# rakhimovv/lvt

Hardware: AMD Instinct MI355X
Metric: video-clips/sec/node (VQVAE+DSFVT train step, BAIR 64x64x16) (higher is better)
Workload: dtype f32

## Files before the change

include/lvt_hip.h:

```cpp
#ifndef LVT_HIP_H
#define LVT_HIP_H
#include <stddef.h>
#include <stdint.h>
#ifdef __cplusplus
extern "C" {
#endif

#define LVT_OK            0
#define LVT_EINVAL      (-1)
#define LVT_EWORKSPACE  (-2)
#define LVT_ELAUNCH     (-3)
#define LVT_ENODEVICE   (-4)

const char *lvt_last_error(void);
int lvt_version(void);
int lvt_device_info(char *name, int name_len, int *cus, int *clock_khz, long long *hbm_bytes);

#define LVT_MATH_F32   (1 << 16)
#define LVT_MATH_F16X2 (1 << 18)
typedef struct { const float *a; const float *b; float *c; } lvt_amax_io;
int lvt_amax(const float *x, long long n, float *out, void *stream);
typedef struct { const float *x; long long n; float *out; } lvt_amax_entry;
int lvt_amax_multi(const lvt_amax_entry *entries, int n, void *stream);
int lvt_amax_merge(const float *a, const float *b, float *out, void *stream);
#define LVT_VQ_COARSE  (1 << 17)
#define LVT_VQ_GENERIC (1 << 22)

#define LVT_EPI_BIAS        1
#define LVT_EPI_RESIDUAL    2
#define LVT_EPI_RELU        4
#define LVT_EPI_TANH        8
#define LVT_EPI_MASK       16
#define LVT_EPI_ACCUM      32
#define LVT_EPI_PLANES     64
#define LVT_CAUSAL_KMAX   (1 << 8)
#define LVT_CAUSAL_KMIN   (1 << 9)
#define LVT_CAUSAL_TILE   (1 << 10)

typedef struct {
    int M, N, K;
    int ta, tb;
    const float *A; long long lda; int a_kb; long long a_skb;
    const float *B; long long ldb; int b_kb; long long b_skb;
    float *C;       long long ldc;
    int batch_outer, batch_inner;
    long long sA_o, sA_i, sB_o, sB_i, sC_o, sC_i;
    float alpha;
    int flags;
    const float *bias;
    const float *res;  long long ldr;
    const float *mask; long long ldm;
    int splits;
    float *a_colsum;
    long long c_plane;
    const float *a_amax, *b_amax;
    const float *a_amax2, *b_amax2;
    float *c_amax;
} lvt_gemm_desc;
size_t lvt_gemm_workspace_bytes(const lvt_gemm_desc *d);
int lvt_gemm_f32(const lvt_gemm_desc *d, void *workspace, size_t workspace_bytes, void *stream);

int lvt_vq_argmax_scores(const float *scores, long long rows, int K, long long ld, const float *codebook, int D,
                         long long *idx, void *stream);

typedef struct {
    int M, N, K;
    const void *A; long long lda; int a_planes; int a_kb; long long a_skb;
    const void *B; long long ldb;
    float *C; long long ldc;
    int batch_outer, batch_inner;
    long long sA_o, sA_i, sB_o, sB_i, sC_o, sC_i;
    float alpha;
    int flags;
    const float *bias;
    const float *res;  long long ldr;
    const float *mask; long long ldm;
    const float *a_amax, *b_amax;
    float *c_amax;
    void *Cp; long long ldcp; const float *cp_amax;
} lvt_gemm_p2_desc;
int lvt_gemm_p2_f32(const lvt_gemm_p2_desc *d, void *stream);
typedef struct { const float *src; void *dst; int rows, cols; long long ld_src, ld_dst; int transpose; const float *amax;
                 int batch; long long bs_src, bs_dst; } lvt_p2_pack_entry;
int lvt_p2_pack_multi(const lvt_p2_pack_entry *entries, int n, void *stream);

int lvt_gemm_smallm_f32(int M, int N, int K, int tb, const float *A, long long lda, const float *B,
                        long long ldb, float *C, long long ldc, int batch, long long sB, long long sC,
                        float alpha, int flags, const float *bias, const float *res, long long ldr,
                        const int *pos, long long c_pos, long long r_pos, void *stream);
size_t lvt_gemm_smallm_splitk_workspace_bytes(int M, int N, int splits);
int lvt_gemm_smallm_splitk_f32(int M, int N, int K, int splits, const float *A, long long lda, const float *B,
                               long long ldb, float *C, long long ldc, float alpha, int flags, const float *bias,
                               const float *res, long long ldr, const int *pos, long long c_pos, long long r_pos,
                               void *workspace, size_t workspace_bytes, void *stream);
int lvt_gemm_smallm_partial_f32(int M, int N, int K, int splits, const float *A, long long lda, const float *B,
                                long long ldb, void *workspace, size_t workspace_bytes, void *stream);
int lvt_splitsum_layernorm_fwd(const float *partials, int splits, int rows, int d, const float *bias, const float *res,
                               long long ldr, float *x_out, float eps, const float *w, const float *b, float *y,
                               void *stream);

typedef struct {
    int N, Ti, Hi, Wi, Ci;
    int To, Ho, Wo, Co;
    int Kt, Kh, Kw;
    int st, sh, sw;
    int pt, ph, pw;
} lvt_conv_geom;
int lvt_conv3d_pack_weight(const lvt_conv_geom *g, const float *w, int Ci_real, int Co_real,
                           float *wp, void *stream);
typedef struct { const float *w; float *dst; int kind, taps, Ci, Co, Ci_real, Co_real; } lvt_pack_entry;
int lvt_conv3d_pack_weights_multi(const lvt_pack_entry *entries, int n, void *stream);
#define LVT_CONV_WEIGHT_IMAGE (1 << 21)
typedef struct { const float *wp; int rows, cols; const float *amax; } lvt_weight_image_entry;
size_t lvt_conv3d_weight_image_bytes(int rows, int cols);
int lvt_conv3d_weight_images(const lvt_weight_image_entry *entries, int n, void *stream);
int lvt_conv3d_pack_weight_t(const lvt_conv_geom *g, const float *w, int Ci_real, int Co_real,
                             float *wt, void *stream);
int lvt_conv3d_uses_patch_kernel(const lvt_conv_geom *g, int flags);
int lvt_conv3d_fwd_uses_parity_kernel(const lvt_conv_geom *g, int flags);
int lvt_conv3d_pack_weight_parity(const lvt_conv_geom *g, const float *w, int Ci_real, int Co_real,
                                  float *wq, void *stream);
int lvt_conv3d_fwd_parity(const lvt_conv_geom *g, const float *x, const float *wq, const float *bias,
                          const float *res, const float *mask, float *y, int flags, const lvt_amax_io *ax,
        void *stream);
int lvt_conv3d_fwd(const lvt_conv_geom *g, const float *x, const float *wp, const float *bias,
                   const float *res, const float *mask, float *y, int flags, const lvt_amax_io *ax,
        void *stream);
int lvt_conv3d_bwd_data_uses_phase_kernel(const lvt_conv_geom *g, int flags);
int lvt_conv3d_pack_weight_phases(const lvt_conv_geom *g, const float *w, int Ci_real, int Co_real,
                                  float *wph, void *stream);
int lvt_conv3d_bwd_data_phases(const lvt_conv_geom *g, const float *dy, const float *wph, const float *bias,
                               const float *res, const float *mask, float *dx, int flags, const lvt_amax_io *ax,
        void *stream);
int lvt_conv3d_bwd_data(const lvt_conv_geom *g, const float *dy, const float *wp, const float *bias,
                        const float *res, const float *mask, float *dx, int flags, const lvt_amax_io *ax,
        void *stream);
size_t lvt_conv3d_bwd_weight_workspace_bytes(const lvt_conv_geom *g);
int lvt_conv3d_bwd_weight_fuses_bias(const lvt_conv_geom *g, int flags);
#define LVT_WGRAD_DB_OF_X (1 << 20)
int lvt_conv3d_bwd_weight(const lvt_conv_geom *g, const float *x, const float *dy, float *dw, float *db,
                          int Ci_real, int Co_real, int flags, const lvt_amax_io *ax, void *workspace,
                          size_t workspace_bytes, void *stream);
int lvt_convt4_fwd(const float *x, const float *w, const float *bias, int N, int Hi, int Wi, int Ci, int Cr,
                   int act_tanh, float *y, int flags, const lvt_amax_io *ax, void *stream);
size_t lvt_colsum_workspace_bytes(long long M, int N);
int lvt_colsum(const float *g, long long M, int N, long long ld, float *out, void *workspace,
               size_t workspace_bytes, void *stream);

size_t lvt_vq_nearest_workspace_bytes(long long rows, int num, int KC);
size_t lvt_vq_nearest_generic_workspace_bytes(int num, int D, int KC);
int lvt_vq_nearest(const float *z, long long rows, int ldz, int num, int D, int KC,
                   const float *codebooks, long long *idx, int P, int flags, void *workspace, size_t workspace_bytes,
                   void *stream);
int lvt_vq_gather(const long long *idx, const float *codebooks, long long rows, int num, int D, int KC,
                  int P, float *out, int ldo, void *stream);
size_t lvt_vq_ema_workspace_bytes(long long rows, int num, int D, int KC);
int lvt_vq_ema_accumulate(const long long *idx, const float *z, long long rows, int ldz, int num, int D,
                          int KC, int P, float *stats, void *workspace, size_t workspace_bytes,
                          void *stream);
int lvt_vq_ema_finalize(const float *stats, int num, int D, int KC, float decay, float eps,
                        float *running_size, float *running_sum, float *weight, void *stream);

int lvt_to_channels_last(const float *in, int B, int C, long long R, int ldo, int mode, const float *a,
                         const float *s, float *out, float *out_amax, void *stream);
int lvt_to_channels_first(const float *in, int B, int C, long long R, int ldi, int mode, const float *a,
                          const float *s, float lo, float hi, float *out, void *stream);

size_t lvt_reduce_workspace_bytes(void);
int lvt_mse_fwd(const float *a, const float *b, long long n, double denom, float scale, float *out,
                void *workspace, size_t workspace_bytes, void *stream);
int lvt_mse_bwd(const float *a, const float *b, long long n, double denom, float scale,
                const float *gout_dev, const float *add, int tanh_of_a, float *out, float *out_amax, void *stream);
int lvt_l1_fwd(const float *a, const float *b, long long n, double denom, float scale, float *out,
               void *workspace, size_t workspace_bytes, void *stream);
int lvt_l1_bwd(const float *a, const float *b, long long n, double denom, float scale,
               const float *gout_dev, const float *add, int tanh_of_a, float *out, float *out_amax, void *stream);
int lvt_tanh_bwd(const float *g, const float *y, long long n, float *out, float *out_amax, void *stream);
int lvt_axpy(const float *x, const float *add, long long n, const float *alpha_dev, float alpha,
             float *out, void *stream);
int lvt_add_periodic(float *x, const float *table, long long rows, int P, int d, void *stream);

int lvt_layernorm_fwd(const float *x, long long rows, int d, float eps, const float *w, const float *b,
                      float *y, float *mean, float *rstd, float *y_amax, const float *w_amax, const float *b_amax,
                      void *stream);
int lvt_layernorm_fwd_p2(const float *x, long long rows, int d, float eps, const float *w, const float *b,
                         float *y, void *yp, float *mean, float *rstd, float *y_amax, const float *w_amax,
                         const float *b_amax, void *stream);
size_t lvt_layernorm_bwd_workspace_bytes(int d);
int lvt_layernorm_bwd(const float *dy, const float *x, const float *mean, const float *rstd,
                      const float *w, long long rows, int d, const float *add, float *dx, float *dw,
                      float *db, float *dx_amax, void *workspace, size_t workspace_bytes, void *stream);

int lvt_attn_softmax_fwd(float *scores, int B, int H, int S, float temper, const float *dt,
                         const float *dh, const float *dw, int bt, int bh, int bw, int masked, float fill,
                         void *stream);
int lvt_attn_softmax_bwd(const float *P, float *dP, int B, int H, int S, float temper, int bt, int bh,
                         int bw, float *G, float *ddt, float *ddh, float *ddw, void *stream);

int lvt_attn_fwd(const float *q, const float *k, const float *v, int B, int H, int S, int da, float temper,
                 const float *dt, const float *dh, const float *dw, int bt, int bh, int bw, int masked, float fill,
                 float *P, float *o, void *stream);

int lvt_attn_planes_supported(int S, int da, int bt, int bh, int bw);
int lvt_attn_fwd_planes(const void *qkv_planes, long long plane_stride, long long operand_stride, int B, int H, int S, int da,
                        float temper, const float *dt, const float *dh, const float *dw, int bt, int bh, int bw, int masked,
                        float fill, float *P, float *o, float *o_amax, void *stream);
size_t lvt_attn_bwd_planes_workspace_bytes(int B, int H, int S, int bt, int bh, int bw);
int lvt_attn_bwd_planes(const void *qkv_planes, long long plane_stride, long long operand_stride, const void *do_planes,
                        const float *P, const float *o, int B, int H, int S, int da, float temper, int bt, int bh, int bw,
                        int masked, float *dq, float *dk, float *dv, float *ddt, float *ddh, float *ddw, float *d_amax,
                        void *workspace, size_t workspace_bytes, void *stream);

int lvt_attn_flash_supported(int S, int da, int bt, int bh, int bw);
int lvt_attn_fwd_flash(const float *q, const float *k, const float *v, long long ld, int B, int H, int S, int da,
                       float temper, const float *dt, const float *dh, const float *dw, int bt, int bh, int bw,
                       int masked, float fill, float *o, float *stats, float *o_amax, void *stream);
size_t lvt_attn_bwd_flash_workspace_bytes(int B, int H, int S, int bt, int bh, int bw);
int lvt_attn_bwd_flash(const float *q, const float *k, const float *v, const float *d_o, long long ld, const float *stats,
                       const float *o, int B, int H, int S, int da, float temper, const float *dt, const float *dh, const float *dw,
                       int bt, int bh, int bw, int masked, float fill, float *dq, float *dk, float *dv, float *ddt,
                       float *ddh, float *ddw, float *d_amax, void *workspace, size_t workspace_bytes, void *stream);

int lvt_attn_decode(const float *q, long long ldq, const float *Kc, const float *Vc, int B, int H, int S, int da, int qi,
                    float temper, const float *dt, const float *dh, const float *dw, int bt, int bh, int bw,
                    float *o, const int *pos, long long q_pos, void *stream);

int lvt_decode_gather_codes(const long long *codes, const long long *nb, const int *pos, int rows, int S1, int taps,
                            long long *out, void *stream);
int lvt_decode_commit(const long long *drawn, int rows, int S1, long long *codes, int *pos, void *stream);

int lvt_sample_categorical(const float *logits, long long rows, int V, float temp, const float *u,
                           long long *out, long long out_stride, float *probs, const int *pos, long long u_pos,
                           void *stream);

int lvt_embbag_fwd(const long long *idx, long long bstride, int P, long long rows, int nslots,
                   const int *slot_off, const int *tab_row, const float *table, int D, const float *bias,
                   const float *btable, const long long *bindex, float *out, void *stream);
#define LVT_ONEHOT_DENSE (1 << 19)
size_t lvt_onehot_tn_workspace_bytes(int nslots, int V, int N, long long rows);
int lvt_onehot_tn_is_gather(int nslots, int V, int N, long long ldb, const float *dout, int flags);
int lvt_onehot_tn_gemm(const long long *idx, int nslots, int V, const int *slot_off, long long bstride,
                       long long pstride, int P, long long rows, const float *dout, long long ldb, int N,
                       float *out, int flags, const float *dout_amax, void *workspace, size_t workspace_bytes,
                       void *stream);
int lvt_permute3(const float *in, long long s0, long long s1, long long s2, int n0, int n1, int n2,
                 float *out, void *stream);

int lvt_row_gather(const float *x, const long long *perm, long long B, int S, int d, float *out, void *stream);

int lvt_slice_context(const long long *video, int B, int T, int nc, int H, int W, const int *abc, int st, int sh,
                      int sw, int kt, int kh, int kw, int n_prime, long long pad_value, long long *ctx,
                      long long *slice, long long *slice_idx, unsigned char *ignore, void *stream);

size_t lvt_xent_workspace_bytes(void);
int lvt_xent_fwd(const float *logits, const long long *target, long long tstride_b, long long tstride_pos,
                 int P, long long rows, int V, long long ignore, float scale, float *row_loss, float *lse,
                 float *loss, float *count, void *workspace, size_t workspace_bytes, void *stream);
int lvt_xent_bwd(const float *logits, const long long *target, long long tstride_b, long long tstride_pos,
                 int P, long long rows, int V, long long ignore, const float *lse, const float *count,
                 const float *gout, float scale, float *dlogits, float *dl_amax, void *stream);

typedef struct {
    float *p; const float *g; float *s0; float *s1;
    long long n; float lr; float wd;
} lvt_opt_entry;
int lvt_adam_step(const lvt_opt_entry *entries, int n, float beta1, float beta2, float eps, int step,
                  void *stream);
int lvt_rmsprop_step(const lvt_opt_entry *entries, int n, float alpha, float eps, float momentum,
                     void *stream);

#define LVT_BN_RUNNING  1
#define LVT_BN_UPDATE   2
#define LVT_BN_UNBIASED 4
#define LVT_BN_COUNT    8
#define LVT_BN_TRAIN    16
size_t lvt_bn_workspace_bytes(long long M, int Cp);
int lvt_bn_stats(const float *y, long long M, int Cp, float *stats, void *workspace, size_t workspace_bytes, void *stream);
int lvt_bn_finalize(const float *stats, int nranks, long long count, int C, int Cp, const float *gamma, const float *beta,
                    float *running_mean, float *running_var, long long *num_batches_tracked, float momentum, float eps,
                    int flags, float *scale, float *shift, float *saved, void *stream);
int lvt_bn_apply(const float *y, const float *res, long long M, int Cp, const float *scale, const float *shift, int flags,
                 float *out, float *out_amax, void *stream);
int lvt_bn_bwd_reduce(const float *g, const float *y, long long M, int Cp, const float *saved, float *sums, void *workspace,
                      size_t workspace_bytes, void *stream);
int lvt_bn_bwd_apply(const float *g, const float *y, long long M, int Cp, const float *scale, const float *saved,
                     const float *sums, long long n, int flags, float *dy, float *dy_amax, void *stream);
typedef struct {
    const float *w; float *w_out; int outer, Co, inner, Cp;
    const float *gamma, *beta, *running_mean, *running_var; float eps;
    float *bias_out; float *w_amax;
} lvt_bn_fold_entry;
int lvt_bn_fold(const lvt_bn_fold_entry *entries, int n, void *stream);

#ifdef __cplusplus
}
#endif
#endif
```

lvt_amd/csrc/attention_flash.hip:

```cpp
#include "attn_common.h"

namespace {

template <int I> struct IC { static constexpr int value = I; };
template <int N, int I = 0, class F> __device__ __forceinline__ void static_for(F &&f) {
    if constexpr (I < N) { f(IC<I>{}); static_for<N, I + 1>(f); }
}

typedef _Float16 f16x8 __attribute__((ext_vector_type(8)));
typedef _Float16 f16x2v __attribute__((ext_vector_type(2)));
typedef float f32x2 __attribute__((ext_vector_type(2)));
typedef float f32x4v __attribute__((ext_vector_type(4)));
typedef short s16x4 __attribute__((ext_vector_type(4)));
typedef __attribute__((address_space(3))) s16x4 lds_s16x4;
typedef unsigned u32x4 __attribute__((ext_vector_type(4)));

#define FA_LD 144
#define FA_PL (64 * FA_LD)
#define FA_SLOT (2 * FA_PL)
#define FA_EMIN 30
#define FA_EMAX 254
#define FA_LOG2E 1.4426950408889634f

typedef unsigned u32x2 __attribute__((ext_vector_type(2)));

__device__ __forceinline__ float fa_u2f(unsigned u) { return __uint_as_float(u); }
__device__ __forceinline__ float fa_exp_field(int e) { return e <= 0 ? 0.f : fa_u2f((unsigned)e << 23); }
__device__ __forceinline__ int fa_clamp_e(int e) { return e < FA_EMIN ? FA_EMIN : (e > FA_EMAX ? FA_EMAX : e); }
__device__ __forceinline__ int fa_ebits(float nonneg) { return fa_clamp_e((int)((__float_as_uint(nonneg) >> 23) & 0xffu)); }
template <int CTRL> __device__ __forceinline__ float fa_dpp_max(float v) {
    const int o = __builtin_amdgcn_update_dpp(0, __builtin_bit_cast(int, v), CTRL, 0xf, 0xf, false);
    return fmaxf(v, __builtin_bit_cast(float, o));
}
__device__ __forceinline__ float fa_row16_max(float v) {
    v = fa_dpp_max<0xB1>(v);
    v = fa_dpp_max<0x4E>(v);
    v = fa_dpp_max<0x141>(v);
    v = fa_dpp_max<0x140>(v);
    return v;
}
__device__ __forceinline__ float fa_kg_max(float v) {
    u32x2 r = __builtin_amdgcn_permlane16_swap(__float_as_uint(v), __float_as_uint(v), false, false);
    v = fmaxf(fa_u2f(r[0]), fa_u2f(r[1]));
    r = __builtin_amdgcn_permlane32_swap(__float_as_uint(v), __float_as_uint(v), false, false);
    return fmaxf(fa_u2f(r[0]), fa_u2f(r[1]));
}
__device__ __forceinline__ float fa_kg_sum(float v) {
    u32x2 r = __builtin_amdgcn_permlane16_swap(__float_as_uint(v), __float_as_uint(v), false, false);
    v = fa_u2f(r[0]) + fa_u2f(r[1]);
    r = __builtin_amdgcn_permlane32_swap(__float_as_uint(v), __float_as_uint(v), false, false);
    return fa_u2f(r[0]) + fa_u2f(r[1]);
}
__device__ __forceinline__ float fa_max4(const f32x4v a) { return fmaxf(fmaxf(a[0], a[1]), fmaxf(a[2], a[3])); }
__device__ __forceinline__ float fa_absmax4(const float4 a) { return fmaxf(fmaxf(fabsf(a.x), fabsf(a.y)), fmaxf(fabsf(a.z), fabsf(a.w))); }

__device__ __forceinline__ float fa_mix_lo(unsigned h, float c) {
    float r;
    asm("v_fma_mix_f32 %0, %1, %2, %3 op_sel:[0,0,0] op_sel_hi:[1,0,0]" : "=v"(r) : "v"(h), "v"(-1.f), "v"(c));
    return r;
}
__device__ __forceinline__ float fa_mix_hi(unsigned h, float c) {
    float r;
    asm("v_fma_mix_f32 %0, %1, %2, %3 op_sel:[1,0,0] op_sel_hi:[1,0,0]" : "=v"(r) : "v"(h), "v"(-1.f), "v"(c));
    return r;
}
__device__ __forceinline__ void fa_split_pair(float a, float b, float s, unsigned &ph, unsigned &pl) {
    const f32x2 t = f32x2{a, b} * s;
    ph = __builtin_bit_cast(unsigned, __builtin_convertvector(t, f16x2v));
    const f32x2 r = {fa_mix_lo(ph, t.x), fa_mix_hi(ph, t.y)};
    pl = __builtin_bit_cast(unsigned, __builtin_convertvector(r, f16x2v));
}
__device__ __forceinline__ void fa_split_pair1(float a, float b, unsigned &ph, unsigned &pl) {
    const f32x2 t = {a, b};
    ph = __builtin_bit_cast(unsigned, __builtin_convertvector(t, f16x2v));
    const f32x2 r = {fa_mix_lo(ph, a), fa_mix_hi(ph, b)};
    pl = __builtin_bit_cast(unsigned, __builtin_convertvector(r, f16x2v));
}
__device__ __forceinline__ void fa_split8(const float (&v)[8], f16x8 &h, f16x8 &l) {
    u32x4 uh, ul;
    unsigned a, b;
    fa_split_pair1(v[0], v[1], a, b); uh[0] = a; ul[0] = b;
    fa_split_pair1(v[2], v[3], a, b); uh[1] = a; ul[1] = b;
    fa_split_pair1(v[4], v[5], a, b); uh[2] = a; ul[2] = b;
// ... 758 lines not shown
#pragma unroll
        for (int qt = 0; qt < 2; ++qt) {
            const int T = 2 * c + qt;
            const f32x4v qinv = *reinterpret_cast<const f32x4v *>(cinv + 16 * qt + 4 * kg);
            const f32x4v doinv = *reinterpret_cast<const f32x4v *>(cinv + 32 + 16 * qt + 4 * kg);
            const float bth = bt_[T / HP] + dhl[HSTEP * (T % HP)];
            const f32x4v qk = qinv * kc, bm = bw4 + bth;
            const f32x4v lds = l4[qt] * (doinv * srun);
            const f32x4v qzl = l4[qt] * qinv;
            const f32x4v dvq = (doinv * vinv) * qzl, dq_ = d4[qt] * qzl;
#pragma unroll
            for (int r = 0; r < 4; ++r) {
                float x = fa_score(st[qt][r], qk[r], bm[r]);
                if (MASKED && j > 16 * T + 4 * kg + r) x = A.fill2;
                const float ex = __builtin_amdgcn_exp2f(x - m4[qt][r]);
                pw[4 * qt + r] = ex * lds[r];
                u[4 * qt + r] = (ex * fmaf(dp[qt][r], dvq[r], -dq_[r])) * zrun;
            }
        }
        f16x8 pbh, pbl, ubh, ubl;
        fa_split8(pw, pbh, pbl);
        fa_split8(u, ubh, ubl);
        f16x8 ao[2][2], aqt[2];
        auto load_o = [&](int d_, int bf) {
#pragma unroll
            for (int pl = 0; pl < 2; ++pl) ao[bf][pl] = fa_trfrag(cur, pl, 32, d_, c16, kg);
        };
        load_o(0, 0);
        static_for<AT_D / 16>([&](auto dc) {
            constexpr int d = decltype(dc)::value, bf = d & 1;
#pragma unroll
            for (int pl = 0; pl < 2; ++pl) aqt[pl] = fa_trfrag(cur, pl, 0, d, c16, kg);
            accv[d] = fa_mfma(ao[bf][1], pbh, accv[d]);
            accv[d] = fa_mfma(ao[bf][0], pbl, accv[d]);
            accv[d] = fa_mfma(ao[bf][0], pbh, accv[d]);
            if constexpr (d + 1 < AT_D / 16) load_o(d + 1, bf ^ 1);
            acck[d] = fa_mfma(aqt[1], ubh, acck[d]);
            acck[d] = fa_mfma(aqt[0], ubl, acck[d]);
            acck[d] = fa_mfma(aqt[0], ubh, acck[d]);
            __builtin_amdgcn_sched_group_barrier(0x100, 4, 0);
            __builtin_amdgcn_sched_group_barrier(0x008, 3, 0);
            if constexpr (d + 1 < AT_D / 16) __builtin_amdgcn_sched_group_barrier(0x100, 4, 0);
            __builtin_amdgcn_sched_group_barrier(0x008, 3, 0);
            __builtin_amdgcn_sched_barrier(0);
        });
        __syncthreads();
    });
    const float fvs = domax * (1.f / 32768.f), fks = fa_exp_field(zb - 14) * A.inv_temper;
    float am = 0.f;
    {
        float *vrow = A.dv + (row0 + j) * A.ld + h * AT_D + 4 * kg, *krow = A.dk + (row0 + j) * A.ld + h * AT_D + 4 * kg;
#pragma unroll
        for (int d = 0; d < AT_D / 16; ++d) {
            const f32x4v ov = accv[d] * fvs, ok = acck[d] * fks;
            *reinterpret_cast<f32x4v *>(vrow + 16 * d) = ov;
            *reinterpret_cast<f32x4v *>(krow + 16 * d) = ok;
#pragma unroll
            for (int e = 0; e < 4; ++e) am = fmaxf(am, fmaxf(fabsf(ov[e]), fabsf(ok[e])));
        }
    }
    return am;
}

template <int BT, int BH, int BW, int MASKED>
__global__ __launch_bounds__(512, 1) void lvt_attn_bwd_flash_b_kernel(const FaArgs A, float *__restrict__ d_amax) {
    __shared__ __attribute__((aligned(16))) FaSmemB sm;
    if (threadIdx.x >= 256) __builtin_amdgcn_s_setprio(1);
    float am;
    if (MASKED) {
        if (fa_half(blockIdx.x) == 0) am = fa_bwd_b_body<BT, BH, BW, MASKED, 0, 8>(A, sm, fa_pair(blockIdx.x), 0);
        else am = fa_bwd_b_body<BT, BH, BW, MASKED, 4, 4>(A, sm, fa_pair(blockIdx.x), 1);
    } else {
        am = fa_bwd_b_body<BT, BH, BW, MASKED, 0, 8>(A, sm, fa_pair(blockIdx.x), fa_half(blockIdx.x));
    }
    if (d_amax) {
        __syncthreads();
        lvt_block_amax_commit(am, d_amax, reinterpret_cast<float *>(sm.ring[0]));
    }
}

__global__ __launch_bounds__(256) void lvt_attn_flash_bank_reduce_kernel(const float *__restrict__ partial, int B, int H, int NB, int nt,
                                                                         int nh, float *__restrict__ ddt, float *__restrict__ ddh,
                                                                         float *__restrict__ ddw) {
    const int idx = blockIdx.x * 4 + (threadIdx.x >> 6), lane = threadIdx.x & 63;
    if (idx >= H * NB) return;
    const int h = idx / NB, e = idx % NB;
    float s = 0.f;
    for (int jj = lane; jj < 2 * B; jj += 64) s += partial[(((long long)(jj >> 1) * H + h) * 2 + (jj & 1)) * NB + e];
#pragma unroll
    for (int m = 32; m >= 1; m >>= 1) s += __shfl_xor(s, m, 64);
    if (lane) return;
    const int nw = NB - nt - nh;
    if (e < nt) ddt[h * nt + e] = nt == 1 ? 0.f : s;
    else if (e < nt + nh) ddh[h * nh + e - nt] = nh == 1 ? 0.f : s;
    else ddw[h * nw + e - nt - nh] = nw == 1 ? 0.f : s;
}

}

extern "C" int lvt_attn_flash_supported(int S, int da, int bt, int bh, int bw) {
    return S == AT_S && da == AT_D && ((bt == 1 && bh == 16 && bw == 16) || (bt == 4 && bh == 8 && bw == 8)) ? 1 : 0;
}

#define LVT_FA_GEOMS(X) X(1, 16, 16) X(4, 8, 8)

extern "C" int lvt_attn_fwd_flash(const float *q, const float *k, const float *v, long long ld, int B, int H, int S, int da,
                                  float temper, const float *dt, const float *dh, const float *dw, int bt, int bh, int bw,
                                  int masked, float fill, float *o, float *stats, float *o_amax, void *stream) {
    LVT_REQUIRE(q && k && v && dt && dh && dw && o && stats && B > 0 && H > 0, "attn_fwd_flash: bad args");
    LVT_REQUIRE((B * H) % 8 == 0, "attn_fwd_flash: B * H = %d must be a multiple of 8 (workgroup pairing per XCD)", B * H);
    LVT_REQUIRE(lvt_attn_flash_supported(S, da, bt, bh, bw), "attn_fwd_flash: S=%d da=%d block (%d,%d,%d) has no instantiation", S, da, bt, bh, bw);
    LVT_REQUIRE(lvt_aligned16(q) && lvt_aligned16(k) && lvt_aligned16(v) && lvt_aligned16(o) && lvt_aligned16(stats) && ld % 4 == 0 &&
                ld >= (long long)H * da, "attn_fwd_flash: alignment / row stride");
    FaArgs A = {};
    A.q = q; A.k = k; A.v = v; A.ld = ld; A.H = H; A.inv_temper = 1.f / temper; A.c1 = FA_LOG2E / temper; A.fill2 = fill * FA_LOG2E;
    A.dt = dt; A.dh = dh; A.dw = dw; A.o = o; A.m = stats; A.l = stats + (size_t)B * H * S;
    const dim3 grid((unsigned)(B * H * (masked ? 1 : 2))), blk(512);
    hipStream_t s = (hipStream_t)stream;
#define LVT_X(BT, BH, BW)                                                                                       \
    if (bt == BT && bh == BH && bw == BW) {                                                                     \
        if (masked) hipLaunchKernelGGL((lvt_attn_fwd_flash_kernel<BT, BH, BW, 1>), grid, blk, 0, s, A, o_amax); \
        else hipLaunchKernelGGL((lvt_attn_fwd_flash_kernel<BT, BH, BW, 0>), grid, blk, 0, s, A, o_amax);        \
    }
    LVT_FA_GEOMS(LVT_X)
#undef LVT_X
    LVT_CHECK_LAUNCH("lvt_attn_fwd_flash_kernel");
    return LVT_OK;
}

extern "C" size_t lvt_attn_bwd_flash_workspace_bytes(int B, int H, int S, int bt, int bh, int bw) {
    const size_t nb = (size_t)(2 * bt - 1) + (2 * bh - 1) + (2 * bw - 1);
    return (size_t)B * H * S * sizeof(float) + (size_t)B * H * 4 * sizeof(float) + (size_t)B * H * 2 * nb * sizeof(float);
}

extern "C" int lvt_attn_bwd_flash(const float *q, const float *k, const float *v, const float *d_o, long long ld, const float *stats,
                                  const float *o, int B, int H, int S, int da, float temper, const float *dt, const float *dh, const float *dw,
                                  int bt, int bh, int bw, int masked, float fill, float *dq, float *dk, float *dv, float *ddt,
                                  float *ddh, float *ddw, float *d_amax, void *workspace, size_t workspace_bytes, void *stream) {
    LVT_REQUIRE(q && k && v && d_o && stats && dt && dh && dw && dq && dk && dv && ddt && ddh && ddw && B > 0 && H > 0, "attn_bwd_flash: bad args");
    LVT_REQUIRE((B * H) % 8 == 0, "attn_bwd_flash: B * H = %d must be a multiple of 8 (workgroup pairing per XCD)", B * H);
    LVT_REQUIRE(lvt_attn_flash_supported(S, da, bt, bh, bw), "attn_bwd_flash: S=%d da=%d block (%d,%d,%d) has no instantiation", S, da, bt, bh, bw);
    LVT_REQUIRE(lvt_aligned16(q) && lvt_aligned16(k) && lvt_aligned16(v) && lvt_aligned16(d_o) && lvt_aligned16(stats) && lvt_aligned16(dq) &&
                lvt_aligned16(dk) && lvt_aligned16(dv) && ld % 4 == 0 && ld >= (long long)H * da, "attn_bwd_flash: alignment / row stride");
    if (!workspace || workspace_bytes < lvt_attn_bwd_flash_workspace_bytes(B, H, S, bt, bh, bw) || !lvt_aligned16(workspace)) {
        lvt_set_error("attn_bwd_flash: workspace too small or misaligned");
        return LVT_EWORKSPACE;
    }
    FaArgs A = {};
    A.q = q; A.k = k; A.v = v; A.d_o = d_o; A.ld = ld; A.H = H; A.inv_temper = 1.f / temper; A.c1 = FA_LOG2E / temper; A.fill2 = fill * FA_LOG2E;
    A.dt = dt; A.dh = dh; A.dw = dw; A.m = const_cast<float *>(stats); A.l = const_cast<float *>(stats) + (size_t)B * H * S;
    A.dq = dq; A.dk = dk; A.dv = dv;
    LVT_REQUIRE(!o || lvt_aligned16(o), "attn_bwd_flash: o must be 16-byte aligned");
    const bool onep = o != nullptr;
    A.o = const_cast<float *>(o);
    A.delta = (float *)workspace;
    A.scal = A.delta + (size_t)B * H * S;
    A.bank_partial = A.scal + (size_t)B * H * 4;
    const int nt = 2 * bt - 1, nh = 2 * bh - 1, nw = 2 * bw - 1, nb = nt + nh + nw;
    const dim3 grid((unsigned)(B * H * (masked ? 1 : 2))), blk(512);
    const dim3 gridb((unsigned)(B * H * 2));
    hipStream_t s = (hipStream_t)stream;
#define LVT_X(BT, BH, BW)                                                                                         \
    if (bt == BT && bh == BH && bw == BW) {                                                                       \
        if (masked && onep) hipLaunchKernelGGL((lvt_attn_bwd_flash_a_kernel<BT, BH, BW, 1, 1>), grid, blk, 0, s, A, d_amax); \
        else if (masked) hipLaunchKernelGGL((lvt_attn_bwd_flash_a_kernel<BT, BH, BW, 1, 0>), grid, blk, 0, s, A, d_amax);    \
        else if (onep) hipLaunchKernelGGL((lvt_attn_bwd_flash_a_kernel<BT, BH, BW, 0, 1>), grid, blk, 0, s, A, d_amax);      \
        else hipLaunchKernelGGL((lvt_attn_bwd_flash_a_kernel<BT, BH, BW, 0, 0>), grid, blk, 0, s, A, d_amax);                \
    }
    LVT_FA_GEOMS(LVT_X)
#undef LVT_X
    LVT_CHECK_LAUNCH("lvt_attn_bwd_flash_a_kernel");
#define LVT_X(BT, BH, BW)                                                                                         \
    if (bt == BT && bh == BH && bw == BW) {                                                                       \
        if (masked) hipLaunchKernelGGL((lvt_attn_bwd_flash_b_kernel<BT, BH, BW, 1>), gridb, blk, 0, s, A, d_amax); \
        else hipLaunchKernelGGL((lvt_attn_bwd_flash_b_kernel<BT, BH, BW, 0>), grid, blk, 0, s, A, d_amax);        \
    }
    LVT_FA_GEOMS(LVT_X)
#undef LVT_X
    LVT_CHECK_LAUNCH("lvt_attn_bwd_flash_b_kernel");
    hipLaunchKernelGGL(lvt_attn_flash_bank_reduce_kernel, dim3((unsigned)lvt_cdiv((long long)H * nb, 4)), dim3(256), 0, s,
                       A.bank_partial, B, H, nb, nt, nh, ddt, ddh, ddw);
    LVT_CHECK_LAUNCH("lvt_attn_flash_bank_reduce_kernel");
    return LVT_OK;
}
```

lvt_amd/csrc/elementwise.hip:

```cpp
#include "lvt_common.h"

static inline int grid_for(long long n, int per_block, int cap = 8192) {
    long long b = lvt_cdiv(n, per_block);
    if (b < 1) b = 1;
    return (int)(b < cap ? b : cap);
}

__device__ __forceinline__ float wave_sum(float v) {
#pragma unroll
    for (int off = 32; off >= 1; off >>= 1) v += __shfl_xor(v, off);
    return v;
}
__device__ __forceinline__ float wave_max(float v) {
#pragma unroll
    for (int off = 32; off >= 1; off >>= 1) v = fmaxf(v, __shfl_xor(v, off));
    return v;
}

__global__ void lvt_to_channels_last_kernel(const float *__restrict__ in, int B, int C, long long R, int ldo,
                                            int mode, const float *__restrict__ a, const float *__restrict__ s,
                                            float *__restrict__ out, float *__restrict__ out_amax) {
    __shared__ float amax_scratch[4];
    float am = 0.f;
    const long long total = (long long)B * R * ldo;
    for (long long i = (long long)blockIdx.x * blockDim.x + threadIdx.x; i < total;
         i += (long long)gridDim.x * blockDim.x) {
        const int c = i % ldo; const long long t = i / ldo;
        const long long r = t % R; const long long b = t / R;
        float v = 0.f;
        if (c < C) {
            v = in[(b * C + c) * R + r];
            if (mode == 1) v = (v - a[c]) / s[c];
        }
        out[i] = v;
        am = fmaxf(am, lvt_absf(v));
    }
    if (out_amax) lvt_block_amax_commit(am, out_amax, amax_scratch);
}
__global__ void lvt_to_channels_first_kernel(const float *__restrict__ in, int B, int C, long long R, int ldi,
                                             int mode, const float *__restrict__ a, const float *__restrict__ s,
                                             float lo, float hi, float *__restrict__ out) {
    const long long total = (long long)B * C * R;
    for (long long i = (long long)blockIdx.x * blockDim.x + threadIdx.x; i < total;
         i += (long long)gridDim.x * blockDim.x) {
        const long long r = i % R; const long long t = i / R;
        const int c = t % C; const long long b = t / C;
        float v = in[(b * R + r) * ldi + c];
        if (mode == 2) { v = v * s[c] + a[c]; v = fminf(fmaxf(v, lo), hi); }
        out[i] = v;
    }
}

extern "C" int lvt_to_channels_last(const float *in, int B, int C, long long R, int ldo, int mode, const float *a,
                                    const float *s, float *out, float *out_amax, void *stream) {
    LVT_REQUIRE(in && out && B > 0 && C > 0 && R > 0 && ldo >= C, "to_channels_last: bad args");
    LVT_REQUIRE(mode == 0 || (a && s), "to_channels_last: affine tables missing");
    hipLaunchKernelGGL(lvt_to_channels_last_kernel, dim3(grid_for((long long)B * R * ldo, 256, out_amax ? 2048 : 8192)), dim3(256), 0,
                       (hipStream_t)stream, in, B, C, R, ldo, mode, a, s, out, out_amax);
    LVT_CHECK_LAUNCH("lvt_to_channels_last_kernel");
    return LVT_OK;
}
extern "C" int lvt_to_channels_first(const float *in, int B, int C, long long R, int ldi, int mode, const float *a,
                                     const float *s, float lo, float hi, float *out, void *stream) {
    LVT_REQUIRE(in && out && B > 0 && C > 0 && R > 0 && ldi >= C, "to_channels_first: bad args");
    LVT_REQUIRE(mode == 0 || (a && s), "to_channels_first: affine tables missing");
    hipLaunchKernelGGL(lvt_to_channels_first_kernel, dim3(grid_for((long long)B * C * R, 256)), dim3(256), 0,
                       (hipStream_t)stream, in, B, C, R, ldi, mode, a, s, lo, hi, out);
    LVT_CHECK_LAUNCH("lvt_to_channels_first_kernel");
    return LVT_OK;
}

#define RED_BLOCKS 1024
template <int L1>
__global__ void lvt_sqdiff_partial_kernel(const float *__restrict__ a, const float *__restrict__ b, long long n4,
                                          float *__restrict__ partial) {
    __shared__ float red[256];
    float s = 0.f;
    for (long long i = (long long)blockIdx.x * blockDim.x + threadIdx.x; i < n4;
         i += (long long)gridDim.x * blockDim.x) {
        const float4 x = reinterpret_cast<const float4 *>(a)[i];
        const float4 y = reinterpret_cast<const float4 *>(b)[i];
        const float d0 = x.x - y.x, d1 = x.y - y.y, d2 = x.z - y.z, d3 = x.w - y.w;
        if (L1) s += (fabsf(d0) + fabsf(d1)) + (fabsf(d2) + fabsf(d3));
// ... 284 lines not shown
    const int d4 = d / 4;
    float4 adw[LN_MAXV], adb[LN_MAXV];
#pragma unroll
    for (int i = 0; i < LN_MAXV; ++i) { adw[i] = make_float4(0.f, 0.f, 0.f, 0.f); adb[i] = adw[i]; }
    const long long rows_per_block = lvt_cdiv(rows, gridDim.x);
    const long long r0 = blockIdx.x * rows_per_block;
    const long long r1 = min(rows, r0 + rows_per_block);
    for (long long row0 = r0 + wave; row0 < r1; row0 += 4 * LN_BWD_ROWS) {
        float4 xh[LN_BWD_ROWS][LN_MAXV], gw[LN_BWD_ROWS][LN_MAXV], zv[LN_BWD_ROWS][LN_MAXV];
        float rs[LN_BWD_ROWS], s1[LN_BWD_ROWS], s2[LN_BWD_ROWS];
#pragma unroll
        for (int u = 0; u < LN_BWD_ROWS; ++u) {
            const long long row = row0 + 4 * u;
            if (row >= r1) continue;
            if (add) {
#pragma unroll
                for (int i = 0; i < LN_MAXV; ++i)
                    if (lane + 64 * i < d4) zv[u][i] = reinterpret_cast<const float4 *>(add + row * d)[lane + 64 * i];
            }
            const float m = mean[row];
            rs[u] = rstd[row];
            const float4 *xp = reinterpret_cast<const float4 *>(x + row * d);
            const float4 *gp = reinterpret_cast<const float4 *>(dy + row * d);
            s1[u] = 0.f; s2[u] = 0.f;
#pragma unroll
            for (int i = 0; i < LN_MAXV; ++i) {
                const int c = lane + 64 * i;
                if (c < d4) {
                    const float4 xv = xp[c], gv = gp[c], ww = reinterpret_cast<const float4 *>(w)[c];
                    const float r = rs[u];
                    xh[u][i] = make_float4((xv.x - m) * r, (xv.y - m) * r, (xv.z - m) * r, (xv.w - m) * r);
                    gw[u][i] = make_float4(gv.x * ww.x, gv.y * ww.y, gv.z * ww.z, gv.w * ww.w);
                    const float4 h = xh[u][i], g = gw[u][i];
                    s1[u] += (g.x + g.y) + (g.z + g.w);
                    s2[u] += (g.x * h.x + g.y * h.y) + (g.z * h.z + g.w * h.w);
                    adw[i].x += gv.x * h.x; adw[i].y += gv.y * h.y; adw[i].z += gv.z * h.z; adw[i].w += gv.w * h.w;
                    adb[i].x += gv.x; adb[i].y += gv.y; adb[i].z += gv.z; adb[i].w += gv.w;
                }
            }
        }
#pragma unroll
        for (int u = 0; u < LN_BWD_ROWS; ++u) {
            const long long row = row0 + 4 * u;
            if (row >= r1) continue;
            const float m1 = wave_sum(s1[u]) / d, m2 = wave_sum(s2[u]) / d;
            float4 *op = reinterpret_cast<float4 *>(dx + row * d);
#pragma unroll
            for (int i = 0; i < LN_MAXV; ++i) {
                const int c = lane + 64 * i;
                if (c < d4) {
                    const float4 h = xh[u][i], g = gw[u][i];
                    const float r = rs[u];
                    float4 o;
                    o.x = r * (g.x - m1 - h.x * m2); o.y = r * (g.y - m1 - h.y * m2);
                    o.z = r * (g.z - m1 - h.z * m2); o.w = r * (g.w - m1 - h.w * m2);
                    if (add) {
                        const float4 z = zv[u][i];
                        o.x += z.x; o.y += z.y; o.z += z.z; o.w += z.w;
                    }
                    op[c] = o;
                    am = fmaxf(am, fmaxf(fmaxf(lvt_absf(o.x), lvt_absf(o.y)), fmaxf(lvt_absf(o.z), lvt_absf(o.w))));
                }
            }
        }
    }
    if (dx_amax) lvt_block_amax_commit(am, dx_amax, amax_scratch);
#pragma unroll
    for (int i = 0; i < LN_MAXV; ++i) {
        const int c = lane + 64 * i;
        if (c < d4) {
            reinterpret_cast<float4 *>(sdw[wave])[c] = adw[i];
            reinterpret_cast<float4 *>(sdb[wave])[c] = adb[i];
        }
    }
    __syncthreads();
    for (int c = threadIdx.x; c < d; c += 256) {
        pdw[(long long)blockIdx.x * d + c] = ((sdw[0][c] + sdw[1][c]) + sdw[2][c]) + sdw[3][c];
        pdb[(long long)blockIdx.x * d + c] = ((sdb[0][c] + sdb[1][c]) + sdb[2][c]) + sdb[3][c];
    }
}
__global__ __launch_bounds__(256) void lvt_rowsum_partials_kernel(const float *__restrict__ partial0, const float *__restrict__ partial1,
                                                                  int nblk, int n, float *__restrict__ out0, float *__restrict__ out1) {
    __shared__ float red[256];
    const float *partial = blockIdx.y ? partial1 : partial0;
    float *out = blockIdx.y ? out1 : out0;
    constexpr int cols = 8, RL = 256 / cols;
    const int c = blockIdx.x * cols + (threadIdx.x % cols);
    const int rl = threadIdx.x / cols;
    float s0 = 0.f, s1 = 0.f, s2 = 0.f, s3 = 0.f;
    if (c < n) {
        int b = rl;
        for (; b + 3 * RL < nblk; b += 4 * RL) {
            s0 += partial[(long long)b * n + c]; s1 += partial[(long long)(b + RL) * n + c];
            s2 += partial[(long long)(b + 2 * RL) * n + c]; s3 += partial[(long long)(b + 3 * RL) * n + c];
        }
        for (; b < nblk; b += RL) s0 += partial[(long long)b * n + c];
    }
    float s = (s0 + s1) + (s2 + s3);
    red[threadIdx.x] = s;
    __syncthreads();
    if (rl == 0 && c < n) {
        for (int k = 1; k < RL; ++k) s += red[k * cols + threadIdx.x];
        out[c] = s;
    }
}
extern "C" size_t lvt_layernorm_bwd_workspace_bytes(int d) { return (size_t)2 * LN_BWD_BLOCKS * d * sizeof(float); }
extern "C" int lvt_layernorm_bwd(const float *dy, const float *x, const float *mean, const float *rstd,
                                 const float *w, long long rows, int d, const float *add, float *dx, float *dw,
                                 float *db, float *dx_amax, void *workspace, size_t workspace_bytes, void *stream) {
    LVT_REQUIRE(dy && x && mean && rstd && w && dx && dw && db && rows > 0 && d % 4 == 0 && d <= 256 * LN_MAXV,
                "layernorm_bwd: bad args");
    LVT_REQUIRE(workspace && workspace_bytes >= lvt_layernorm_bwd_workspace_bytes(d), "layernorm_bwd: workspace");
    hipStream_t s = (hipStream_t)stream;
    int blocks = (int)(lvt_cdiv(rows, 8) < LN_BWD_BLOCKS ? lvt_cdiv(rows, 8) : LN_BWD_BLOCKS);
    const long long rpb = lvt_cdiv(rows, blocks);
    blocks = (int)lvt_cdiv(rows, rpb);
    float *pdw = (float *)workspace, *pdb = pdw + (size_t)LN_BWD_BLOCKS * d;
    hipLaunchKernelGGL(lvt_layernorm_bwd_kernel, dim3(blocks), dim3(256), 0, s, dy, x, mean, rstd, w, rows, d, add,
                       dx, pdw, pdb, dx_amax);
    LVT_CHECK_LAUNCH("lvt_layernorm_bwd_kernel");
    hipLaunchKernelGGL(lvt_rowsum_partials_kernel, dim3((d + 7) / 8, 2), dim3(256), 0, s, (const float *)pdw, (const float *)pdb,
                       blocks, d, dw, db);
    LVT_CHECK_LAUNCH("lvt_rowsum_partials_kernel");
    return LVT_OK;
}

struct SliceGeom { int B, T, nc, H, W, st, sh, sw, kt, kh, kw, n_prime, t, h, w, Tc, Hc, Wc; long long pad; };
__global__ void lvt_slice_context_kernel(const long long *__restrict__ video, const int *__restrict__ abc, SliceGeom g,
                                         long long *__restrict__ ctx, long long *__restrict__ slice,
                                         long long *__restrict__ slice_idx, unsigned char *__restrict__ ignore) {
    const long long n_ctx = (long long)g.B * g.nc * g.Tc * g.Hc * g.Wc;
    const long long n_sl = (long long)g.B * g.nc * g.t * g.h * g.w;
    const long long n_ig = (long long)g.B * g.t * g.h * g.w;
    const long long total = n_ctx + n_sl + n_ig + g.B;
    for (long long i = (long long)blockIdx.x * blockDim.x + threadIdx.x; i < total; i += (long long)gridDim.x * blockDim.x) {
        if (i < n_ctx) {
            long long r = i;
            const int ow = r % g.Wc; r /= g.Wc;
            const int oh = r % g.Hc; r /= g.Hc;
            const int ot = r % g.Tc; r /= g.Tc;
            const int ch = r % g.nc; const int b = r / g.nc;
            const int a = abc[3 * b], bo = abc[3 * b + 1], c = abc[3 * b + 2];
            const int ti = ot - g.kt / 2 + a, hi = oh - g.kh / 2 + bo, wi = ow - g.kw / 2 + c;
            long long v = g.pad;
            if ((unsigned)ti < (unsigned)g.T && (unsigned)hi < (unsigned)g.H && (unsigned)wi < (unsigned)g.W) {
                const int mine = ((ti % g.st) * g.sh + (hi % g.sh)) * g.sw + (wi % g.sw);
                if (mine < (a * g.sh + bo) * g.sw + c)
                    v = video[((((long long)b * g.T + ti) * g.nc + ch) * g.H + hi) * g.W + wi];
            }
            ctx[i] = v;
        } else if (i < n_ctx + n_sl) {
            long long r = i - n_ctx;
            const int wi = r % g.w; r /= g.w;
            const int hi = r % g.h; r /= g.h;
            const int ti = r % g.t; r /= g.t;
            const int ch = r % g.nc; const int b = r / g.nc;
            const int a = abc[3 * b], bo = abc[3 * b + 1], c = abc[3 * b + 2];
            slice[i - n_ctx] = video[((((long long)b * g.T + ti * g.st + a) * g.nc + ch) * g.H + hi * g.sh + bo) * g.W + wi * g.sw + c];
        } else if (i < n_ctx + n_sl + n_ig) {
            long long r = i - n_ctx - n_sl;
            r /= (long long)g.h * g.w;
            const int ti = r % g.t; const int b = r / g.t;
            ignore[i - n_ctx - n_sl] = (ti * g.st + abc[3 * b]) < g.n_prime ? 1 : 0;
        } else {
            const int b = (int)(i - n_ctx - n_sl - n_ig);
            slice_idx[b] = (abc[3 * b] * g.sh + abc[3 * b + 1]) * g.sw + abc[3 * b + 2];
        }
    }
}
extern "C" int lvt_slice_context(const long long *video, int B, int T, int nc, int H, int W, const int *abc, int st, int sh,
                                 int sw, int kt, int kh, int kw, int n_prime, long long pad_value, long long *ctx,
                                 long long *slice, long long *slice_idx, unsigned char *ignore, void *stream) {
    LVT_REQUIRE(video && abc && ctx && slice && slice_idx && ignore, "slice_context: null pointer");
    LVT_REQUIRE(B > 0 && nc > 0 && st > 0 && sh > 0 && sw > 0 && T % st == 0 && H % sh == 0 && W % sw == 0 &&
                kt > 0 && kh > 0 && kw > 0, "slice_context: bad geometry");
    SliceGeom g;
    g.B = B; g.T = T; g.nc = nc; g.H = H; g.W = W; g.st = st; g.sh = sh; g.sw = sw; g.kt = kt; g.kh = kh; g.kw = kw;
    g.n_prime = n_prime; g.pad = pad_value;
    g.t = T / st; g.h = H / sh; g.w = W / sw;
    g.Tc = 2 * (kt / 2) + (g.t - 1) * st + 1; g.Hc = 2 * (kh / 2) + (g.h - 1) * sh + 1; g.Wc = 2 * (kw / 2) + (g.w - 1) * sw + 1;
    const long long total = (long long)B * nc * g.Tc * g.Hc * g.Wc + (long long)B * (nc + 1) * g.t * g.h * g.w + B;
    const int blocks = (int)(lvt_cdiv(total, 256) < 4096 ? lvt_cdiv(total, 256) : 4096);
    hipLaunchKernelGGL(lvt_slice_context_kernel, dim3(blocks), dim3(256), 0, (hipStream_t)stream, video, abc, g, ctx, slice,
                       slice_idx, ignore);
    LVT_CHECK_LAUNCH("lvt_slice_context_kernel");
    return LVT_OK;
}

__global__ void lvt_row_gather_kernel(const float *__restrict__ x, const long long *__restrict__ perm, long long B, int S,
                                      int d4, float *__restrict__ out) {
    const long long total = B * S * d4;
    for (long long i = (long long)blockIdx.x * blockDim.x + threadIdx.x; i < total; i += (long long)gridDim.x * blockDim.x) {
        const int c = i % d4; const long long r = i / d4;
        const int s = r % S; const long long b = r / S;
        reinterpret_cast<float4 *>(out)[i] = reinterpret_cast<const float4 *>(x)[(b * S + perm[s]) * d4 + c];
    }
}
extern "C" int lvt_row_gather(const float *x, const long long *perm, long long B, int S, int d, float *out, void *stream) {
    LVT_REQUIRE(x && perm && out && B > 0 && S > 0 && d > 0 && d % 4 == 0 && lvt_aligned16(x) && lvt_aligned16(out),
                "row_gather: bad args");
    const long long total = B * S * (d / 4);
    const int blocks = (int)(lvt_cdiv(total, 256) < 8192 ? lvt_cdiv(total, 256) : 8192);
    hipLaunchKernelGGL(lvt_row_gather_kernel, dim3(blocks), dim3(256), 0, (hipStream_t)stream, x, perm, B, S, d / 4, out);
    LVT_CHECK_LAUNCH("lvt_row_gather_kernel");
    return LVT_OK;
}

// ... 74 lines not shown
```

lvt_amd/csrc/gemm_engine.hip:

```cpp
#include "lvt_common.h"
#include "epilogue_fast.h"
#include <string.h>
#include <stdlib.h>
#include <stdint.h>
#include <type_traits>

typedef float f32x16 __attribute__((ext_vector_type(16)));

#define BK 32
#define NTHREADS 256

enum { A_KPLAIN = 0, A_MPLAIN = 1, A_CONV_K = 2, A_CONVT_K = 3, A_CONV_M = 4, A_ONEHOT_M = 5, A_PATCH = 6, A_PATCHT = 7 };
enum { B_KPLAIN = 0, B_NPLAIN = 1, B_CONVT_W = 2 };

struct KParams {
    int M, N, K;
    const float *A; long long lda; int a_kb; long long a_skb;
    const float *B; long long ldb; int b_kb; long long b_skb;
    float *C; long long ldc; long long c_plane;
    int batch_inner;
    long long sA_o, sA_i, sB_o, sB_i, sC_o, sC_i;
    float alpha; int flags;
    const float *bias; const float *res; long long ldr; const float *mask; long long ldm;
    int splits; int k_per_split; float *partial; long long partial_stride;
    int vec_epi;
    float *colsum_partial;
    const float *a_amax, *b_amax;
    const float *a_amax2, *b_amax2;
    float *c_amax;
    lvt_conv_geom g;
    const char *b_img;
    int Tq, Hq, Wq;
    int jT, jH, jW;
    const long long *oh_idx; long long oh_bstride, oh_pstride; int oh_P, oh_V; int oh_off[32];
};

__device__ __forceinline__ float4 ldg4(const float *p) { return *reinterpret_cast<const float4 *>(p); }

__device__ __forceinline__ unsigned cvt_pk_bf16(float lo, float hi) {
    unsigned r;
    asm("v_cvt_pk_bf16_f32 %0, %1, %2" : "=v"(r) : "v"(lo), "v"(hi));
    return r;
}
__device__ __forceinline__ float bf_lo(unsigned p) { return __uint_as_float(p << 16); }
__device__ __forceinline__ float bf_hi(unsigned p) { return __uint_as_float(p & 0xffff0000u); }
__device__ __forceinline__ void split3(const float4 v, uint2 &p1, uint2 &p2, uint2 &p3) {
    p1.x = cvt_pk_bf16(v.x, v.y); p1.y = cvt_pk_bf16(v.z, v.w);
    const float r0 = v.x - bf_lo(p1.x), r1 = v.y - bf_hi(p1.x), r2 = v.z - bf_lo(p1.y), r3 = v.w - bf_hi(p1.y);
    p2.x = cvt_pk_bf16(r0, r1); p2.y = cvt_pk_bf16(r2, r3);
    const float s0 = r0 - bf_lo(p2.x), s1 = r1 - bf_hi(p2.x), s2 = r2 - bf_lo(p2.y), s3 = r3 - bf_hi(p2.y);
    p3.x = cvt_pk_bf16(s0, s1); p3.y = cvt_pk_bf16(s2, s3);
}
#define HLD 40
template <int ROWS> __device__ __forceinline__ int hrow(int m) {
    if (ROWS >= 128) {
        const int r = (m & ~127) + ((m & 3) << 5) + ((m & 127) >> 2);
        return r * HLD + (r >> 5) * 32;
    }
    return m * HLD;
}
template <int ROWS> struct HPlane { static constexpr int SIZE = ROWS * HLD + (ROWS >= 128 ? ROWS : 0); };
template <int ROWS> __device__ __forceinline__ void store_split_k(unsigned short *lds, int row, int k4, const float4 v) {
    uint2 p1, p2, p3;
    split3(v, p1, p2, p3);
    unsigned short *d = lds + hrow<ROWS>(row) + k4;
    *reinterpret_cast<uint2 *>(d) = p1;
    *reinterpret_cast<uint2 *>(d + HPlane<ROWS>::SIZE) = p2;
    *reinterpret_cast<uint2 *>(d + 2 * HPlane<ROWS>::SIZE) = p3;
}
template <int ROWS> __device__ __forceinline__ void store_split_m(unsigned short *lds, int row4, int k, const float4 v) {
    uint2 p[3];
    split3(v, p[0], p[1], p[2]);
#pragma unroll
    for (int q = 0; q < 3; ++q) {
        unsigned short *d = lds + q * HPlane<ROWS>::SIZE + k;
        d[hrow<ROWS>(row4)] = (unsigned short)(p[q].x & 0xffffu); d[hrow<ROWS>(row4 + 1)] = (unsigned short)(p[q].x >> 16);
        d[hrow<ROWS>(row4 + 2)] = (unsigned short)(p[q].y & 0xffffu); d[hrow<ROWS>(row4 + 3)] = (unsigned short)(p[q].y >> 16);
    }
}
template <int ROWS> __device__ __forceinline__ void store_split_block(unsigned short *lds, int row4, int k4, const float4 *v) {
    store_split_k<ROWS>(lds, row4 + 0, k4, make_float4(v[0].x, v[1].x, v[2].x, v[3].x));
    store_split_k<ROWS>(lds, row4 + 1, k4, make_float4(v[0].y, v[1].y, v[2].y, v[3].y));
    store_split_k<ROWS>(lds, row4 + 2, k4, make_float4(v[0].z, v[1].z, v[2].z, v[3].z));
    store_split_k<ROWS>(lds, row4 + 3, k4, make_float4(v[0].w, v[1].w, v[2].w, v[3].w));
// ... 1343 lines not shown
                for (int i = 0; i < TM; ++i) a[q][i] = *reinterpret_cast<const f16x8 *>(cur + fa[i] + q * PSA + ks);
#pragma unroll
                for (int j = 0; j < TN; ++j) b[q][j] = *reinterpret_cast<const f16x8 *>(cur + fb[j] + q * PSB + ks);
            }
#pragma unroll
            for (int i = 0; i < TM; ++i)
#pragma unroll
                for (int j = 0; j < TN; ++j)
                    acx[i][j] = __builtin_amdgcn_mfma_f32_32x32x16_f16(a[0][i], b[1][j], acx[i][j], 0, 0, 0);
#pragma unroll
            for (int i = 0; i < TM; ++i)
#pragma unroll
                for (int j = 0; j < TN; ++j)
                    acc[i][j] = __builtin_amdgcn_mfma_f32_32x32x16_f16(a[0][i], b[0][j], acc[i][j], 0, 0, 0);
#pragma unroll
            for (int i = 0; i < TM; ++i)
#pragma unroll
                for (int j = 0; j < TN; ++j)
                    acx[i][j] = __builtin_amdgcn_mfma_f32_32x32x16_f16(a[1][i], b[0][j], acx[i][j], 0, 0, 0);
            if (ks == 0) {
                if constexpr (decltype(do_store)::value) store(nxt);
                if constexpr (decltype(do_fetch)::value) fetch();
            }
        }
    };
    typedef std::integral_constant<bool, true> yes_t;
    typedef std::integral_constant<bool, false> no_t;

    const int ntiles = kbeg < kend ? (kend - kbeg) / BK : 0;
    if (ntiles > 0) {
        fetch();
        store(S0);
        if (ntiles > 1) fetch();
    }
    __syncthreads();
    int kt = 0;
    for (; kt + 2 < ntiles; ++kt) {
        tile(S0 + (kt & 1) * STAGE, S0 + ((kt + 1) & 1) * STAGE, yes_t(), yes_t());
        __syncthreads();
    }
    if (kt + 1 < ntiles) {
        tile(S0 + (kt & 1) * STAGE, S0 + ((kt + 1) & 1) * STAGE, yes_t(), no_t());
        __syncthreads();
        ++kt;
    }
    if (kt < ntiles) tile(S0 + (kt & 1) * STAGE, nullptr, no_t(), no_t());
    __syncthreads();
    lvt_f16x2_finish<TM, TN>(acc, acx, unscale);

    if (TA && sum_on) {
        float *scratch = lds;
        *reinterpret_cast<float4 *>(&scratch[(kk0 * 64 + mq) * 4]) = colacc;
        __syncthreads();
        if (tid < BM) {
            float s_ = 0.f;
            for (int r = 0; r < 8; ++r) s_ += scratch[(r * 64 + tid / 4) * 4 + (tid & 3)];
            if (m0 + tid < p.M) p.colsum_partial[((long long)tc.split * gridDim.y + tc.z) * p.M + m0 + tid] = s_;
        }
        __syncthreads();
    }
    if (p.vec_epi && !(p.flags & (LVT_EPI_PLANES | LVT_EPI_ACCUM | LVT_EPI_TANH))) {
        LvtEpi e;
        e.M = p.M; e.N = p.N;
        float *wave_tile = lds + wave * (32 * TN * 32);
        if (p.splits > 1) {
            e.C = p.partial; e.ldc = p.N; e.coff = tc.split * p.partial_stride + (long long)tc.z * p.M * p.N; e.alpha = 1.f; e.flags = 0;
            e.bias = nullptr; e.res = nullptr; e.ldr = 0; e.mask = nullptr; e.ldm = 0;
            (void)lvt_epi_fast_wave<0, TM, TN>(e, acc, wave_tile, m0 + wm * (TM * 32), n0 + wn * (TN * 32), lane);
            return;
        }
        const unsigned seen = lvt_amax_peek(p.c_amax);
        e.C = p.C; e.ldc = p.ldc; e.coff = tc.coff; e.alpha = p.alpha; e.flags = p.flags;
        e.bias = p.bias; e.res = p.res; e.ldr = p.ldr; e.mask = p.mask; e.ldm = p.ldm;
        const float am_w = lvt_epi_fast_dispatch<TM, TN>(e, acc, wave_tile, m0 + wm * (TM * 32), n0 + wn * (TN * 32), lane);
        if (p.c_amax) lvt_block_amax_commit_seen(am_w, p.c_amax, lds + TURN_FLOATS, seen);
        return;
    }
    if (p.vec_epi) lvt_epilogue_vec<AMODE, BM, BN, WM, WN>(p, acc, lds, m0, n0, wm, wn, lane, 0, tc.coff, tc.z, tc.split);
    else lvt_epilogue<AMODE, BM, BN, WM, WN>(p, acc, m0, n0, wm, wn, l31, half, 0, tc.coff, tc.z, tc.split);
}

__global__ void lvt_reduce_splits_kernel(const float *__restrict__ partial, long long n4, long long stride,
                                         int splits, float *__restrict__ out, int accumulate) {
    long long i = (long long)blockIdx.x * blockDim.x + threadIdx.x;
    const long long step = (long long)gridDim.x * blockDim.x;
    for (; i < n4; i += step) {
        float4 s0 = ldg4(partial + i * 4), s1 = zero4(), s2 = zero4(), s3 = zero4();
        int k = 1;
        for (; k + 3 < splits; k += 4) {
            const float4 t0 = ldg4(partial + k * stride + i * 4), t1 = ldg4(partial + (k + 1) * stride + i * 4);
            const float4 t2 = ldg4(partial + (k + 2) * stride + i * 4), t3 = ldg4(partial + (k + 3) * stride + i * 4);
            s0.x += t0.x; s0.y += t0.y; s0.z += t0.z; s0.w += t0.w;
            s1.x += t1.x; s1.y += t1.y; s1.z += t1.z; s1.w += t1.w;
            s2.x += t2.x; s2.y += t2.y; s2.z += t2.z; s2.w += t2.w;
            s3.x += t3.x; s3.y += t3.y; s3.z += t3.z; s3.w += t3.w;
        }
        for (; k < splits; ++k) {
            const float4 t = ldg4(partial + k * stride + i * 4);
            s0.x += t.x; s0.y += t.y; s0.z += t.z; s0.w += t.w;
        }
        float4 s;
        s.x = (s0.x + s1.x) + (s2.x + s3.x); s.y = (s0.y + s1.y) + (s2.y + s3.y);
        s.z = (s0.z + s1.z) + (s2.z + s3.z); s.w = (s0.w + s1.w) + (s2.w + s3.w);
        float4 *o = reinterpret_cast<float4 *>(out + i * 4);
        if (accumulate) { const float4 c = *o; s.x += c.x; s.y += c.y; s.z += c.z; s.w += c.w; }
        *o = s;
    }
}

__global__ void lvt_pack_weight_kernel(const float *__restrict__ w, float *__restrict__ wp, int taps, int Ci,
                                       int Co, int Ci_real, int Co_real) {
    const long long total = (long long)taps * Ci * Co;
    for (long long i = (long long)blockIdx.x * blockDim.x + threadIdx.x; i < total;
         i += (long long)gridDim.x * blockDim.x) {
        const int co = i % Co; long long t = i / Co;
        const int ci = t % Ci; const int tap = t / Ci;
        float v = 0.f;
        if (co < Co_real && ci < Ci_real) v = w[((long long)co * Ci_real + ci) * taps + tap];
        wp[i] = v;
    }
}
__global__ void lvt_pack_weight_t_kernel(const float *__restrict__ w, float *__restrict__ wt, int taps, int Ci,
                                         int Co, int Ci_real, int Co_real) {
    const long long total = (long long)taps * Co * Ci;
    for (long long i = (long long)blockIdx.x * blockDim.x + threadIdx.x; i < total;
         i += (long long)gridDim.x * blockDim.x) {
        const int ci = i % Ci; long long t = i / Ci;
        const int co = t % Co; const int tr = t / Co;
        float v = 0.f;
        if (co < Co_real && ci < Ci_real) v = w[((long long)co * Ci_real + ci) * taps + (taps - 1 - tr)];
        wt[i] = v;
    }
}
__global__ void lvt_pack_weight_phases_kernel(const float *__restrict__ w, float *__restrict__ wph, int Ci, int Co,
                                              int Ci_real, int Co_real) {
    const long long total = 16LL * Co * Ci;
    for (long long i = (long long)blockIdx.x * blockDim.x + threadIdx.x; i < total; i += (long long)gridDim.x * blockDim.x) {
        const int ci = i % Ci; long long t = i / Ci;
        const int co = t % Co; const int pt = t / Co;
        const int ph = pt >> 2, tap = pt & 3;
        const int ky = 3 - (ph >> 1) - 2 * (tap >> 1), kx = 3 - (ph & 1) - 2 * (tap & 1);
        float v = 0.f;
        if (co < Co_real && ci < Ci_real) v = w[(((long long)co * Ci_real + ci) * 4 + ky) * 4 + kx];
        wph[i] = v;
    }
}
__global__ void lvt_pack_weight_parity_kernel(const float *__restrict__ w, float *__restrict__ wq, int Ci, int Co,
                                              int Ci_real, int Co_real) {
    const long long total = 16LL * Ci * Co;
    for (long long i = (long long)blockIdx.x * blockDim.x + threadIdx.x; i < total; i += (long long)gridDim.x * blockDim.x) {
        const int co = i % Co; long long t = i / Co;
        const int ci = t % Ci; const int ct = t / Ci;
        const int cls = ct >> 2, tap = ct & 3;
        const int ky = 2 * (tap >> 1) + (cls >> 1), kx = 2 * (tap & 1) + (cls & 1);
        float v = 0.f;
        if (co < Co_real && ci < Ci_real) v = w[(((long long)co * Ci_real + ci) * 4 + ky) * 4 + kx];
        wq[i] = v;
    }
}
#define UW_CO 64
#define UW_CI 4
#define UW_WAVES 16
__global__ __launch_bounds__(64 * UW_WAVES) void lvt_unpack_wgrad_tiled_kernel(const float *__restrict__ partial, long long stride,
                                                                               int splits, float *__restrict__ dw, int taps, int Ci,
                                                                               int Co) {
    extern __shared__ float tile[];
    const int ld = UW_CI * taps + 1;
    const int nco = Co / UW_CO;
    const int co0 = (blockIdx.x % nco) * UW_CO, ci0 = (blockIdx.x / nco) * UW_CI;
    const int lane_co = threadIdx.x & (UW_CO - 1), r0 = threadIdx.x >> 6;
    const int rows = taps * UW_CI;
    for (int r = r0; r < rows; r += UW_WAVES) {
        const int tap = r / UW_CI, cil = r % UW_CI;
        const float *src = partial + ((long long)tap * Ci + ci0 + cil) * Co + co0 + lane_co;
        float s0 = 0.f, s1 = 0.f, s2 = 0.f, s3 = 0.f;
        int k = 0;
        for (; k + 3 < splits; k += 4) {
            s0 += src[k * stride]; s1 += src[(k + 1) * stride]; s2 += src[(k + 2) * stride]; s3 += src[(k + 3) * stride];
        }
        for (; k < splits; ++k) s0 += src[k * stride];
        tile[lane_co * ld + cil * taps + tap] = (s0 + s1) + (s2 + s3);
    }
    __syncthreads();
    const int per_co = UW_CI * taps;
    for (int e = threadIdx.x; e < UW_CO * per_co; e += 64 * UW_WAVES) {
        const int col = e / per_co, off = e % per_co;
        dw[((long long)(co0 + col) * Ci + ci0) * taps + off] = tile[col * ld + off];
    }
}

// ... 83 lines not shown
            ok = ok && al16(p.C) && p.ldc % 4 == 0 && p.sC_o % 4 == 0 && p.sC_i % 4 == 0;
            if (p.flags & LVT_EPI_BIAS) ok = ok && al16(p.bias);
            if (p.flags & LVT_EPI_RESIDUAL) ok = ok && al16(p.res) && p.ldr % 4 == 0;
            if (p.flags & LVT_EPI_MASK) ok = ok && al16(p.mask) && p.ldm % 4 == 0;
        }
        pv.vec_epi = ok ? 1 : 0;
    }
    if ((p.flags & LVT_EPI_PLANES) && !pv.vec_epi) {
        lvt_set_error("gemm: LVT_EPI_PLANES needs 16-byte aligned bias / res / mask and ldr, ldm %% 4 == 0");
        return LVT_EINVAL;
    }
    if (math_of(p.flags) == 2)
        hipLaunchKernelGGL((lvt_gemm_kernel<AMODE, BMODE, BM, BN, WM, WN, 2>), grid, dim3(NTHREADS), 0, s, pv);
    else if (math_of(p.flags) == 1)
        hipLaunchKernelGGL((lvt_gemm_kernel<AMODE, BMODE, BM, BN, WM, WN, 1>), grid, dim3(NTHREADS), 0, s, pv);
    else
        hipLaunchKernelGGL((lvt_gemm_kernel<AMODE, BMODE, BM, BN, WM, WN, 0>), grid, dim3(NTHREADS), 0, s, pv);
    LVT_CHECK_LAUNCH("lvt_gemm_kernel");
    return LVT_OK;
}

template <int TA, int TB>
static int launch_wide(const KParams &p, int zcount, hipStream_t s) {
    const long long ntm = lvt_cdiv(p.M, 256), ntn = lvt_cdiv(p.N, 128);
    if (ntm * ntn > 0x7fffffffLL || zcount > 65535 || p.splits > 65535) {
        lvt_set_error("gemm: grid too large (%lld tiles, z=%d, splits=%d)", ntm * ntn, zcount, p.splits);
        return LVT_EINVAL;
    }
    dim3 grid((unsigned)(ntm * ntn), (unsigned)zcount, (unsigned)(p.splits > 1 ? p.splits : 1));
    KParams pv = p;
    {
        auto al16 = [](const void *q) { return ((uintptr_t)q & 15) == 0; };
        bool ok = p.N % 4 == 0;
        if (p.splits > 1) ok = ok && al16(p.partial) && p.partial_stride % 4 == 0 && ((long long)p.M * p.N) % 4 == 0;
        else {
            ok = ok && al16(p.C) && p.ldc % 4 == 0 && p.sC_o % 4 == 0 && p.sC_i % 4 == 0;
            if (p.flags & LVT_EPI_BIAS) ok = ok && al16(p.bias);
            if (p.flags & LVT_EPI_RESIDUAL) ok = ok && al16(p.res) && p.ldr % 4 == 0;
            if (p.flags & LVT_EPI_MASK) ok = ok && al16(p.mask) && p.ldm % 4 == 0;
        }
        pv.vec_epi = ok ? 1 : 0;
    }
    if ((p.flags & LVT_EPI_PLANES) && !pv.vec_epi) {
        lvt_set_error("gemm: LVT_EPI_PLANES needs 16-byte aligned bias / res / mask and ldr, ldm %% 4 == 0");
        return LVT_EINVAL;
    }
    hipLaunchKernelGGL((lvt_gemm_wide_kernel<TA, TB>), grid, dim3(WIDE_THREADS), 0, s, pv);
    LVT_CHECK_LAUNCH("lvt_gemm_wide_kernel");
    return LVT_OK;
}

static int choose_splits(long long tiles, int K, int min_k) {
    int s = (int)((2 * LVT_NUM_CU) / (tiles > 0 ? tiles : 1));
    const int maxs = K / min_k > 0 ? K / min_k : 1;
    if (s > maxs) s = maxs;
    if (s < 1) s = 1;
    return s;
}

static void kparams_from_desc(const lvt_gemm_desc *d, KParams &p) {
    memset(&p, 0, sizeof(p));
    p.M = d->M; p.N = d->N; p.K = d->K;
    p.A = d->A; p.lda = d->lda; p.a_kb = d->a_kb > 0 ? d->a_kb : d->K; p.a_skb = d->a_skb;
    p.B = d->B; p.ldb = d->ldb; p.b_kb = d->b_kb > 0 ? d->b_kb : d->K; p.b_skb = d->b_skb;
    p.C = d->C; p.ldc = d->ldc; p.c_plane = d->c_plane;
    p.batch_inner = d->batch_inner > 0 ? d->batch_inner : 1;
    p.sA_o = d->sA_o; p.sA_i = d->sA_i; p.sB_o = d->sB_o; p.sB_i = d->sB_i; p.sC_o = d->sC_o; p.sC_i = d->sC_i;
    p.alpha = d->alpha; p.flags = d->flags; p.bias = d->bias; p.res = d->res; p.ldr = d->ldr;
    p.mask = d->mask; p.ldm = d->ldm;
    p.splits = d->splits > 1 ? d->splits : 1;
    p.a_amax = d->a_amax; p.b_amax = d->b_amax; p.c_amax = d->c_amax;
    p.a_amax2 = d->a_amax2; p.b_amax2 = d->b_amax2;
}

static int gemm_batch(const lvt_gemm_desc *d) {
    return (d->batch_outer > 0 ? d->batch_outer : 1) * (d->batch_inner > 0 ? d->batch_inner : 1);
}

extern "C" size_t lvt_gemm_workspace_bytes(const lvt_gemm_desc *d) {
    if (!d || d->splits <= 1) return 0;
    return (size_t)d->splits * gemm_batch(d) * ((size_t)d->M * d->N + (d->a_colsum ? (size_t)d->M : 0)) * sizeof(float);
}

extern "C" int lvt_gemm_f32(const lvt_gemm_desc *d, void *workspace, size_t workspace_bytes, void *stream) {
    LVT_REQUIRE(d && d->A && d->B && d->C, "gemm: null pointer");
    LVT_REQUIRE(d->M > 0 && d->N > 0 && d->K > 0, "gemm: bad shape %d %d %d", d->M, d->N, d->K);
    LVT_REQUIRE(d->K % 4 == 0, "gemm: K=%d must be a multiple of 4", d->K);
    LVT_REQUIRE(d->lda % 4 == 0 && d->ldb % 4 == 0, "gemm: lda/ldb must be multiples of 4");
    LVT_REQUIRE(lvt_aligned16(d->A) && lvt_aligned16(d->B), "gemm: A/B must be 16-byte aligned");
    LVT_REQUIRE(d->ta == 0 || d->M % 4 == 0, "gemm: ta=1 needs M %% 4 == 0");
    LVT_REQUIRE(d->tb == 0 || d->N % 4 == 0, "gemm: tb=1 needs N %% 4 == 0");
    LVT_REQUIRE(d->a_kb <= 0 || (d->a_kb % 4 == 0 && d->a_skb % 4 == 0), "gemm: a_kb/a_skb %% 4");
    LVT_REQUIRE(d->b_kb <= 0 || (d->b_kb % 4 == 0 && d->b_skb % 4 == 0), "gemm: b_kb/b_skb %% 4");
    LVT_REQUIRE(!(d->ta == 1 && d->tb == 0), "gemm: (ta=1, tb=0) is not instantiated");
    LVT_REQUIRE(!(d->flags & LVT_EPI_BIAS) || d->bias, "gemm: BIAS flag without bias");
    LVT_REQUIRE(!(d->flags & LVT_EPI_RESIDUAL) || d->res, "gemm: RESIDUAL flag without res");
    LVT_REQUIRE(!(d->flags & LVT_EPI_MASK) || d->mask, "gemm: MASK flag without mask");
    LVT_REQUIRE(math_of(d->flags) != 2 || (d->a_amax && d->b_amax), "gemm: LVT_MATH_F16X2 needs a_amax and b_amax");
    LVT_REQUIRE(!d->c_amax || d->splits <= 1, "gemm: c_amax is not produced by split-K launches");
    if (d->flags & LVT_EPI_PLANES)
        LVT_REQUIRE(d->splits <= 1 && !(d->flags & LVT_EPI_ACCUM) && d->N % 4 == 0 && d->ldc % 4 == 0 && d->c_plane % 4 == 0 &&
                    d->sC_o % 4 == 0 && d->sC_i % 4 == 0 && lvt_aligned16(d->C) && !(d->flags & LVT_MATH_F32),
                    "gemm: PLANES needs the bf16x3 arithmetic, no split-K / ACCUM, N, ldc, c_plane, sC %% 4 == 0 and an aligned C");
    hipStream_t s = (hipStream_t)stream;
    KParams p; kparams_from_desc(d, p);
    const int zc = gemm_batch(d);
    if (p.splits > 1) {
        LVT_REQUIRE((d->flags & ~(LVT_EPI_ACCUM | LVT_MATH_F32 | LVT_MATH_F16X2)) == 0 && d->alpha == 1.0f, "gemm: split-K allows only ACCUM");
        LVT_REQUIRE(d->ldc == d->N && (zc == 1 || (d->sC_i == (long long)d->M * d->N)),
                    "gemm: split-K needs a dense C (ldc == N)");
        LVT_REQUIRE(((long long)d->M * d->N) % 4 == 0 && lvt_aligned16(d->C), "gemm: split-K C alignment");
        const size_t need = lvt_gemm_workspace_bytes(d);
        if (workspace_bytes < need || !workspace) {
            lvt_set_error("gemm: workspace %zu < %zu", workspace_bytes, need);
            return LVT_EWORKSPACE;
        }
        p.k_per_split = (int)(lvt_cdiv(lvt_cdiv(p.K, p.splits), BK) * BK);
        p.partial = (float *)workspace;
        p.partial_stride = (long long)zc * d->M * d->N;
        if (d->a_colsum) {
            LVT_REQUIRE(d->ta == 1 && d->M % 4 == 0, "gemm: a_colsum needs ta == 1 and M %% 4 == 0");
            p.colsum_partial = p.partial + (long long)p.splits * p.partial_stride;
        }
    } else {
        LVT_REQUIRE(!d->a_colsum, "gemm: a_colsum needs splits > 1");
    }
    int rc;
    const long long a_span = d->ta ? (long long)d->K * d->lda : (long long)d->M * d->lda + (long long)(d->K / p.a_kb) * d->a_skb;
    const long long b_span = d->tb ? (long long)d->K * d->ldb : (long long)d->N * d->ldb + (long long)(d->K / p.b_kb) * d->b_skb;
    const bool wide = math_of(d->flags) == 2 && d->M > 128 && d->K % BK == 0 && p.a_kb % BK == 0 &&
                      p.b_kb % BK == 0 && a_span < (1LL << 30) && b_span < (1LL << 30) &&
                      !(d->flags & (LVT_CAUSAL_KMAX | LVT_CAUSAL_KMIN | LVT_CAUSAL_TILE));
    if (wide && d->ta == 0 && d->tb == 0) rc = launch_wide<0, 0>(p, zc, s);
    else if (wide && d->ta == 0 && d->tb == 1) rc = launch_wide<0, 1>(p, zc, s);
    else if (wide) rc = launch_wide<1, 1>(p, zc, s);
    else if (d->ta == 0 && d->tb == 0) rc = launch_tile<A_KPLAIN, B_KPLAIN, 128, 128, 2, 2>(p, zc, s);
    else if (d->ta == 0 && d->tb == 1) rc = launch_tile<A_KPLAIN, B_NPLAIN, 128, 128, 2, 2>(p, zc, s);
    else rc = launch_tile<A_MPLAIN, B_NPLAIN, 128, 128, 2, 2>(p, zc, s);
    if (rc != LVT_OK) return rc;
    if (p.splits > 1) {
        const long long n4 = p.partial_stride / 4;
        const int blocks = (int)(lvt_cdiv(n4, 256) < 2048 ? lvt_cdiv(n4, 256) : 2048);
        hipLaunchKernelGGL(lvt_reduce_splits_kernel, dim3(blocks), dim3(256), 0, s, p.partial, n4,
                           p.partial_stride, p.splits, d->C, (d->flags & LVT_EPI_ACCUM) ? 1 : 0);
        LVT_CHECK_LAUNCH("lvt_reduce_splits_kernel");
        if (p.colsum_partial) {
            hipLaunchKernelGGL(lvt_reduce_splits_kernel, dim3((unsigned)lvt_cdiv((long long)zc * d->M / 4, 256)), dim3(256), 0, s,
                               (const float *)p.colsum_partial, (long long)zc * d->M / 4, (long long)zc * d->M, p.splits,
                               d->a_colsum, 0);
            LVT_CHECK_LAUNCH("lvt_reduce_splits_kernel");
        }
    }
    return LVT_OK;
}

struct PackTable { const float *w[64]; float *dst[64]; int kind[64], taps[64], Ci[64], Co[64], Ci_real[64], Co_real[64]; };
__global__ void lvt_pack_weights_multi_kernel(const PackTable t) {
    const int e = blockIdx.y;
    const float *__restrict__ w = t.w[e];
    float *__restrict__ dst = t.dst[e];
    const int kind = t.kind[e], taps = t.taps[e], Ci = t.Ci[e], Co = t.Co[e], Ci_real = t.Ci_real[e], Co_real = t.Co_real[e];
    const long long total = (long long)(kind >= 2 ? 16 : taps) * Ci * Co;
    for (long long i = (long long)blockIdx.x * blockDim.x + threadIdx.x; i < total; i += (long long)gridDim.x * blockDim.x) {
        int co, ci, tap;
        if (kind == 0 || kind == 3) { co = i % Co; const long long q = i / Co; ci = q % Ci; tap = (int)(q / Ci); }
        else { ci = i % Ci; const long long q = i / Ci; co = q % Co; tap = (int)(q / Co); }
        int src_tap = tap;
        if (kind == 1) src_tap = taps - 1 - tap;
        else if (kind == 2) { const int ph = tap >> 2, tp = tap & 3; src_tap = (3 - (ph >> 1) - 2 * (tp >> 1)) * 4 + 3 - (ph & 1) - 2 * (tp & 1); }
        else if (kind == 3) { const int cls = tap >> 2, tp = tap & 3; src_tap = (2 * (tp >> 1) + (cls >> 1)) * 4 + 2 * (tp & 1) + (cls & 1); }
        float v = 0.f;
        if (co < Co_real && ci < Ci_real) v = w[((long long)co * Ci_real + ci) * (kind >= 2 ? 16 : taps) + src_tap];
        dst[i] = v;
    }
}
extern "C" int lvt_conv3d_pack_weights_multi(const lvt_pack_entry *entries, int n, void *stream) {
    LVT_REQUIRE(entries && n > 0, "pack_weights_multi: bad args");
    for (int base = 0; base < n; base += 64) {
        const int cnt = n - base < 64 ? n - base : 64;
        PackTable t;
        long long biggest = 0;
        for (int i = 0; i < cnt; ++i) {
            const lvt_pack_entry &e = entries[base + i];
            LVT_REQUIRE(e.w && e.dst && e.kind >= 0 && e.kind <= 3 && e.taps > 0 && e.Ci > 0 && e.Co > 0 && e.Ci_real <= e.Ci &&
                            e.Co_real <= e.Co && (e.kind < 2 || e.taps == 16), "pack_weights_multi: bad entry %d", base + i);
            t.w[i] = e.w; t.dst[i] = e.dst; t.kind[i] = e.kind; t.taps[i] = e.taps; t.Ci[i] = e.Ci; t.Co[i] = e.Co;
            t.Ci_real[i] = e.Ci_real; t.Co_real[i] = e.Co_real;
            const long long total = (long long)e.taps * e.Ci * e.Co;
            if (total > biggest) biggest = total;
        }
        const unsigned bx = (unsigned)(lvt_cdiv(biggest, 256) < 1024 ? lvt_cdiv(biggest, 256) : 1024);
        hipLaunchKernelGGL(lvt_pack_weights_multi_kernel, dim3(bx, (unsigned)cnt), dim3(256), 0, (hipStream_t)stream, t);
        LVT_CHECK_LAUNCH("lvt_pack_weights_multi_kernel");
    }
    return LVT_OK;
}

struct WImgTable { const float *wp[64]; char *img[64]; const float *amax[64]; int rows[64], cols[64]; };
__global__ __launch_bounds__(256) void lvt_weight_images_kernel(const WImgTable t) {
    const int e = blockIdx.y;
    const float *__restrict__ wp = t.wp[e];
    const int rows = t.rows[e], cols = t.cols[e];
    const int ntn = cols / 128, ntiles = (rows / 32) * ntn;
    int unscale = 0;
    const float sb = lvt_f16_scale(t.amax[e], unscale);
    const int n = threadIdx.x & 127, q0 = threadIdx.x >> 7;
    for (int tile = blockIdx.x; tile < ntiles; tile += gridDim.x) {
        const int kt = tile / ntn, nt = tile - kt * ntn;
        unsigned short *img = reinterpret_cast<unsigned short *>(t.img[e] + (long long)tile * PT_BIMG_BYTES);
        const float *src = wp + (long long)(kt * 32) * cols + nt * 128 + n;
#pragma unroll
        for (int kq = q0; kq < 8; kq += 2) {
            const float4 v = make_float4(src[(long long)(4 * kq) * cols], src[(long long)(4 * kq + 1) * cols],
                                         src[(long long)(4 * kq + 2) * cols], src[(long long)(4 * kq + 3) * cols]);
            store_split2_k<128>(img, n, 4 * kq, v, sb);
        }
    }
}
extern "C" size_t lvt_conv3d_weight_image_bytes(int rows, int cols) {
    if (rows <= 0 || cols <= 0 || rows % 32 || cols % 128) return 0;
    return (size_t)(rows / 32) * (cols / 128) * PT_BIMG_BYTES;
}
extern "C" int lvt_conv3d_weight_images(const lvt_weight_image_entry *entries, int n, void *stream) {
    LVT_REQUIRE(entries && n > 0, "weight_images: bad args");
    for (int base = 0; base < n; base += 64) {
        const int cnt = n - base < 64 ? n - base : 64;
        WImgTable t;
        int most = 0;
        for (int i = 0; i < cnt; ++i) {
            const lvt_weight_image_entry &e = entries[base + i];
            LVT_REQUIRE(e.wp && e.amax && e.rows > 0 && e.cols > 0 && e.rows % 32 == 0 && e.cols % 128 == 0,
                        "weight_images: entry %d: rows %% 32 / cols %% 128 / pointers", base + i);
            t.wp[i] = e.wp; t.img[i] = (char *)(e.wp + (size_t)e.rows * e.cols); t.amax[i] = e.amax; t.rows[i] = e.rows; t.cols[i] = e.cols;
            LVT_REQUIRE(lvt_aligned16(t.img[i]), "weight_images: entry %d: the packed weight must be 16-byte aligned", base + i);
            const int tiles = (e.rows / 32) * (e.cols / 128);
            if (tiles > most) most = tiles;
// ... 443 lines not shown
```

lvt_amd/csrc/lvt_core.hip:

```cpp
#include "lvt_common.h"
#include <string.h>

static thread_local char g_err[512] = "";

void lvt_set_error(const char *fmt, ...) {
    va_list ap;
    va_start(ap, fmt);
    vsnprintf(g_err, sizeof(g_err), fmt, ap);
    va_end(ap);
}

extern "C" const char *lvt_last_error(void) { return g_err; }
extern "C" int lvt_version(void) { return 630; }

extern "C" int lvt_device_info(char *name, int name_len, int *cus, int *clock_khz, long long *hbm_bytes) {
    int n = 0;
    if (hipGetDeviceCount(&n) != hipSuccess || n == 0) {
        lvt_set_error("no HIP device visible");
        return LVT_ENODEVICE;
    }
    int dev = 0;
    (void)hipGetDevice(&dev);
    hipDeviceProp_t prop;
    if (hipGetDeviceProperties(&prop, dev) != hipSuccess) {
        lvt_set_error("hipGetDeviceProperties failed");
        return LVT_ENODEVICE;
    }
    if (name && name_len > 0) {
        snprintf(name, name_len, "%s (%s)", prop.name, prop.gcnArchName);
    }
    if (cus) *cus = prop.multiProcessorCount;
    if (clock_khz) *clock_khz = prop.clockRate;
    if (hbm_bytes) *hbm_bytes = (long long)prop.totalGlobalMem;
    return LVT_OK;
}
```

lvt_amd/hip/binding.py:

```python
import ctypes as C
import os

import torch

_HERE = os.path.dirname(os.path.abspath(__file__))
_LIB_PATH = os.environ.get("LVT_HIP_LIB") or os.path.join(os.path.dirname(_HERE), "liblvt_hip.so")

EPI_BIAS, EPI_RESIDUAL, EPI_RELU, EPI_TANH, EPI_MASK, EPI_ACCUM, EPI_PLANES = 1, 2, 4, 8, 16, 32, 64
CAUSAL_KMAX, CAUSAL_KMIN, CAUSAL_TILE = 1 << 8, 1 << 9, 1 << 10
ABI_VERSION = 630
MATH_F32 = 1 << 16
MATH_F16X2 = 1 << 18
ONEHOT_DENSE = 1 << 19
WGRAD_DB_OF_X = 1 << 20
CONV_WEIGHT_IMAGE = 1 << 21
BN_RUNNING, BN_UPDATE, BN_UNBIASED, BN_COUNT, BN_TRAIN = 1, 2, 4, 8, 16


class LvtError(RuntimeError):
    pass


class GemmDesc(C.Structure):
    _fields_ = [
        ("M", C.c_int), ("N", C.c_int), ("K", C.c_int), ("ta", C.c_int), ("tb", C.c_int),
        ("A", C.c_void_p), ("lda", C.c_longlong), ("a_kb", C.c_int), ("a_skb", C.c_longlong),
        ("B", C.c_void_p), ("ldb", C.c_longlong), ("b_kb", C.c_int), ("b_skb", C.c_longlong),
        ("C", C.c_void_p), ("ldc", C.c_longlong),
        ("batch_outer", C.c_int), ("batch_inner", C.c_int),
        ("sA_o", C.c_longlong), ("sA_i", C.c_longlong), ("sB_o", C.c_longlong), ("sB_i", C.c_longlong),
        ("sC_o", C.c_longlong), ("sC_i", C.c_longlong),
        ("alpha", C.c_float), ("flags", C.c_int),
        ("bias", C.c_void_p), ("res", C.c_void_p), ("ldr", C.c_longlong),
        ("mask", C.c_void_p), ("ldm", C.c_longlong), ("splits", C.c_int),
        ("a_colsum", C.c_void_p), ("c_plane", C.c_longlong),
        ("a_amax", C.c_void_p), ("b_amax", C.c_void_p), ("a_amax2", C.c_void_p), ("b_amax2", C.c_void_p), ("c_amax", C.c_void_p),
    ]


class GemmP2Desc(C.Structure):
    _fields_ = [
        ("M", C.c_int), ("N", C.c_int), ("K", C.c_int),
        ("A", C.c_void_p), ("lda", C.c_longlong), ("a_planes", C.c_int), ("a_kb", C.c_int), ("a_skb", C.c_longlong),
        ("B", C.c_void_p), ("ldb", C.c_longlong),
        ("C", C.c_void_p), ("ldc", C.c_longlong),
        ("batch_outer", C.c_int), ("batch_inner", C.c_int),
        ("sA_o", C.c_longlong), ("sA_i", C.c_longlong), ("sB_o", C.c_longlong), ("sB_i", C.c_longlong),
        ("sC_o", C.c_longlong), ("sC_i", C.c_longlong),
        ("alpha", C.c_float), ("flags", C.c_int),
        ("bias", C.c_void_p), ("res", C.c_void_p), ("ldr", C.c_longlong),
        ("mask", C.c_void_p), ("ldm", C.c_longlong),
        ("a_amax", C.c_void_p), ("b_amax", C.c_void_p), ("c_amax", C.c_void_p),
        ("Cp", C.c_void_p), ("ldcp", C.c_longlong), ("cp_amax", C.c_void_p),
    ]


class P2PackEntry(C.Structure):
    _fields_ = [("src", C.c_void_p), ("dst", C.c_void_p), ("rows", C.c_int), ("cols", C.c_int), ("ld_src", C.c_longlong),
                ("ld_dst", C.c_longlong), ("transpose", C.c_int), ("amax", C.c_void_p),
                ("batch", C.c_int), ("bs_src", C.c_longlong), ("bs_dst", C.c_longlong)]


class AmaxEntry(C.Structure):
    _fields_ = [("x", C.c_void_p), ("n", C.c_longlong), ("out", C.c_void_p)]


class PackEntry(C.Structure):
    _fields_ = [("w", C.c_void_p), ("dst", C.c_void_p), ("kind", C.c_int), ("taps", C.c_int), ("Ci", C.c_int), ("Co", C.c_int),
                ("Ci_real", C.c_int), ("Co_real", C.c_int)]


class WeightImageEntry(C.Structure):
    _fields_ = [("wp", C.c_void_p), ("rows", C.c_int), ("cols", C.c_int), ("amax", C.c_void_p)]


class BnFoldEntry(C.Structure):
    _fields_ = [("w", C.c_void_p), ("w_out", C.c_void_p), ("outer", C.c_int), ("Co", C.c_int), ("inner", C.c_int),
                ("Cp", C.c_int), ("gamma", C.c_void_p), ("beta", C.c_void_p), ("running_mean", C.c_void_p),
                ("running_var", C.c_void_p), ("eps", C.c_float), ("bias_out", C.c_void_p), ("w_amax", C.c_void_p)]


class AmaxIO(C.Structure):
    _fields_ = [("a", C.c_void_p), ("b", C.c_void_p), ("c", C.c_void_p)]


class OptEntry(C.Structure):
    _fields_ = [("p", C.c_void_p), ("g", C.c_void_p), ("s0", C.c_void_p), ("s1", C.c_void_p),
                ("n", C.c_longlong), ("lr", C.c_float), ("wd", C.c_float)]


class ConvGeom(C.Structure):
    _fields_ = [(n, C.c_int) for n in
                ("N", "Ti", "Hi", "Wi", "Ci", "To", "Ho", "Wo", "Co", "Kt", "Kh", "Kw",
                 "st", "sh", "sw", "pt", "ph", "pw")]

    def key(self):
        return tuple(getattr(self, n) for n, _ in self._fields_)


_lib = None


def _declare(lib):
    vp, ci, cll, cf, sz = C.c_void_p, C.c_int, C.c_longlong, C.c_float, C.c_size_t
    P = C.POINTER
    sigs = {
        "lvt_last_error": (C.c_char_p, []),
        "lvt_version": (ci, []),
        "lvt_device_info": (ci, [C.c_char_p, ci, P(ci), P(ci), P(cll)]),
        "lvt_gemm_workspace_bytes": (sz, [P(GemmDesc)]),
        "lvt_gemm_f32": (ci, [P(GemmDesc), vp, sz, vp]),
        "lvt_vq_argmax_scores": (ci, [vp, cll, ci, cll, vp, ci, vp, vp]),
        "lvt_gemm_p2_f32": (ci, [P(GemmP2Desc), vp]),
        "lvt_p2_pack_multi": (ci, [P(P2PackEntry), ci, vp]),
        "lvt_layernorm_fwd_p2": (ci, [vp, cll, ci, cf, vp, vp, vp, vp, vp, vp, vp, vp, vp, vp]),
        "lvt_gemm_smallm_f32": (ci, [ci, ci, ci, ci, vp, cll, vp, cll, vp, cll, ci, cll, cll, cf, ci, vp, vp, cll, vp, cll, cll, vp]),
        "lvt_gemm_smallm_splitk_workspace_bytes": (sz, [ci, ci, ci]),
        "lvt_gemm_smallm_splitk_f32": (ci, [ci, ci, ci, ci, vp, cll, vp, cll, vp, cll, cf, ci, vp, vp, cll, vp, cll, cll, vp, sz, vp]),
        "lvt_gemm_smallm_partial_f32": (ci, [ci, ci, ci, ci, vp, cll, vp, cll, vp, sz, vp]),
        "lvt_splitsum_layernorm_fwd": (ci, [vp, ci, ci, ci, vp, vp, cll, vp, cf, vp, vp, vp, vp]),
        "lvt_conv3d_pack_weight": (ci, [P(ConvGeom), vp, ci, ci, vp, vp]),
        "lvt_conv3d_pack_weight_t": (ci, [P(ConvGeom), vp, ci, ci, vp, vp]),
        "lvt_conv3d_uses_patch_kernel": (ci, [P(ConvGeom), ci]),
        "lvt_conv3d_fwd_uses_parity_kernel": (ci, [P(ConvGeom), ci]),
        "lvt_conv3d_pack_weight_parity": (ci, [P(ConvGeom), vp, ci, ci, vp, vp]),
        "lvt_amax": (ci, [vp, cll, vp, vp]),
        "lvt_amax_multi": (ci, [P(AmaxEntry), ci, vp]),
        "lvt_conv3d_pack_weights_multi": (ci, [P(PackEntry), ci, vp]),
        "lvt_conv3d_weight_image_bytes": (sz, [ci, ci]),
        "lvt_conv3d_weight_images": (ci, [P(WeightImageEntry), ci, vp]),
        "lvt_amax_merge": (ci, [vp, vp, vp, vp]),
        "lvt_conv3d_fwd_parity": (ci, [P(ConvGeom), vp, vp, vp, vp, vp, vp, ci, P(AmaxIO), vp]),
        "lvt_conv3d_fwd": (ci, [P(ConvGeom), vp, vp, vp, vp, vp, vp, ci, P(AmaxIO), vp]),
        "lvt_conv3d_bwd_data_uses_phase_kernel": (ci, [P(ConvGeom), ci]),
        "lvt_conv3d_pack_weight_phases": (ci, [P(ConvGeom), vp, ci, ci, vp, vp]),
        "lvt_conv3d_bwd_data_phases": (ci, [P(ConvGeom), vp, vp, vp, vp, vp, vp, ci, P(AmaxIO), vp]),
        "lvt_conv3d_bwd_data": (ci, [P(ConvGeom), vp, vp, vp, vp, vp, vp, ci, P(AmaxIO), vp]),
        "lvt_conv3d_bwd_weight_workspace_bytes": (sz, [P(ConvGeom)]),
        "lvt_conv3d_bwd_weight_fuses_bias": (ci, [P(ConvGeom), ci]),
        "lvt_conv3d_bwd_weight": (ci, [P(ConvGeom), vp, vp, vp, vp, ci, ci, ci, P(AmaxIO), vp, sz, vp]),
        "lvt_convt4_fwd": (ci, [vp, vp, vp, ci, ci, ci, ci, ci, ci, vp, ci, vp, vp]),
        "lvt_colsum_workspace_bytes": (sz, [cll, ci]),
        "lvt_colsum": (ci, [vp, cll, ci, cll, vp, vp, sz, vp]),
        "lvt_vq_nearest_workspace_bytes": (sz, [cll, ci, ci]),
        "lvt_vq_nearest_generic_workspace_bytes": (sz, [ci, ci, ci]),
        "lvt_vq_nearest": (ci, [vp, cll, ci, ci, ci, ci, vp, vp, ci, ci, vp, sz, vp]),
        "lvt_vq_gather": (ci, [vp, vp, cll, ci, ci, ci, ci, vp, ci, vp]),
        "lvt_vq_ema_workspace_bytes": (sz, [cll, ci, ci, ci]),
        "lvt_vq_ema_accumulate": (ci, [vp, vp, cll, ci, ci, ci, ci, ci, vp, vp, sz, vp]),
        "lvt_vq_ema_finalize": (ci, [vp, ci, ci, ci, cf, cf, vp, vp, vp, vp]),
        "lvt_to_channels_last": (ci, [vp, ci, ci, cll, ci, ci, vp, vp, vp, vp, vp]),
        "lvt_to_channels_first": (ci, [vp, ci, ci, cll, ci, ci, vp, vp, cf, cf, vp, vp]),
        "lvt_reduce_workspace_bytes": (sz, []),
        "lvt_mse_fwd": (ci, [vp, vp, cll, C.c_double, cf, vp, vp, sz, vp]),
        "lvt_mse_bwd": (ci, [vp, vp, cll, C.c_double, cf, vp, vp, ci, vp, vp, vp]),
        "lvt_l1_fwd": (ci, [vp, vp, cll, C.c_double, cf, vp, vp, sz, vp]),
        "lvt_l1_bwd": (ci, [vp, vp, cll, C.c_double, cf, vp, vp, ci, vp, vp, vp]),
        "lvt_tanh_bwd": (ci, [vp, vp, cll, vp, vp, vp]),
        "lvt_axpy": (ci, [vp, vp, cll, vp, cf, vp, vp]),
        "lvt_add_periodic": (ci, [vp, vp, cll, ci, ci, vp]),
        "lvt_layernorm_fwd": (ci, [vp, cll, ci, cf, vp, vp, vp, vp, vp, vp, vp, vp, vp]),
        "lvt_layernorm_bwd_workspace_bytes": (sz, [ci]),
        "lvt_layernorm_bwd": (ci, [vp, vp, vp, vp, vp, cll, ci, vp, vp, vp, vp, vp, vp, sz, vp]),
        "lvt_attn_softmax_fwd": (ci, [vp, ci, ci, ci, cf, vp, vp, vp, ci, ci, ci, ci, cf, vp]),
        "lvt_attn_softmax_bwd": (ci, [vp, vp, ci, ci, ci, cf, ci, ci, ci, vp, vp, vp, vp, vp]),
        "lvt_attn_fwd": (ci, [vp, vp, vp, ci, ci, ci, ci, cf, vp, vp, vp, ci, ci, ci, ci, cf, vp, vp, vp]),
        "lvt_attn_planes_supported": (ci, [ci, ci, ci, ci, ci]),
        "lvt_attn_fwd_planes": (ci, [vp, cll, cll, ci, ci, ci, ci, cf, vp, vp, vp, ci, ci, ci, ci, cf, vp, vp, vp, vp]),
        "lvt_attn_bwd_planes_workspace_bytes": (sz, [ci, ci, ci, ci, ci, ci]),
        "lvt_attn_bwd_planes": (ci, [vp, cll, cll, vp, vp, vp, ci, ci, ci, ci, cf, ci, ci, ci, ci, vp, vp, vp, vp, vp, vp, vp, vp, sz, vp]),
        "lvt_attn_flash_supported": (ci, [ci, ci, ci, ci, ci]),
        "lvt_attn_fwd_flash": (ci, [vp, vp, vp, cll, ci, ci, ci, ci, cf, vp, vp, vp, ci, ci, ci, ci, cf, vp, vp, vp, vp]),
        "lvt_attn_bwd_flash_workspace_bytes": (sz, [ci, ci, ci, ci, ci, ci]),
        "lvt_attn_bwd_flash": (ci, [vp, vp, vp, vp, cll, vp, vp, ci, ci, ci, ci, cf, vp, vp, vp, ci, ci, ci, ci, cf, vp, vp, vp, vp,
                                    vp, vp, vp, vp, sz, vp]),
        "lvt_attn_decode": (ci, [vp, cll, vp, vp, ci, ci, ci, ci, ci, cf, vp, vp, vp, ci, ci, ci, vp, vp, cll, vp]),
        "lvt_decode_gather_codes": (ci, [vp, vp, vp, ci, ci, ci, vp, vp]),
        "lvt_decode_commit": (ci, [vp, ci, ci, vp, vp, vp]),
        "lvt_sample_categorical": (ci, [vp, cll, ci, cf, vp, vp, cll, vp, vp, cll, vp]),
        "lvt_embbag_fwd": (ci, [vp, cll, ci, cll, ci, P(ci), P(ci), vp, ci, vp, vp, vp, vp, vp]),
        "lvt_onehot_tn_workspace_bytes": (sz, [ci, ci, ci, cll]),
        "lvt_onehot_tn_is_gather": (ci, [ci, ci, ci, cll, vp, ci]),
        "lvt_onehot_tn_gemm": (ci, [vp, ci, ci, P(ci), cll, cll, ci, cll, vp, cll, ci, vp, ci, vp, vp, sz, vp]),
        "lvt_permute3": (ci, [vp, cll, cll, cll, ci, ci, ci, vp, vp]),
        "lvt_row_gather": (ci, [vp, vp, cll, ci, ci, vp, vp]),
        "lvt_slice_context": (ci, [vp, ci, ci, ci, ci, ci, vp, ci, ci, ci, ci, ci, ci, ci, cll, vp, vp, vp, vp, vp]),
        "lvt_xent_workspace_bytes": (sz, []),
        "lvt_xent_fwd": (ci, [vp, vp, cll, cll, ci, cll, ci, cll, cf, vp, vp, vp, vp, vp, sz, vp]),
        "lvt_xent_bwd": (ci, [vp, vp, cll, cll, ci, cll, ci, cll, vp, vp, vp, cf, vp, vp, vp]),
        "lvt_adam_step": (ci, [P(OptEntry), ci, cf, cf, cf, ci, vp]),
        "lvt_rmsprop_step": (ci, [P(OptEntry), ci, cf, cf, cf, vp]),
        "lvt_bn_workspace_bytes": (sz, [cll, ci]),
        "lvt_bn_stats": (ci, [vp, cll, ci, vp, vp, sz, vp]),
        "lvt_bn_finalize": (ci, [vp, ci, cll, ci, ci, vp, vp, vp, vp, vp, cf, cf, ci, vp, vp, vp, vp]),
        "lvt_bn_apply": (ci, [vp, vp, cll, ci, vp, vp, ci, vp, vp, vp]),
        "lvt_bn_bwd_reduce": (ci, [vp, vp, cll, ci, vp, vp, vp, sz, vp]),
        "lvt_bn_bwd_apply": (ci, [vp, vp, cll, ci, vp, vp, vp, cll, ci, vp, vp, vp]),
        "lvt_bn_fold": (ci, [P(BnFoldEntry), ci, vp]),
    }
    for name, (res, args) in sigs.items():
        fn = getattr(lib, name)
        fn.restype = res
        fn.argtypes = args
    return sigs


def available():
    return os.path.exists(_LIB_PATH)


def lib():
    global _lib
    if _lib is None:
        if not os.path.exists(_LIB_PATH):
            raise LvtError("liblvt_hip.so not found at %s -- run `python -c 'import __graft_entry__ as g; "
                           "g.build()'` (or `make -C lvt_amd/csrc`); there is no CPU fallback" % _LIB_PATH)
        handle = C.CDLL(_LIB_PATH)
        handle.lvt_version.restype = C.c_int
        if handle.lvt_version() != ABI_VERSION:
            raise LvtError("liblvt_hip.so at %s has ABI version %d, this package binds version %d -- rebuild it "
                           "(`make -C lvt_amd/csrc`)" % (_LIB_PATH, handle.lvt_version(), ABI_VERSION))
        handle._lvt_sigs = _declare(handle)
        _lib = handle
    return _lib


MATH_MODES = ("f32", "bf16x3", "f16x2")
_math_mode = os.environ.get("LVT_MATH", "f16x2")
if _math_mode not in MATH_MODES:
    raise LvtError("LVT_MATH must be one of %s (got %r)" % (MATH_MODES, _math_mode))


def set_math_mode(mode):
    global _math_mode
    if mode not in MATH_MODES:
        raise LvtError("math mode must be one of %s (got %r)" % (MATH_MODES, mode))
    _math_mode = mode
    bump_epoch()


def get_math_mode():
    return _math_mode


def math_flag():
    return MATH_F32 if _math_mode == "f32" else (MATH_F16X2 if _math_mode == "f16x2" else 0)


def f16x2():
    return _math_mode == "f16x2"


_amax_pool, _amax_pos, _epoch = None, 0, 0
_wgen, _wlog = 0, {}
_WLOG_MAX = 64


def bump_epoch():
# ... 265 lines not shown
```

lvt_amd/hip/ew.py:

```python
import ctypes as C

import torch

from . import binding as L


def _f32(*shape, like):
    return torch.empty(*shape, dtype=torch.float32, device=like.device)


def to_channels_last(x_bcr, ldo, mode=0, a=None, s=None):
    L.require(x_bcr, a, s)
    B, Cc, R = x_bcr.shape
    out = _f32(B, R, ldo, like=x_bcr)
    L.check(L.lib().lvt_to_channels_last(L.ptr(x_bcr), B, Cc, R, ldo, mode, L.ptr(a), L.ptr(s), L.ptr(out),
                                         L.out_amax(out), L.stream_ptr()), "lvt_to_channels_last")
    return out


def to_channels_first(x_brc, Cc, mode=0, a=None, s=None, lo=0.0, hi=0.0):
    L.require(x_brc, a, s)
    B, R, ldi = x_brc.shape
    out = _f32(B, Cc, R, like=x_brc)
    L.check(L.lib().lvt_to_channels_first(L.ptr(x_brc), B, Cc, R, ldi, mode, L.ptr(a), L.ptr(s), lo, hi,
                                          L.ptr(out), L.stream_ptr()), "lvt_to_channels_first")
    return out


def _red_ws(dev):
    n = L.lib().lvt_reduce_workspace_bytes()
    return L.workspace(n, dev, "reduce"), n


def mse_fwd(a, b, denom, scale=1.0, l1=False):
    L.require(a, b)
    out = _f32(1, like=a)
    ws, n = _red_ws(a.device)
    L.check((L.lib().lvt_l1_fwd if l1 else L.lib().lvt_mse_fwd)(L.ptr(a), L.ptr(b), a.numel(), float(denom), scale, L.ptr(out), L.ptr(ws), n,
                                L.stream_ptr()), "lvt_mse_fwd")
    return out.view(())


def mse_bwd(a, b, denom, scale=1.0, gout=None, add=None, tanh_of_a=False, l1=False):
    L.require(a, b, gout, add)
    out = torch.empty_like(a)
    L.check((L.lib().lvt_l1_bwd if l1 else L.lib().lvt_mse_bwd)(L.ptr(a), L.ptr(b), a.numel(), float(denom), scale, L.ptr(gout), L.ptr(add),
                                1 if tanh_of_a else 0, L.ptr(out), L.out_amax(out), L.stream_ptr()), "lvt_mse_bwd")
    return out


def tanh_bwd(g, y):
    L.require(g, y)
    out = torch.empty_like(g)
    L.check(L.lib().lvt_tanh_bwd(L.ptr(g), L.ptr(y), g.numel(), L.ptr(out), L.out_amax(out), L.stream_ptr()), "lvt_tanh_bwd")
    return out


def axpy(x, alpha=1.0, alpha_dev=None, add=None):
    L.require(x, alpha_dev, add)
    out = torch.empty_like(x)
    L.check(L.lib().lvt_axpy(L.ptr(x), L.ptr(add), x.numel(), L.ptr(alpha_dev), alpha, L.ptr(out), L.stream_ptr()),
            "lvt_axpy")
    return out


def add_periodic_(x, table, P):
    L.require(x, table)
    d = x.shape[-1]
    L.check(L.lib().lvt_add_periodic(L.ptr(x), L.ptr(table), x.numel() // d, P, d, L.stream_ptr()),
            "lvt_add_periodic")
    L.drop_amax(x)
    return x


def layernorm_fwd(x, w, b, eps=1e-5, save_stats=True):
    L.require(x, w, b)
    d = x.shape[-1]
    rows = x.numel() // d
    y = torch.empty_like(x)
    mean = _f32(rows, like=x) if save_stats else None
    rstd = _f32(rows, like=x) if save_stats else None
    f16 = L.f16x2()
    L.check(L.lib().lvt_layernorm_fwd(L.ptr(x), rows, d, eps, L.ptr(w), L.ptr(b), L.ptr(y), L.ptr(mean),
                                      L.ptr(rstd), L.out_amax(y), L.ptr(L.amax_of(w)) if f16 else None,
                                      L.ptr(L.amax_of(b)) if f16 else None, L.stream_ptr()), "lvt_layernorm_fwd")
    return y, mean, rstd


def layernorm_fwd_p2(x, w, b, eps=1e-5):
    L.require(x, w, b)
    d = x.shape[-1]
    rows = x.numel() // d
    y = torch.empty_like(x)
    yp = torch.empty_like(x)
    mean, rstd = _f32(rows, like=x), _f32(rows, like=x)
    L.check(L.lib().lvt_layernorm_fwd_p2(L.ptr(x), rows, d, eps, L.ptr(w), L.ptr(b), L.ptr(y), L.ptr(yp), L.ptr(mean),
                                         L.ptr(rstd), L.out_amax(y), L.ptr(L.amax_of(w)), L.ptr(L.amax_of(b)),
                                         L.stream_ptr()), "lvt_layernorm_fwd_p2")
    return y, yp, mean, rstd


def layernorm_bwd(dy, x, mean, rstd, w, add=None):
    L.require(dy, x, mean, rstd, w, add)
    d = x.shape[-1]
    rows = x.numel() // d
    dx = torch.empty_like(x)
    dw, db = _f32(d, like=x), _f32(d, like=x)
    n = L.lib().lvt_layernorm_bwd_workspace_bytes(d)
    ws = L.workspace(n, x.device, "ln")
    L.check(L.lib().lvt_layernorm_bwd(L.ptr(dy), L.ptr(x), L.ptr(mean), L.ptr(rstd), L.ptr(w), rows, d, L.ptr(add),
                                      L.ptr(dx), L.ptr(dw), L.ptr(db), L.out_amax(dx), L.ptr(ws), n, L.stream_ptr()),
            "lvt_layernorm_bwd")
    return dx, dw, db


def row_gather(x, perm, S):
    L.require(x, perm)
    d = x.shape[-1]
    out = torch.empty_like(x)
    L.check(L.lib().lvt_row_gather(L.ptr(x), L.ptr(perm), x.numel() // (S * d), S, d, L.ptr(out), L.stream_ptr()),
            "lvt_row_gather")
    if L.f16x2() and L._valid_amax(x) is not None:
        L.set_amax(out, L._valid_amax(x))
    return out
```

lvt_amd/hip/gemm.py:

```python
import ctypes as C
import os

import torch

from . import binding as L


def gemm(A, B, C_out, M, N, K, ta=0, tb=0, lda=None, ldb=None, ldc=None, a_kb=0, a_skb=0, b_kb=0,
         b_skb=0, batch_outer=1, batch_inner=1, sA=(0, 0), sB=(0, 0), sC=(0, 0), alpha=1.0, flags=0,
         bias=None, res=None, ldr=0, mask=None, ldm=0, splits=1, a_colsum=None, c_plane=0, a_also=None, b_also=None):
    L.require(A, B, C_out, bias, res, mask)
    d = L.GemmDesc()
    d.M, d.N, d.K, d.ta, d.tb = M, N, K, ta, tb
    d.A, d.lda, d.a_kb, d.a_skb = A.data_ptr(), (lda if lda is not None else (K if ta == 0 else M)), a_kb, a_skb
    d.B, d.ldb, d.b_kb, d.b_skb = B.data_ptr(), (ldb if ldb is not None else (K if tb == 0 else N)), b_kb, b_skb
    d.C, d.ldc = C_out.data_ptr(), (ldc if ldc is not None else N)
    d.batch_outer, d.batch_inner = batch_outer, batch_inner
    d.sA_o, d.sA_i = sA
    d.sB_o, d.sB_i = sB
    d.sC_o, d.sC_i = sC
    d.alpha, d.flags = alpha, flags | L.math_flag()
    d.bias = bias.data_ptr() if bias is not None else None
    d.res = res.data_ptr() if res is not None else None
    d.ldr = ldr if res is not None and ldr else d.ldc
    d.mask = mask.data_ptr() if mask is not None else None
    d.ldm = ldm if mask is not None and ldm else d.ldc
    d.splits = splits
    d.a_colsum = a_colsum.data_ptr() if a_colsum is not None else None
    d.c_plane = c_plane
    if L.f16x2():
        d.a_amax, d.b_amax = L.amax_of(A).data_ptr(), L.amax_of(B).data_ptr()
        d.a_amax2 = L.amax_of(a_also).data_ptr() if a_also is not None else None
        d.b_amax2 = L.amax_of(b_also).data_ptr() if b_also is not None else None
        if splits <= 1 and C_out.dtype == torch.float32:
            d.c_amax = L.new_amax(C_out).data_ptr()
    if not d.c_amax:
        L.drop_amax(C_out)
    lib = L.lib()
    ws, nws = None, 0
    if splits > 1:
        nws = lib.lvt_gemm_workspace_bytes(C.byref(d))
        ws = L.workspace(nws, A.device, "gemm")
    t0 = L.TIMER.begin() if L.TIMER is not None else None
    L.check(lib.lvt_gemm_f32(C.byref(d), L.ptr(ws), nws, L.stream_ptr()), "lvt_gemm_f32")
    if t0 is not None:
        causal = 0.75 if flags & (L.CAUSAL_KMAX | L.CAUSAL_KMIN | L.CAUSAL_TILE) and M == 256 and N % 128 == 0 else 1.0
        L.TIMER.end("gemm_%s%s" % ("nt"[ta], "tn"[tb]), 2.0 * M * N * K * batch_outer * batch_inner * causal, t0)
    return C_out


class P2Image:
    __slots__ = ("data", "amax")

    def __init__(self, data, amax):
        self.data, self.amax = data, amax


def p2_mode(force=None):
    if not L.f16x2():
        return "off"
    if force is not None:
        return "full" if force else "off"
    env = os.environ.get("LVT_P2", "")
    if env == "qkv":
        return "qkv"
    return "full" if env not in ("", "0") else "off"


def p2_supported(force=None):
    return p2_mode(force) == "full"


def p2_pack(specs):
    arr = (L.P2PackEntry * len(specs))()
    for e, sp in zip(arr, specs):
        src, transpose, dst, amax = sp[:4]
        if src.dim() != 2 or dst.dim() != 2 or src.stride(1) != 1 or dst.stride(1) != 1 or not src.is_cuda:
            raise L.LvtError("p2_pack: 2-D device views with unit column stride expected")
        e.src, e.dst, e.rows, e.cols = src.data_ptr(), dst.data_ptr(), src.shape[0], src.shape[1]
        e.ld_src, e.ld_dst, e.transpose, e.amax = src.stride(0), dst.stride(0), int(bool(transpose)), amax.data_ptr()
        e.batch, e.bs_src, e.bs_dst = sp[4:7] if len(sp) > 4 else (1, 0, 0)
    L.check(L.lib().lvt_p2_pack_multi(arr, len(specs), L.stream_ptr()), "lvt_p2_pack_multi")


def gemm_p2(A, Bimg, C_out, M, N, K, lda=None, a_kb=0, a_skb=0, ldb=None, ldc=None, batch_outer=1, batch_inner=1, sA=(0, 0),
            sB=(0, 0), sC=(0, 0), alpha=1.0, flags=0, bias=None, res=None, ldr=0, mask=None, ldm=0, out_image=None, out_bound=None):
    a_img = isinstance(A, P2Image)
    At = A.data if a_img else A
    L.require(C_out, bias, res, mask)
    d = L.GemmP2Desc()
    d.M, d.N, d.K = M, N, K
    d.A, d.lda, d.a_planes, d.a_kb, d.a_skb = At.data_ptr(), (lda if lda is not None else K), int(a_img), a_kb, a_skb
    d.B, d.ldb = Bimg.data.data_ptr(), (ldb if ldb is not None else K)
    d.C, d.ldc = C_out.data_ptr(), (ldc if ldc is not None else N)
    d.batch_outer, d.batch_inner = batch_outer, batch_inner
    d.sA_o, d.sA_i = sA
    d.sB_o, d.sB_i = sB
    d.sC_o, d.sC_i = sC
    d.alpha, d.flags = alpha, flags | L.MATH_F16X2
    d.bias = bias.data_ptr() if bias is not None else None
    d.res = res.data_ptr() if res is not None else None
    d.ldr = ldr if res is not None and ldr else d.ldc
    d.mask = mask.data_ptr() if mask is not None else None
    d.ldm = ldm if mask is not None and ldm else d.ldc
    d.a_amax = (A.amax if a_img else L.amax_of(A)).data_ptr()
    d.b_amax = Bimg.amax.data_ptr()
    d.c_amax = L.new_amax(C_out).data_ptr()
    img = None
    if out_image is not None:
        d.Cp, d.ldcp, d.cp_amax = out_image.data_ptr(), d.ldc, out_bound.data_ptr()
        img = P2Image(out_image, out_bound)
    t0 = L.TIMER.begin() if L.TIMER is not None else None
    L.check(L.lib().lvt_gemm_p2_f32(C.byref(d), L.stream_ptr()), "lvt_gemm_p2_f32")
    if t0 is not None:
        L.TIMER.end("gemm_p2a" if a_img else "gemm_p2", 2.0 * M * N * K * batch_outer * batch_inner, t0)
    return C_out, img


def _smallm_splits(N, K):
    if K < 1024 or K % 256 != 0:
        return 1
    return K // 256


def gemm_small(A, B, C_out, M, N, K, tb=0, lda=None, ldb=None, ldc=None, batch=1, sB=0, sC=0, alpha=1.0, flags=0,
               bias=None, res=None, ldr=0, split_ws=None, pos=None, c_pos=0, r_pos=0):
    L.require(A, B, bias, res, pos)
# ... 292 lines not shown
```

lvt_amd/hip/tx.py:

```python
import ctypes as C

import torch

from . import binding as L
from . import ew


def _iarr(vals):
    return (C.c_int * len(vals))(*[int(v) for v in vals])


def attn_softmax_fwd_(scores, temper, dt, dh, dw, block, masked, fill=-1e4):
    L.require(scores, dt, dh, dw)
    B, H, S, _ = scores.shape
    L.check(L.lib().lvt_attn_softmax_fwd(L.ptr(scores), B, H, S, temper, L.ptr(dt), L.ptr(dh), L.ptr(dw),
                                         block[0], block[1], block[2], 1 if masked else 0, fill, L.stream_ptr()),
            "lvt_attn_softmax_fwd")
    L.drop_amax(scores)
    return scores


def attn_fwd_supported(S, da):
    return S == 256 and da == 128


def attn_fwd(q, k, v, B, H, S, da, temper, dt, dh, dw, block, masked, fill=-1e4):
    L.require(q, k, v, dt, dh, dw)
    P = torch.empty(B, H, S, S, dtype=torch.float32, device=q.device)
    o = torch.empty(B * S, H * da, dtype=torch.float32, device=q.device)
    t0 = L.TIMER.begin() if L.TIMER is not None else None
    L.check(L.lib().lvt_attn_fwd(L.ptr(q), L.ptr(k), L.ptr(v), B, H, S, da, temper, L.ptr(dt), L.ptr(dh), L.ptr(dw),
                                 block[0], block[1], block[2], 1 if masked else 0, fill, L.ptr(P), L.ptr(o),
                                 L.stream_ptr()), "lvt_attn_fwd")
    if t0 is not None:
        L.TIMER.end("attn_fwd", 4.0 * B * H * S * S * da, t0)
    return P, o


def attn_planes_supported(S, da, block, bh_pairs=8):
    return bh_pairs % 8 == 0 and bool(L.lib().lvt_attn_planes_supported(S, da, block[0], block[1], block[2])) and L.get_math_mode() != "f32"


def attn_fwd_planes(qkvp, B, H, S, da, temper, dt, dh, dw, block, masked, fill=-1e4):
    L.require(qkvp, dt, dh, dw)
    M, hd = B * S, H * da
    P = torch.empty(B, H, S, S, dtype=torch.float32, device=qkvp.device)
    o = torch.empty(M, hd, dtype=torch.float32, device=qkvp.device)
    t0 = L.TIMER.begin() if L.TIMER is not None else None
    L.check(L.lib().lvt_attn_fwd_planes(L.ptr(qkvp), M * hd, 3 * M * hd, B, H, S, da, temper, L.ptr(dt), L.ptr(dh), L.ptr(dw),
                                        block[0], block[1], block[2], 1 if masked else 0, fill, L.ptr(P), L.ptr(o),
                                        L.out_amax(o), L.stream_ptr()), "lvt_attn_fwd_planes")
    if t0 is not None:
        L.TIMER.end("attn_fwd", 4.0 * B * H * S * S * da, t0)
    return P, o


def attn_bwd_planes(qkvp, dop, P, o, B, H, S, da, temper, block, masked):
    L.require(qkvp, dop, P, o)
    M, hd = B * S, H * da
    dev = P.device
    dqkv = torch.empty(3, M, hd, dtype=torch.float32, device=dev)
    ddt = torch.empty(H, 2 * block[0] - 1, dtype=torch.float32, device=dev)
    ddh = torch.empty(H, 2 * block[1] - 1, dtype=torch.float32, device=dev)
    ddw = torch.empty(H, 2 * block[2] - 1, dtype=torch.float32, device=dev)
    lib = L.lib()
    nws = lib.lvt_attn_bwd_planes_workspace_bytes(B, H, S, block[0], block[1], block[2])
    ws = L.workspace(nws, dev, "attn_bwd")
    t0 = L.TIMER.begin() if L.TIMER is not None else None
    L.check(lib.lvt_attn_bwd_planes(L.ptr(qkvp), M * hd, 3 * M * hd, L.ptr(dop), L.ptr(P), L.ptr(o), B, H, S, da, temper,
                                    block[0], block[1], block[2], 1 if masked else 0, L.ptr(dqkv[0]), L.ptr(dqkv[1]),
                                    L.ptr(dqkv[2]), L.ptr(ddt), L.ptr(ddh), L.ptr(ddw), L.out_amax(dqkv), L.ptr(ws), nws,
                                    L.stream_ptr()),
            "lvt_attn_bwd_planes")
    if t0 is not None:
        L.TIMER.end("attn_bwd", 8.0 * B * H * S * S * da, t0)
    return dqkv, ddt, ddh, ddw


def attn_flash_supported(S, da, block, bh_pairs=8):
    return (bh_pairs % 8 == 0 and L.get_math_mode() == "f16x2" and
            bool(L.lib().lvt_attn_flash_supported(S, da, block[0], block[1], block[2])))


def attn_fwd_flash(qkv, B, H, S, da, temper, dt, dh, dw, block, masked, fill=-1e4):
    L.require(qkv, dt, dh, dw)
    M, hd = B * S, H * da
    o = torch.empty(M, hd, dtype=torch.float32, device=qkv.device)
    stats = torch.empty(2, B * H * S, dtype=torch.float32, device=qkv.device)
    t0 = L.TIMER.begin() if L.TIMER is not None else None
    L.check(L.lib().lvt_attn_fwd_flash(L.ptr(qkv[0]), L.ptr(qkv[1]), L.ptr(qkv[2]), hd, B, H, S, da, temper, L.ptr(dt), L.ptr(dh),
                                       L.ptr(dw), block[0], block[1], block[2], 1 if masked else 0, fill, L.ptr(o), L.ptr(stats),
                                       L.out_amax(o), L.stream_ptr()), "lvt_attn_fwd_flash")
    if t0 is not None:
        L.TIMER.end("attn_fwd", 4.0 * B * H * S * S * da, t0)
    return o, stats


def attn_bwd_flash(qkv, do, stats, B, H, S, da, temper, dt, dh, dw, block, masked, fill=-1e4, o=None):
    L.require(qkv, do, stats, dt, dh, dw, o)
    M, hd = B * S, H * da
    dev = qkv.device
    dqkv = torch.empty(3, M, hd, dtype=torch.float32, device=dev)
    ddt = torch.empty(H, 2 * block[0] - 1, dtype=torch.float32, device=dev)
    ddh = torch.empty(H, 2 * block[1] - 1, dtype=torch.float32, device=dev)
    ddw = torch.empty(H, 2 * block[2] - 1, dtype=torch.float32, device=dev)
    lib = L.lib()
    nws = lib.lvt_attn_bwd_flash_workspace_bytes(B, H, S, block[0], block[1], block[2])
    ws = L.workspace(nws, dev, "attn_bwd")
    t0 = L.TIMER.begin() if L.TIMER is not None else None
    L.check(lib.lvt_attn_bwd_flash(L.ptr(qkv[0]), L.ptr(qkv[1]), L.ptr(qkv[2]), L.ptr(do), hd, L.ptr(stats), L.ptr(o), B, H, S, da, temper,
                                   L.ptr(dt), L.ptr(dh), L.ptr(dw), block[0], block[1], block[2], 1 if masked else 0, fill,
                                   L.ptr(dqkv[0]), L.ptr(dqkv[1]), L.ptr(dqkv[2]), L.ptr(ddt), L.ptr(ddh), L.ptr(ddw),
                                   L.out_amax(dqkv), L.ptr(ws), nws, L.stream_ptr()), "lvt_attn_bwd_flash")
    if t0 is not None:
        L.TIMER.end("attn_bwd", 8.0 * B * H * S * S * da, t0)
    return dqkv, ddt, ddh, ddw


def attn_softmax_bwd_(P, dP, temper, block):
    L.require(P, dP)
    B, H, S, _ = P.shape
    G = torch.empty(H, S, S, dtype=torch.float32, device=P.device)
    ddt = torch.empty(H, 2 * block[0] - 1, dtype=torch.float32, device=P.device)
    ddh = torch.empty(H, 2 * block[1] - 1, dtype=torch.float32, device=P.device)
    ddw = torch.empty(H, 2 * block[2] - 1, dtype=torch.float32, device=P.device)
    L.check(L.lib().lvt_attn_softmax_bwd(L.ptr(P), L.ptr(dP), B, H, S, temper, block[0], block[1], block[2], L.ptr(G),
                                         L.ptr(ddt), L.ptr(ddh), L.ptr(ddw), L.stream_ptr()), "lvt_attn_softmax_bwd")
    L.drop_amax(dP)
    return ddt, ddh, ddw


MAX_SLOTS = 32


def _embbag_once(idx, bstride, P, rows, slot_off, tab_row, table, D, bias, btable, bindex):
    out = torch.empty(rows, D, dtype=torch.float32, device=idx.device)
    L.check(L.lib().lvt_embbag_fwd(L.ptr(idx), bstride, P, rows, len(slot_off), _iarr(slot_off), _iarr(tab_row),
                                   L.ptr(table), D, L.ptr(bias), L.ptr(btable), L.ptr(bindex), L.ptr(out),
                                   L.stream_ptr()), "lvt_embbag_fwd")
    return out


def embbag_fwd(idx, bstride, P, rows, slot_off, tab_row, table, D, bias=None, btable=None, bindex=None):
    L.require(idx, table, bias, btable, bindex)
    out = _embbag_once(idx, bstride, P, rows, slot_off[:MAX_SLOTS], tab_row[:MAX_SLOTS], table, D, bias, btable, bindex)
    for s in range(MAX_SLOTS, len(slot_off), MAX_SLOTS):
        part = _embbag_once(idx, bstride, P, rows, slot_off[s:s + MAX_SLOTS], tab_row[s:s + MAX_SLOTS], table, D,
                            None, None, None)
        out = ew.axpy(part, add=out)
    return out


def _onehot_once(idx, V, slot_off, bstride, pstride, P, rows, dout, N, ldb, dense):
    lib = L.lib()
    ns = len(slot_off)
    out = torch.empty(ns * V, N, dtype=torch.float32, device=dout.device)
    nws = lib.lvt_onehot_tn_workspace_bytes(ns, V, N, rows)
    ws = L.workspace(nws, dout.device, "onehot")
    ldb = ldb if ldb is not None else N
    flags = L.math_flag() | (L.ONEHOT_DENSE if dense else 0)
    gather = bool(lib.lvt_onehot_tn_is_gather(ns, V, N, ldb, L.ptr(dout), flags))
    t0 = L.TIMER.begin() if L.TIMER is not None else None
    L.check(lib.lvt_onehot_tn_gemm(L.ptr(idx), ns, V, _iarr(slot_off), bstride, pstride, P, rows, L.ptr(dout), ldb, N,
                                   L.ptr(out), flags, L.ptr(L.amax_of(dout)) if (L.f16x2() and not gather) else None,
                                   L.ptr(ws), nws, L.stream_ptr()),
            "lvt_onehot_tn_gemm")
    if t0 is not None:
        if gather:
            L.TIMER.end("embbag_wgrad_gather", 0.0, t0)
        else:
            L.TIMER.end("gemm_onehot_tn", 2.0 * ns * V * N * rows, t0)
    return out


def onehot_tn_gemm(idx, V, slot_off, bstride, pstride, P, rows, dout, N, ldb=None, dense=False):
    L.require(idx, dout)
    if len(slot_off) <= MAX_SLOTS:
        return _onehot_once(idx, V, slot_off, bstride, pstride, P, rows, dout, N, ldb, dense)
    return torch.cat([_onehot_once(idx, V, slot_off[s:s + MAX_SLOTS], bstride, pstride, P, rows, dout, N, ldb, dense)
                      for s in range(0, len(slot_off), MAX_SLOTS)], 0)



def permute3(x, strides, shape):
    L.require(x)
    out = torch.empty(*shape, dtype=torch.float32, device=x.device)
    L.check(L.lib().lvt_permute3(L.ptr(x), strides[0], strides[1], strides[2], shape[0], shape[1], shape[2],
                                 L.ptr(out), L.stream_ptr()), "lvt_permute3")
    return out


def xent_fwd(logits, target, tstride_b, tstride_pos, P, ignore, scale, want_rows=False):
    L.require(logits)
    rows, V = logits.shape
    dev = logits.device
    row_loss = torch.empty(rows, dtype=torch.float32, device=dev)
# ... 59 lines not shown
```

lvt_amd/modeling/autoregressive/vt_attention.py:

```python
import math
import os

import numpy as np
import torch
from torch import nn
from torch.nn import init

from ...hip import binding as L
from ...hip import ew, tx
from ...hip import gemm as G


class PositionalEncoding(nn.Module):

    def __init__(self, d_model, num_dims=3, min_timescale=1.0, max_timescale=1.0e4):
        super().__init__()
        assert d_model >= num_dims * 2, "d_model should be >= then 2*num_dims"
        self.d_model, self.num_dims = d_model, num_dims
        self.num_timescales = d_model // (num_dims * 2)
        inc = np.log(max_timescale / min_timescale) / self.num_timescales
        self.register_buffer("inv_timescales",
                             min_timescale * torch.exp(torch.arange(self.num_timescales).float() * -inc))
        self._tables = {}

    def table(self, T, H, W, device):
        key = (T, H, W, str(device))
        if key not in self._tables:
            inv = self.inv_timescales.detach().float().cpu()
            nts = self.num_timescales
            tab = torch.zeros(T, H, W, self.d_model)
            for dim, length in enumerate((T, H, W)):
                scaled = torch.arange(length, dtype=torch.float).view(-1, 1) * inv.view(1, -1)
                sig = torch.cat([torch.sin(scaled), torch.cos(scaled)], 1)
                shape = [1, 1, 1, 2 * nts]
                shape[dim] = length
                tab[..., dim * 2 * nts:(dim + 1) * 2 * nts] += sig.view(shape)
            self._tables[key] = tab.view(T * H * W, self.d_model).contiguous().to(device)
        return self._tables[key]

    def add_tokens_(self, x_tok, T, H, W):
        return ew.add_periodic_(x_tok, self.table(T, H, W, x_tok.device), T * H * W)

    def forward(self, x):
        b, d, T, H, W = x.shape
        tab = self.table(T, H, W, x.device).t().reshape(1, d, T, H, W)
        x += tab
        return x


class MultiHeadAttention(nn.Module):

    def __init__(self, na, d, da):
        super().__init__()
        self.na, self.da = na, da
        self.layer_norm = nn.LayerNorm(d)
        self.w_q = nn.Parameter(torch.empty(na, d, da))
        self.w_k = nn.Parameter(torch.empty(na, d, da))
        self.w_v = nn.Parameter(torch.empty(na, d, da))
        self.proj = nn.Linear(na * da, d, bias=False)
        self.init_weights()

    def init_weights(self, *args, **kwargs):
        init.xavier_normal_(self.w_q)
        init.xavier_normal_(self.w_k)
        init.xavier_normal_(self.w_v)
        init.xavier_normal_(self.proj.weight)

    def packed_qkv(self):
        ws = (self.w_q, self.w_k, self.w_v)
        buf = getattr(self, "_wqkv", None)
        n = self.w_q.numel()
        if (buf is None or buf.device != self.w_q.device or
                any(w.data_ptr() != buf.data_ptr() + buf.element_size() * n * i for i, w in enumerate(ws))):
            with torch.no_grad():
                buf = torch.stack([w.detach() for w in ws], 0).contiguous()
                for i, w in enumerate(ws):
                    w.data = buf[i]
            self._wqkv = buf
        return buf


def _splits(tiles, k):
    s = max(1, 512 // max(1, tiles))
    return max(1, min(s, k // 512 if k >= 1024 else 1))


P2_IMAGES = None


def prefetch_p2_images(module):
    mode = G.p2_mode(P2_IMAGES)
    use, full = mode != "off", mode == "full"
    specs, layers = [], []
    for m in module.modules():
        if not isinstance(m, BlockLocalAttention):
            continue
        m._p2 = None
        mha, f1 = m.mha, m.ffn[1]
        na, d, da = mha.w_q.shape
        if not use or not mha.w_q.is_cuda or d % 32 or da % 32 or f1.weight.shape[1] % 32:
            continue
        wqkv = mha.packed_qkv()
        buf = getattr(m, "_p2_buf", None)
        if buf is None or buf[0].device != wqkv.device or buf[0].shape != (3 * na * da, d) or buf[1].shape != f1.weight.shape:
            buf = m._p2_buf = (torch.empty(3 * na * da, d, dtype=torch.float32, device=wqkv.device),
                               torch.empty_like(f1.weight, dtype=torch.float32))
        aq = L.amax_of(wqkv)
        specs.append((wqkv.view(3 * na * d, da)[:d], True, buf[0][:da], aq, 3 * na, d * da, da * d))
        i1 = None
        if full:
            a1 = L.amax_of(f1.weight)
            specs.append((f1.weight.detach(), False, buf[1], a1))
            i1 = G.P2Image(buf[1], a1)
        layers.append((m, G.P2Image(buf[0], aq), i1))
    if specs:
        G.p2_pack(specs)
    for m, iq, i1 in layers:
        m._p2 = (iq, i1)


def linear_wgrad(dy, x, n_out, k_in, rows, want_bias=False):
    dw = torch.empty(n_out, k_in, dtype=torch.float32, device=dy.device)
    tiles = -(-n_out // 128) * -(-k_in // 128)
    splits = _splits(tiles, rows)
    if not want_bias:
        G.gemm(dy, x, dw, n_out, k_in, rows, ta=1, tb=1, lda=dy.shape[-1], ldb=x.shape[-1], splits=splits)
        return dw
    if splits < 2:
        G.gemm(dy, x, dw, n_out, k_in, rows, ta=1, tb=1, lda=dy.shape[-1], ldb=x.shape[-1], splits=splits)
        return dw, G.colsum(dy, rows, n_out)
    db = torch.empty(n_out, dtype=torch.float32, device=dy.device)
    G.gemm(dy, x, dw, n_out, k_in, rows, ta=1, tb=1, lda=dy.shape[-1], ldb=x.shape[-1], splits=splits, a_colsum=db)
    return dw, db


def linear_wgrad_pair(dy0, x0, dy1, x1, n_out, k_in, rows):
    es = dy0.element_size()
    da, dx = dy1.data_ptr() - dy0.data_ptr(), x1.data_ptr() - x0.data_ptr()
    if (da % (4 * es) or dx % (4 * es) or dy0.shape != dy1.shape or x0.shape != x1.shape or not
            (dy0.is_contiguous() and dy1.is_contiguous() and x0.is_contiguous() and x1.is_contiguous())):
        a, ab = linear_wgrad(dy0, x0, n_out, k_in, rows, want_bias=True)
        b, bb = linear_wgrad(dy1, x1, n_out, k_in, rows, want_bias=True)
        return torch.stack([a, b]), torch.stack([ab, bb])
    dw = torch.empty(2, n_out, k_in, dtype=torch.float32, device=dy0.device)
    db = torch.empty(2, n_out, dtype=torch.float32, device=dy0.device)
    tiles = 2 * -(-n_out // 128) * -(-k_in // 128)
    splits = _splits(tiles, rows)
    if splits < 2:
        a, ab = linear_wgrad(dy0, x0, n_out, k_in, rows, want_bias=True)
        b, bb = linear_wgrad(dy1, x1, n_out, k_in, rows, want_bias=True)
        return torch.stack([a, b]), torch.stack([ab, bb])
    G.gemm(dy0, x0, dw, n_out, k_in, rows, ta=1, tb=1, lda=n_out, ldb=k_in, batch_inner=2, sA=(0, da // es), sB=(0, dx // es),
           sC=(0, n_out * k_in), splits=splits, a_colsum=db, a_also=dy1, b_also=x1)
    return dw, db


FUSED_ATTENTION = True
PLANE_ATTENTION = None
FLASH_ATTENTION = None


def _use_flash(S, da, block, pairs):
    if os.environ.get("LVT_NO_FLASH_ATTENTION") or FLASH_ATTENTION is False:
        return False
    return tx.attn_flash_supported(S, da, block, pairs)


def _use_planes(S, da, block, pairs):
    if os.environ.get("LVT_NO_PLANE_ATTENTION") or PLANE_ATTENTION is False:
        return False
    return tx.attn_planes_supported(S, da, block, pairs)


class _BlockLocalAttentionFn(torch.autograd.Function):
    @staticmethod
    def forward(ctx, x, block, masked, dt, dh, dw, ln_w, ln_b, w_q, w_k, w_v, proj_w, f0w, f0b, f1w, f1b, f3w, f3b,
                wqkv, p2=None):
        L.require(x)
        M, d = x.shape
        S = block[0] * block[1] * block[2]
        b = M // S
        na, _, da = w_q.shape
        hd = na * da
        temper = math.sqrt(da)
        dev = x.device
        flash = FUSED_ATTENTION and _use_flash(S, da, block, b * na)
        planes = FUSED_ATTENTION and not flash and _use_planes(S, da, block, b * na)
        p2 = p2 if (p2 is not None and not planes and L.f16x2()) else None
        p2_full = p2 is not None and p2[1] is not None
        if p2_full:
            xn, xn_img, mean1, rstd1 = ew.layernorm_fwd_p2(x, ln_w, ln_b)
        else:
            xn, mean1, rstd1 = ew.layernorm_fwd(x, ln_w, ln_b)
        if planes:
            qkv = torch.empty(3, 3, M, hd, dtype=torch.bfloat16, device=dev)
            G.gemm(xn, wqkv, qkv, M, da, d, ta=0, tb=1, lda=d, ldb=da, ldc=hd, batch_outer=3, batch_inner=na,
                   sB=(na * d * da, d * da), sC=(3 * M * hd, da), flags=L.EPI_PLANES, c_plane=M * hd)
            P, o = tx.attn_fwd_planes(qkv, b, na, S, da, temper, dt, dh, dw, block, masked)
        else:
            qkv = torch.empty(3, M, hd, dtype=torch.float32, device=dev)
            if p2 is not None:
                G.gemm_p2(G.P2Image(xn_img, L.amax_of(xn)) if p2_full else xn, p2[0], qkv, M, hd, d, lda=d, ldb=d, ldc=hd,
                          batch_outer=3, batch_inner=1, sB=(hd * d, 0), sC=(M * hd, 0))
                if p2_full:
                    del xn_img
            else:
                G.gemm(xn, wqkv, qkv, M, da, d, ta=0, tb=1, lda=d, ldb=da, ldc=hd, batch_outer=3, batch_inner=na,
                       sB=(na * d * da, d * da), sC=(M * hd, da))
            q, k, v = qkv[0], qkv[1], qkv[2]
        if planes:
            pass
        elif flash:
            o, P = tx.attn_fwd_flash(qkv, b, na, S, da, temper, dt, dh, dw, block, masked)
        elif FUSED_ATTENTION and tx.attn_fwd_supported(S, da):
            P, o = tx.attn_fwd(q, k, v, b, na, S, da, temper, dt, dh, dw, block, masked)
        else:
            P = torch.empty(b, na, S, S, dtype=torch.float32, device=dev)
            G.gemm(q, k, P, S, S, da, ta=0, tb=0, lda=hd, ldb=hd, ldc=S, batch_outer=b, batch_inner=na,
                   sA=(S * hd, da), sB=(S * hd, da), sC=(na * S * S, S * S))
            tx.attn_softmax_fwd_(P, temper, dt, dh, dw, block, masked)
            o = torch.empty(M, hd, dtype=torch.float32, device=dev)
            G.gemm(P, v, o, S, da, S, ta=0, tb=1, lda=S, ldb=hd, ldc=hd, batch_outer=b, batch_inner=na,
                   sA=(na * S * S, S * S), sB=(S * hd, da), sC=(S * hd, da))
        y1 = torch.empty(M, d, dtype=torch.float32, device=dev)
        G.gemm(o, proj_w, y1, M, d, hd, flags=L.EPI_RESIDUAL, res=x)
        h1 = torch.empty(M, f1w.shape[0], dtype=torch.float32, device=dev)
        if p2_full:
            fn, fn_img, mean2, rstd2 = ew.layernorm_fwd_p2(y1, f0w, f0b)
            G.gemm_p2(G.P2Image(fn_img, L.amax_of(fn)), p2[1], h1, M, f1w.shape[0], d, flags=L.EPI_BIAS | L.EPI_RELU, bias=f1b)
            del fn_img
        else:
            fn, mean2, rstd2 = ew.layernorm_fwd(y1, f0w, f0b)
            G.gemm(fn, f1w, h1, M, f1w.shape[0], d, flags=L.EPI_BIAS | L.EPI_RELU, bias=f1b)
        if L.RELU_TRACE is not None:
            L.RELU_TRACE.append(h1 > 0)
        y2 = torch.empty(M, d, dtype=torch.float32, device=dev)
        G.gemm(h1, f3w, y2, M, d, f3w.shape[1], flags=L.EPI_BIAS | L.EPI_RESIDUAL, bias=f3b, res=y1)
        ctx.save_for_backward(x, mean1, rstd1, xn, qkv, P, o, y1, mean2, rstd2, fn, h1,
                              ln_w, wqkv, proj_w, f0w, f1w, f3w, dt, dh, dw)
        ctx.block, ctx.dims, ctx.masked, ctx.planes, ctx.flash = block, (M, d, S, b, na, da), bool(masked), bool(planes), bool(flash)
        return y2

    @staticmethod
    def backward(ctx, dy2):
        (x, mean1, rstd1, xn, qkv, P, o, y1, mean2, rstd2, fn, h1,
         ln_w, wqkv, proj_w, f0w, f1w, f3w, dt, dh, dw) = ctx.saved_tensors
        M, d, S, b, na, da = ctx.dims
        hd = na * da
        temper = math.sqrt(da)
        dev = x.device
        dy2 = dy2.contiguous()
        dff = f1w.shape[0]
        dh1 = torch.empty(M, dff, dtype=torch.float32, device=dev)
        G.gemm(dy2, f3w, dh1, M, dff, d, ta=0, tb=1, ldb=dff, flags=L.EPI_MASK, mask=h1)
        dfn = torch.empty(M, d, dtype=torch.float32, device=dev)
        G.gemm(dh1, f1w, dfn, M, d, dff, ta=0, tb=1, ldb=d)
        if d == dff:
            dwp, dbp = linear_wgrad_pair(dy2, h1, dh1, fn, d, dff, M)
            df3w, df3b, df1w, df1b = dwp[0], dbp[0], dwp[1], dbp[1]
        else:
            df3w, df3b = linear_wgrad(dy2, h1, d, dff, M, want_bias=True)
            df1w, df1b = linear_wgrad(dh1, fn, dff, d, M, want_bias=True)
        dy1, df0w, df0b = ew.layernorm_bwd(dfn, y1, mean2, rstd2, f0w, add=dy2)
        if ctx.planes:
            do = torch.empty(3, M, hd, dtype=torch.bfloat16, device=dev)
            G.gemm(dy1, proj_w, do, M, hd, d, ta=0, tb=1, ldb=hd, flags=L.EPI_PLANES, c_plane=M * hd)
            dproj = linear_wgrad(dy1, o, d, hd, M)
            dqkv, ddt, ddh, ddw = tx.attn_bwd_planes(qkv, do, P, o, b, na, S, da, temper, ctx.block, ctx.masked)
            return _BlockLocalAttentionFn._finish_backward(ctx, dqkv, ddt, ddh, ddw, dy1, dproj, df0w, df0b, df1w, df1b,
                                                            df3w, df3b)
        do = torch.empty(M, hd, dtype=torch.float32, device=dev)
        G.gemm(dy1, proj_w, do, M, hd, d, ta=0, tb=1, ldb=hd)
        dproj = linear_wgrad(dy1, o, d, hd, M)
        if ctx.flash:
            dqkv, ddt, ddh, ddw = tx.attn_bwd_flash(qkv, do, P, b, na, S, da, temper, dt, dh, dw, ctx.block, ctx.masked, o=o)
            return _BlockLocalAttentionFn._finish_backward(ctx, dqkv, ddt, ddh, ddw, dy1, dproj, df0w, df0b, df1w, df1b,
                                                            df3w, df3b)
        q, k, v = qkv[0], qkv[1], qkv[2]
        bh = dict(batch_outer=b, batch_inner=na)
        dqkv = torch.empty(3, M, hd, dtype=torch.float32, device=dev)
        dq, dk, dv = dqkv[0], dqkv[1], dqkv[2]
        G.gemm(P, do, dv, S, da, S, ta=1, tb=1, lda=S, ldb=hd, ldc=hd, sA=(na * S * S, S * S), sB=(S * hd, da),
               sC=(S * hd, da), flags=L.CAUSAL_KMIN if ctx.masked else 0, **bh)
        dP = torch.empty(b, na, S, S, dtype=torch.float32, device=dev)
        G.gemm(do, v, dP, S, S, da, ta=0, tb=0, lda=hd, ldb=hd, ldc=S, sA=(S * hd, da), sB=(S * hd, da),
               sC=(na * S * S, S * S), flags=L.CAUSAL_TILE if ctx.masked else 0, **bh)
        ddt, ddh, ddw = tx.attn_softmax_bwd_(P, dP, temper, ctx.block)
        G.gemm(dP, k, dq, S, da, S, ta=0, tb=1, lda=S, ldb=hd, ldc=hd, sA=(na * S * S, S * S), sB=(S * hd, da),
               sC=(S * hd, da), flags=L.CAUSAL_KMAX if ctx.masked else 0, **bh)
        G.gemm(dP, q, dk, S, da, S, ta=1, tb=1, lda=S, ldb=hd, ldc=hd, sA=(na * S * S, S * S), sB=(S * hd, da),
               sC=(S * hd, da), flags=L.CAUSAL_KMIN if ctx.masked else 0, **bh)
        del dP
        return _BlockLocalAttentionFn._finish_backward(ctx, dqkv, ddt, ddh, ddw, dy1, dproj, df0w, df0b, df1w, df1b, df3w, df3b)

    @staticmethod
    def _finish_backward(ctx, dqkv, ddt, ddh, ddw, dy1, dproj, df0w, df0b, df1w, df1b, df3w, df3b):
        x, mean1, rstd1, xn = ctx.saved_tensors[:4]
        ln_w, wqkv = ctx.saved_tensors[12], ctx.saved_tensors[13]
        M, d, S, b, na, da = ctx.dims
        hd = na * da
        dev = x.device
        dxn = torch.empty(M, d, dtype=torch.float32, device=dev)
        G.gemm(dqkv, wqkv, dxn, M, d, 3 * hd, ta=0, tb=0, lda=hd, a_kb=hd, a_skb=M * hd, ldb=da, b_kb=da, b_skb=d * da)
        dws = torch.empty(3, na, d, da, dtype=torch.float32, device=dev)
        G.gemm(xn, dqkv, dws, d, da, M, ta=1, tb=1, lda=d, ldb=hd, ldc=da, batch_outer=3, batch_inner=na,
               sB=(M * hd, da), sC=(na * d * da, d * da), splits=_splits(3 * na * -(-d // 128), M))
        dx, dlnw, dlnb = ew.layernorm_bwd(dxn, x, mean1, rstd1, ln_w, add=dy1)
        return (dx, None, None, ddt, ddh, ddw, dlnw, dlnb, dws[0], dws[1], dws[2], dproj, df0w, df0b,
                df1w, df1b, df3w, df3b, None, None)


class BlockLocalAttention(nn.Module):
    def __init__(self, block_size, da, d, n_head, masked=False):
        super().__init__()
        self.block_size = tuple(block_size)
        self.n_head, self.masked = n_head, masked
        self.mha = MultiHeadAttention(n_head, d, da)
        self.ffn = nn.Sequential(nn.LayerNorm(d), nn.Linear(d, d), nn.ReLU(True), nn.Linear(d, d))
        t, h, w = self.block_size
        self.dt_bank = nn.Parameter(torch.zeros(n_head, 2 * t - 1))
        self.dh_bank = nn.Parameter(torch.zeros(n_head, 2 * h - 1))
        self.dw_bank = nn.Parameter(torch.zeros(n_head, 2 * w - 1))
        it = torch.arange(t).view(t, 1, 1).expand(t, h, w).reshape(-1, 1)
        ih = torch.arange(h).view(1, h, 1).expand(t, h, w).reshape(-1, 1)
        iw = torch.arange(w).view(1, 1, w).expand(t, h, w).reshape(-1, 1)
        for name, ix, n in (("dt", it, t), ("dh", ih, h), ("dw", iw, w)):
            self.register_buffer(name, (ix - ix.t() + (n - 1)).reshape(-1))
        if masked:
            s = t * h * w
            self.register_buffer("mask", torch.triu(torch.ones(1, 1, s, s), diagonal=1))
        else:
            self.register_buffer("mask", None)

    def get_B(self):
        t, h, w = self.block_size
        s = t * h * w
        return (self.dt_bank.index_select(1, self.dt) + self.dh_bank.index_select(1, self.dh)
                + self.dw_bank.index_select(1, self.dw)).view(self.n_head, 1, s, s)

    def forward_tokens(self, x_tok, thw=None):
        m, f = self.mha, self.ffn
        split = thw is not None and tuple(thw) != self.block_size
        if split:
            perm, inv = _block_permutation(tuple(thw), self.block_size, x_tok.device)
            S = perm.numel()
            x_tok = _RowPermuteFn.apply(x_tok, perm, inv, S)
        y = _BlockLocalAttentionFn.apply(
            x_tok, self.block_size, self.masked, self.dt_bank, self.dh_bank, self.dw_bank,
            m.layer_norm.weight, m.layer_norm.bias, m.w_q, m.w_k, m.w_v, m.proj.weight,
            f[0].weight, f[0].bias, f[1].weight, f[1].bias, f[3].weight, f[3].bias, m.packed_qkv(), getattr(self, "_p2", None))
        if split:
            y = _RowPermuteFn.apply(y, inv, perm, S)
        return y

    def forward(self, x):
        from .. import convstack
        B, C, T, H, W = x.shape
        tok = convstack._TokensIn.apply(x)
        tok = self.forward_tokens(tok, (T, H, W))
        return convstack._TokensOut.apply(tok, B, C, T, H, W)


_perm_cache = {}


def _block_permutation(thw, block, device):
    key = (thw, block, str(device))
    hit = _perm_cache.get(key)
    if hit is None:
        (T, H, W), (t, h, w) = thw, block
        if T % t or H % h or W % w:
            raise ValueError("volume %s is not a multiple of the attention block %s" % (thw, block))
        r = torch.arange(T * H * W).view(T // t, t, H // h, h, W // w, w)
        perm = r.permute(0, 2, 4, 1, 3, 5).reshape(-1)
        inv = torch.empty_like(perm)
        inv[perm] = torch.arange(perm.numel())
        hit = _perm_cache[key] = (perm.to(device), inv.to(device))
    return hit


class _RowPermuteFn(torch.autograd.Function):

    @staticmethod
    def forward(ctx, x, perm, inv, S):
        ctx.save_for_backward(perm, inv)
        ctx.S = S
        return ew.row_gather(x.contiguous(), perm, S)

    @staticmethod
    def backward(ctx, g):
# ... 3 lines not shown
```

Measured before the change: 1427.

## Defer split-K, layernorm and bank partial reductions into one batched launch per layer

```diff
diff --git a/include/lvt_hip.h b/include/lvt_hip.h
--- a/include/lvt_hip.h
+++ b/include/lvt_hip.h
@@ -59,6 +59,25 @@
 } lvt_gemm_desc;
 size_t lvt_gemm_workspace_bytes(const lvt_gemm_desc *d);
 int lvt_gemm_f32(const lvt_gemm_desc *d, void *workspace, size_t workspace_bytes, void *stream);
+
+#define LVT_REDUCE_SPLITS 0
+#define LVT_REDUCE_ROWS   1
+#define LVT_REDUCE_BANKS  2
+#define LVT_REDUCE_MAX_ENTRIES 16
+typedef struct {
+    int kind;
+    const float *partial;
+    long long n, stride;
+    int count;
+    int accumulate;
+    float *out, *out1, *out2;
+    int H, nt, nh, nw;
+} lvt_reduce_entry;
+int lvt_reduce_multi(const lvt_reduce_entry *entries, int n, void *stream);
+int lvt_reduce_multi_plan(const lvt_reduce_entry *entries, int n, int *launch_of, int *wg_begin, int *wg_count, int *grids,
+                          int max_launches);
+int lvt_gemm_f32_deferred(const lvt_gemm_desc *d, void *workspace, size_t workspace_bytes, lvt_reduce_entry *entries,
+                          int *n_entries, void *stream);
 
 int lvt_vq_argmax_scores(const float *scores, long long rows, int K, long long ld, const float *codebook, int D,
                          long long *idx, void *stream);
@@ -190,6 +209,10 @@
 int lvt_layernorm_bwd(const float *dy, const float *x, const float *mean, const float *rstd,
                       const float *w, long long rows, int d, const float *add, float *dx, float *dw,
                       float *db, float *dx_amax, void *workspace, size_t workspace_bytes, void *stream);
+int lvt_layernorm_bwd_deferred(const float *dy, const float *x, const float *mean, const float *rstd,
+                               const float *w, long long rows, int d, const float *add, float *dx, float *dw,
+                               float *db, float *dx_amax, void *workspace, size_t workspace_bytes,
+                               lvt_reduce_entry *entries, void *stream);
 
 int lvt_attn_softmax_fwd(float *scores, int B, int H, int S, float temper, const float *dt,
                          const float *dh, const float *dw, int bt, int bh, int bw, int masked, float fill,
@@ -220,6 +243,11 @@
                        const float *o, int B, int H, int S, int da, float temper, const float *dt, const float *dh, const float *dw,
                        int bt, int bh, int bw, int masked, float fill, float *dq, float *dk, float *dv, float *ddt,
                        float *ddh, float *ddw, float *d_amax, void *workspace, size_t workspace_bytes, void *stream);
+int lvt_attn_bwd_flash_deferred(const float *q, const float *k, const float *v, const float *d_o, long long ld, const float *stats,
+                                const float *o, int B, int H, int S, int da, float temper, const float *dt, const float *dh,
+                                const float *dw, int bt, int bh, int bw, int masked, float fill, float *dq, float *dk, float *dv,
+                                float *ddt, float *ddh, float *ddw, float *d_amax, void *workspace, size_t workspace_bytes,
+                                lvt_reduce_entry *entry, void *stream);
 
 int lvt_attn_decode(const float *q, long long ldq, const float *Kc, const float *Vc, int B, int H, int S, int da, int qi,
                     float temper, const float *dt, const float *dh, const float *dw, int bt, int bh, int bw,
diff --git a/lvt_amd/csrc/attention_flash.hip b/lvt_amd/csrc/attention_flash.hip
--- a/lvt_amd/csrc/attention_flash.hip
+++ b/lvt_amd/csrc/attention_flash.hip
@@ -1,4 +1,5 @@
 #include "attn_common.h"
+#include "reduce_bodies.h"
 
 namespace {
 
@@ -923,18 +924,7 @@
 __global__ __launch_bounds__(256) void lvt_attn_flash_bank_reduce_kernel(const float *__restrict__ partial, int B, int H, int NB, int nt,
                                                                          int nh, float *__restrict__ ddt, float *__restrict__ ddh,
                                                                          float *__restrict__ ddw) {
-    const int idx = blockIdx.x * 4 + (threadIdx.x >> 6), lane = threadIdx.x & 63;
-    if (idx >= H * NB) return;
-    const int h = idx / NB, e = idx % NB;
-    float s = 0.f;
-    for (int jj = lane; jj < 2 * B; jj += 64) s += partial[(((long long)(jj >> 1) * H + h) * 2 + (jj & 1)) * NB + e];
-#pragma unroll
-    for (int m = 32; m >= 1; m >>= 1) s += __shfl_xor(s, m, 64);
-    if (lane) return;
-    const int nw = NB - nt - nh;
-    if (e < nt) ddt[h * nt + e] = nt == 1 ? 0.f : s;
-    else if (e < nt + nh) ddh[h * nh + e - nt] = nh == 1 ? 0.f : s;
-    else ddw[h * nw + e - nt - nh] = nw == 1 ? 0.f : s;
+    lvt_flash_bank_reduce_body(blockIdx.x, partial, B, H, NB, nt, nh, ddt, ddh, ddw);
 }
 
 }
@@ -974,10 +964,11 @@
     return (size_t)B * H * S * sizeof(float) + (size_t)B * H * 4 * sizeof(float) + (size_t)B * H * 2 * nb * sizeof(float);
 }
 
-extern "C" int lvt_attn_bwd_flash(const float *q, const float *k, const float *v, const float *d_o, long long ld, const float *stats,
-                                  const float *o, int B, int H, int S, int da, float temper, const float *dt, const float *dh, const float *dw,
-                                  int bt, int bh, int bw, int masked, float fill, float *dq, float *dk, float *dv, float *ddt,
-                                  float *ddh, float *ddw, float *d_amax, void *workspace, size_t workspace_bytes, void *stream) {
+static int attn_bwd_flash_run(const float *q, const float *k, const float *v, const float *d_o, long long ld, const float *stats,
+                              const float *o, int B, int H, int S, int da, float temper, const float *dt, const float *dh, const float *dw,
+                              int bt, int bh, int bw, int masked, float fill, float *dq, float *dk, float *dv, float *ddt,
+                              float *ddh, float *ddw, float *d_amax, void *workspace, size_t workspace_bytes, lvt_reduce_entry *defer,
+                              void *stream) {
     LVT_REQUIRE(q && k && v && d_o && stats && dt && dh && dw && dq && dk && dv && ddt && ddh && ddw && B > 0 && H > 0, "attn_bwd_flash: bad args");
     LVT_REQUIRE((B * H) % 8 == 0, "attn_bwd_flash: B * H = %d must be a multiple of 8 (workgroup pairing per XCD)", B * H);
     LVT_REQUIRE(lvt_attn_flash_supported(S, da, bt, bh, bw), "attn_bwd_flash: S=%d da=%d block (%d,%d,%d) has no instantiation", S, da, bt, bh, bw);
@@ -1019,8 +1010,31 @@
     LVT_FA_GEOMS(LVT_X)
 #undef LVT_X
     LVT_CHECK_LAUNCH("lvt_attn_bwd_flash_b_kernel");
+    if (defer) {
+        lvt_reduce_entry e = {};
+        e.kind = LVT_REDUCE_BANKS; e.partial = A.bank_partial; e.count = B; e.H = H; e.nt = nt; e.nh = nh; e.nw = nw;
+        e.out = ddt; e.out1 = ddh; e.out2 = ddw;
+        *defer = e;
+        return LVT_OK;
+    }
     hipLaunchKernelGGL(lvt_attn_flash_bank_reduce_kernel, dim3((unsigned)lvt_cdiv((long long)H * nb, 4)), dim3(256), 0, s,
                        A.bank_partial, B, H, nb, nt, nh, ddt, ddh, ddw);
     LVT_CHECK_LAUNCH("lvt_attn_flash_bank_reduce_kernel");
     return LVT_OK;
 }
+extern "C" int lvt_attn_bwd_flash(const float *q, const float *k, const float *v, const float *d_o, long long ld, const float *stats,
+                                  const float *o, int B, int H, int S, int da, float temper, const float *dt, const float *dh, const float *dw,
+                                  int bt, int bh, int bw, int masked, float fill, float *dq, float *dk, float *dv, float *ddt,
+                                  float *ddh, float *ddw, float *d_amax, void *workspace, size_t workspace_bytes, void *stream) {
+    return attn_bwd_flash_run(q, k, v, d_o, ld, stats, o, B, H, S, da, temper, dt, dh, dw, bt, bh, bw, masked, fill, dq, dk, dv, ddt, ddh,
+                              ddw, d_amax, workspace, workspace_bytes, nullptr, stream);
+}
+extern "C" int lvt_attn_bwd_flash_deferred(const float *q, const float *k, const float *v, const float *d_o, long long ld,
+                                           const float *stats, const float *o, int B, int H, int S, int da, float temper, const float *dt,
+                                           const float *dh, const float *dw, int bt, int bh, int bw, int masked, float fill, float *dq,
+                                           float *dk, float *dv, float *ddt, float *ddh, float *ddw, float *d_amax, void *workspace,
+                                           size_t workspace_bytes, lvt_reduce_entry *entry, void *stream) {
+    LVT_REQUIRE(entry, "attn_bwd_flash_deferred: no room for the entry");
+    return attn_bwd_flash_run(q, k, v, d_o, ld, stats, o, B, H, S, da, temper, dt, dh, dw, bt, bh, bw, masked, fill, dq, dk, dv, ddt, ddh,
+                              ddw, d_amax, workspace, workspace_bytes, entry, stream);
+}
diff --git a/lvt_amd/csrc/elementwise.hip b/lvt_amd/csrc/elementwise.hip
--- a/lvt_amd/csrc/elementwise.hip
+++ b/lvt_amd/csrc/elementwise.hip
@@ -1,4 +1,5 @@
 #include "lvt_common.h"
+#include "reduce_bodies.h"
 
 static inline int grid_for(long long n, int per_block, int cap = 8192) {
     long long b = lvt_cdiv(n, per_block);
@@ -449,32 +450,12 @@
 __global__ __launch_bounds__(256) void lvt_rowsum_partials_kernel(const float *__restrict__ partial0, const float *__restrict__ partial1,
                                                                   int nblk, int n, float *__restrict__ out0, float *__restrict__ out1) {
     __shared__ float red[256];
-    const float *partial = blockIdx.y ? partial1 : partial0;
-    float *out = blockIdx.y ? out1 : out0;
-    constexpr int cols = 8, RL = 256 / cols;
-    const int c = blockIdx.x * cols + (threadIdx.x % cols);
-    const int rl = threadIdx.x / cols;
-    float s0 = 0.f, s1 = 0.f, s2 = 0.f, s3 = 0.f;
-    if (c < n) {
-        int b = rl;
-        for (; b + 3 * RL < nblk; b += 4 * RL) {
-            s0 += partial[(long long)b * n + c]; s1 += partial[(long long)(b + RL) * n + c];
-            s2 += partial[(long long)(b + 2 * RL) * n + c]; s3 += partial[(long long)(b + 3 * RL) * n + c];
-        }
-        for (; b < nblk; b += RL) s0 += partial[(long long)b * n + c];
-    }
-    float s = (s0 + s1) + (s2 + s3);
-    red[threadIdx.x] = s;
-    __syncthreads();
-    if (rl == 0 && c < n) {
-        for (int k = 1; k < RL; ++k) s += red[k * cols + threadIdx.x];
-        out[c] = s;
-    }
+    lvt_rowsum_partials_body(blockIdx.x, blockIdx.y ? partial1 : partial0, nblk, n, blockIdx.y ? out1 : out0, red);
 }
 extern "C" size_t lvt_layernorm_bwd_workspace_bytes(int d) { return (size_t)2 * LN_BWD_BLOCKS * d * sizeof(float); }
-extern "C" int lvt_layernorm_bwd(const float *dy, const float *x, const float *mean, const float *rstd,
-                                 const float *w, long long rows, int d, const float *add, float *dx, float *dw,
-                                 float *db, float *dx_amax, void *workspace, size_t workspace_bytes, void *stream) {
+static int layernorm_bwd_run(const float *dy, const float *x, const float *mean, const float *rstd,
+                             const float *w, long long rows, int d, const float *add, float *dx, float *dw,
+                             float *db, float *dx_amax, void *workspace, size_t workspace_bytes, lvt_reduce_entry *defer, void *stream) {
     LVT_REQUIRE(dy && x && mean && rstd && w && dx && dw && db && rows > 0 && d % 4 == 0 && d <= 256 * LN_MAXV,
                 "layernorm_bwd: bad args");
     LVT_REQUIRE(workspace && workspace_bytes >= lvt_layernorm_bwd_workspace_bytes(d), "layernorm_bwd: workspace");
@@ -486,10 +467,29 @@
     hipLaunchKernelGGL(lvt_layernorm_bwd_kernel, dim3(blocks), dim3(256), 0, s, dy, x, mean, rstd, w, rows, d, add,
                        dx, pdw, pdb, dx_amax);
     LVT_CHECK_LAUNCH("lvt_layernorm_bwd_kernel");
+    if (defer) {
+        lvt_reduce_entry e = {};
+        e.kind = LVT_REDUCE_ROWS; e.n = d; e.count = blocks;
+        e.partial = pdw; e.out = dw; defer[0] = e;
+        e.partial = pdb; e.out = db; defer[1] = e;
+        return LVT_OK;
+    }
     hipLaunchKernelGGL(lvt_rowsum_partials_kernel, dim3((d + 7) / 8, 2), dim3(256), 0, s, (const float *)pdw, (const float *)pdb,
                        blocks, d, dw, db);
     LVT_CHECK_LAUNCH("lvt_rowsum_partials_kernel");
     return LVT_OK;
+}
+extern "C" int lvt_layernorm_bwd(const float *dy, const float *x, const float *mean, const float *rstd,
+                                 const float *w, long long rows, int d, const float *add, float *dx, float *dw,
+                                 float *db, float *dx_amax, void *workspace, size_t workspace_bytes, void *stream) {
+    return layernorm_bwd_run(dy, x, mean, rstd, w, rows, d, add, dx, dw, db, dx_amax, workspace, workspace_bytes, nullptr, stream);
+}
+extern "C" int lvt_layernorm_bwd_deferred(const float *dy, const float *x, const float *mean, const float *rstd,
+                                          const float *w, long long rows, int d, const float *add, float *dx, float *dw,
+                                          float *db, float *dx_amax, void *workspace, size_t workspace_bytes,
+                                          lvt_reduce_entry *entries, void *stream) {
+    LVT_REQUIRE(entries, "layernorm_bwd_deferred: no room for the entries");
+    return layernorm_bwd_run(dy, x, mean, rstd, w, rows, d, add, dx, dw, db, dx_amax, workspace, workspace_bytes, entries, stream);
 }
 
 struct SliceGeom { int B, T, nc, H, W, st, sh, sw, kt, kh, kw, n_prime, t, h, w, Tc, Hc, Wc; long long pad; };
diff --git a/lvt_amd/csrc/gemm_engine.hip b/lvt_amd/csrc/gemm_engine.hip
--- a/lvt_amd/csrc/gemm_engine.hip
+++ b/lvt_amd/csrc/gemm_engine.hip
@@ -1,5 +1,6 @@
 #include "lvt_common.h"
 #include "epilogue_fast.h"
+#include "reduce_bodies.h"
 #include <string.h>
 #include <stdlib.h>
 #include <stdint.h>
@@ -1509,30 +1510,7 @@
 
 __global__ void lvt_reduce_splits_kernel(const float *__restrict__ partial, long long n4, long long stride,
                                          int splits, float *__restrict__ out, int accumulate) {
-    long long i = (long long)blockIdx.x * blockDim.x + threadIdx.x;
-    const long long step = (long long)gridDim.x * blockDim.x;
-    for (; i < n4; i += step) {
-        float4 s0 = ldg4(partial + i * 4), s1 = zero4(), s2 = zero4(), s3 = zero4();
-        int k = 1;
-        for (; k + 3 < splits; k += 4) {
-            const float4 t0 = ldg4(partial + k * stride + i * 4), t1 = ldg4(partial + (k + 1) * stride + i * 4);
-            const float4 t2 = ldg4(partial + (k + 2) * stride + i * 4), t3 = ldg4(partial + (k + 3) * stride + i * 4);
-            s0.x += t0.x; s0.y += t0.y; s0.z += t0.z; s0.w += t0.w;
-            s1.x += t1.x; s1.y += t1.y; s1.z += t1.z; s1.w += t1.w;
-            s2.x += t2.x; s2.y += t2.y; s2.z += t2.z; s2.w += t2.w;
-            s3.x += t3.x; s3.y += t3.y; s3.z += t3.z; s3.w += t3.w;
-        }
-        for (; k < splits; ++k) {
-            const float4 t = ldg4(partial + k * stride + i * 4);
-            s0.x += t.x; s0.y += t.y; s0.z += t.z; s0.w += t.w;
-        }
-        float4 s;
-        s.x = (s0.x + s1.x) + (s2.x + s3.x); s.y = (s0.y + s1.y) + (s2.y + s3.y);
-        s.z = (s0.z + s1.z) + (s2.z + s3.z); s.w = (s0.w + s1.w) + (s2.w + s3.w);
-        float4 *o = reinterpret_cast<float4 *>(out + i * 4);
-        if (accumulate) { const float4 c = *o; s.x += c.x; s.y += c.y; s.z += c.z; s.w += c.w; }
-        *o = s;
-    }
+    lvt_reduce_splits_body(blockIdx.x, gridDim.x, partial, n4, stride, splits, out, accumulate);
 }
 
 __global__ void lvt_pack_weight_kernel(const float *__restrict__ w, float *__restrict__ wp, int taps, int Ci,
@@ -1782,7 +1760,7 @@
     return (size_t)d->splits * gemm_batch(d) * ((size_t)d->M * d->N + (d->a_colsum ? (size_t)d->M : 0)) * sizeof(float);
 }
 
-extern "C" int lvt_gemm_f32(const lvt_gemm_desc *d, void *workspace, size_t workspace_bytes, void *stream) {
+static int gemm_run(const lvt_gemm_desc *d, void *workspace, size_t workspace_bytes, lvt_reduce_entry *defer, int *n_defer, void *stream) {
     LVT_REQUIRE(d && d->A && d->B && d->C, "gemm: null pointer");
     LVT_REQUIRE(d->M > 0 && d->N > 0 && d->K > 0, "gemm: bad shape %d %d %d", d->M, d->N, d->K);
     LVT_REQUIRE(d->K % 4 == 0, "gemm: K=%d must be a multiple of 4", d->K);
@@ -1838,7 +1816,16 @@
     else if (d->ta == 0 && d->tb == 1) rc = launch_tile<A_KPLAIN, B_NPLAIN, 128, 128, 2, 2>(p, zc, s);
     else rc = launch_tile<A_MPLAIN, B_NPLAIN, 128, 128, 2, 2>(p, zc, s);
     if (rc != LVT_OK) return rc;
-    if (p.splits > 1) {
+    if (p.splits > 1 && defer) {
+        lvt_reduce_entry e = {};
+        e.kind = LVT_REDUCE_SPLITS; e.partial = p.partial; e.n = e.stride = p.partial_stride; e.count = p.splits;
+        e.accumulate = (d->flags & LVT_EPI_ACCUM) ? 1 : 0; e.out = d->C;
+        defer[(*n_defer)++] = e;
+        if (p.colsum_partial) {
+            e.partial = p.colsum_partial; e.n = e.stride = (long long)zc * d->M; e.accumulate = 0; e.out = d->a_colsum;
+            defer[(*n_defer)++] = e;
+        }
+    } else if (p.splits > 1) {
         const long long n4 = p.partial_stride / 4;
         const int blocks = (int)(lvt_cdiv(n4, 256) < 2048 ? lvt_cdiv(n4, 256) : 2048);
         hipLaunchKernelGGL(lvt_reduce_splits_kernel, dim3(blocks), dim3(256), 0, s, p.partial, n4,
@@ -1852,6 +1839,15 @@
         }
     }
     return LVT_OK;
+}
+extern "C" int lvt_gemm_f32(const lvt_gemm_desc *d, void *workspace, size_t workspace_bytes, void *stream) {
+    return gemm_run(d, workspace, workspace_bytes, nullptr, nullptr, stream);
+}
+extern "C" int lvt_gemm_f32_deferred(const lvt_gemm_desc *d, void *workspace, size_t workspace_bytes, lvt_reduce_entry *entries,
+                                     int *n_entries, void *stream) {
+    LVT_REQUIRE(d && d->splits > 1 && entries && n_entries, "gemm_deferred: needs splits > 1 and room for the entries");
+    *n_entries = 0;
+    return gemm_run(d, workspace, workspace_bytes, entries, n_entries, stream);
 }
 
 struct PackTable { const float *w[64]; float *dst[64]; int kind[64], taps[64], Ci[64], Co[64], Ci_real[64], Co_real[64]; };
diff --git a/lvt_amd/csrc/lvt_core.hip b/lvt_amd/csrc/lvt_core.hip
--- a/lvt_amd/csrc/lvt_core.hip
+++ b/lvt_amd/csrc/lvt_core.hip
@@ -11,7 +11,7 @@
 }
 
 extern "C" const char *lvt_last_error(void) { return g_err; }
-extern "C" int lvt_version(void) { return 630; }
+extern "C" int lvt_version(void) { return 640; }
 
 extern "C" int lvt_device_info(char *name, int name_len, int *cus, int *clock_khz, long long *hbm_bytes) {
     int n = 0;
diff --git a/lvt_amd/csrc/reduce_bodies.h b/lvt_amd/csrc/reduce_bodies.h
--- /dev/null
+++ b/lvt_amd/csrc/reduce_bodies.h
@@ -0,0 +1,72 @@
+#pragma once
+#include "lvt_common.h"
+
+__device__ __forceinline__ float4 lvt_ld4(const float *p) { return *reinterpret_cast<const float4 *>(p); }
+
+__device__ __forceinline__ void lvt_reduce_splits_body(int wg, int nwg, const float *__restrict__ partial, long long n4,
+                                                       long long stride, int splits, float *__restrict__ out, int accumulate) {
+    long long i = (long long)wg * 256 + threadIdx.x;
+    const long long step = (long long)nwg * 256;
+    for (; i < n4; i += step) {
+        float4 s0 = lvt_ld4(partial + i * 4), s1 = make_float4(0.f, 0.f, 0.f, 0.f), s2 = s1, s3 = s1;
+        int k = 1;
+        for (; k + 3 < splits; k += 4) {
+            const float4 t0 = lvt_ld4(partial + k * stride + i * 4), t1 = lvt_ld4(partial + (k + 1) * stride + i * 4);
+            const float4 t2 = lvt_ld4(partial + (k + 2) * stride + i * 4), t3 = lvt_ld4(partial + (k + 3) * stride + i * 4);
+            s0.x += t0.x; s0.y += t0.y; s0.z += t0.z; s0.w += t0.w;
+            s1.x += t1.x; s1.y += t1.y; s1.z += t1.z; s1.w += t1.w;
+            s2.x += t2.x; s2.y += t2.y; s2.z += t2.z; s2.w += t2.w;
+            s3.x += t3.x; s3.y += t3.y; s3.z += t3.z; s3.w += t3.w;
+        }
+        for (; k < splits; ++k) {
+            const float4 t = lvt_ld4(partial + k * stride + i * 4);
+            s0.x += t.x; s0.y += t.y; s0.z += t.z; s0.w += t.w;
+        }
+        float4 s;
+        s.x = (s0.x + s1.x) + (s2.x + s3.x); s.y = (s0.y + s1.y) + (s2.y + s3.y);
+        s.z = (s0.z + s1.z) + (s2.z + s3.z); s.w = (s0.w + s1.w) + (s2.w + s3.w);
+        float4 *o = reinterpret_cast<float4 *>(out + i * 4);
+        if (accumulate) { const float4 c = *o; s.x += c.x; s.y += c.y; s.z += c.z; s.w += c.w; }
+        *o = s;
+    }
+}
+
+__device__ __forceinline__ void lvt_rowsum_partials_body(int wg, const float *__restrict__ partial, int nblk, int n,
+                                                         float *__restrict__ out, float *red) {
+    constexpr int cols = 8, RL = 256 / cols;
+    const int c = wg * cols + (threadIdx.x % cols);
+    const int rl = threadIdx.x / cols;
+    float s0 = 0.f, s1 = 0.f, s2 = 0.f, s3 = 0.f;
+    if (c < n) {
+        int b = rl;
+        for (; b + 3 * RL < nblk; b += 4 * RL) {
+            s0 += partial[(long long)b * n + c]; s1 += partial[(long long)(b + RL) * n + c];
+            s2 += partial[(long long)(b + 2 * RL) * n + c]; s3 += partial[(long long)(b + 3 * RL) * n + c];
+        }
+        for (; b < nblk; b += RL) s0 += partial[(long long)b * n + c];
+    }
+    float s = (s0 + s1) + (s2 + s3);
+    red[threadIdx.x] = s;
+    __syncthreads();
+    if (rl == 0 && c < n) {
+        for (int k = 1; k < RL; ++k) s += red[k * cols + threadIdx.x];
+        out[c] = s;
+    }
+}
+
+__device__ __forceinline__ void lvt_flash_bank_reduce_body(int wg, const float *__restrict__ partial, int B, int H, int NB, int nt,
+                                                           int nh, float *__restrict__ ddt, float *__restrict__ ddh,
+                                                           float *__restrict__ ddw) {
+    const int idx = wg * 4 + (threadIdx.x >> 6), lane = threadIdx.x & 63;
+    if (idx >= H * NB) return;
+    const int h = idx / NB, e = idx % NB;
+    float s = 0.f;
+    for (int jj = lane; jj < 2 * B; jj += 64) s += partial[(((long long)(jj >> 1) * H + h) * 2 + (jj & 1)) * NB + e];
+#pragma unroll
+    for (int m = 32; m >= 1; m >>= 1) s += __shfl_xor(s, m, 64);
+    if (lane) return;
+    const int nw = NB - nt - nh;
+    if (e < nt) ddt[h * nt + e] = nt == 1 ? 0.f : s;
+    else if (e < nt + nh) ddh[h * nh + e - nt] = nh == 1 ? 0.f : s;
+    else ddw[h * nw + e - nt - nh] = nw == 1 ? 0.f : s;
+}
diff --git a/lvt_amd/csrc/reduce_multi.hip b/lvt_amd/csrc/reduce_multi.hip
--- /dev/null
+++ b/lvt_amd/csrc/reduce_multi.hip
@@ -0,0 +1,112 @@
+#include "lvt_common.h"
+#include "reduce_bodies.h"
+#include <vector>
+
+namespace {
+
+struct ReduceTable {
+    lvt_reduce_entry e[LVT_REDUCE_MAX_ENTRIES];
+    int wg_begin[LVT_REDUCE_MAX_ENTRIES + 1];
+    int n;
+};
+
+__global__ __launch_bounds__(256) void lvt_reduce_multi_kernel(const ReduceTable t) {
+    __shared__ float red[256];
+    const int wg = blockIdx.x;
+    int i = 0;
+    while (i + 1 < t.n && wg >= t.wg_begin[i + 1]) ++i;
+    const lvt_reduce_entry &e = t.e[i];
+    const int local = wg - t.wg_begin[i], nwg = t.wg_begin[i + 1] - t.wg_begin[i];
+    if (e.kind == LVT_REDUCE_SPLITS) lvt_reduce_splits_body(local, nwg, e.partial, e.n / 4, e.stride, e.count, e.out, e.accumulate);
+    else if (e.kind == LVT_REDUCE_ROWS) lvt_rowsum_partials_body(local, e.partial, e.count, (int)e.n, e.out, red);
+    else lvt_flash_bank_reduce_body(local, e.partial, e.count, e.H, e.nt + e.nh + e.nw, e.nt, e.nh, e.out, e.out1, e.out2);
+}
+
+constexpr long long WG_BUDGET = 8LL * LVT_NUM_CU;
+
+bool entry_empty(const lvt_reduce_entry &e) { return e.kind == LVT_REDUCE_BANKS ? e.H == 0 : e.n == 0; }
+
+int check_entry(const lvt_reduce_entry &e, int i) {
+    LVT_REQUIRE(e.kind >= LVT_REDUCE_SPLITS && e.kind <= LVT_REDUCE_BANKS, "reduce_multi: entry %d: kind %d", i, e.kind);
+    if (entry_empty(e)) return LVT_OK;
+    LVT_REQUIRE(e.partial && e.out && e.count > 0, "reduce_multi: entry %d: null pointer or count %d", i, e.count);
+    if (e.kind == LVT_REDUCE_SPLITS)
+        LVT_REQUIRE(e.n > 0 && e.n % 4 == 0 && e.stride % 4 == 0 && e.stride >= e.n && lvt_aligned16(e.partial) && lvt_aligned16(e.out),
+                    "reduce_multi: entry %d: SPLITS needs n, stride %% 4 == 0, stride >= n and 16-byte aligned pointers", i);
+    else if (e.kind == LVT_REDUCE_ROWS)
+        LVT_REQUIRE(e.n > 0 && e.n < (1LL << 30), "reduce_multi: entry %d: ROWS n = %lld", i, e.n);
+    else
+        LVT_REQUIRE(e.out1 && e.out2 && e.H > 0 && e.nt > 0 && e.nh > 0 && e.nw > 0, "reduce_multi: entry %d: BANKS geometry", i);
+    return LVT_OK;
+}
+
+void size_launch(const lvt_reduce_entry *entries, const int *idx, int cnt, int *wg_count) {
+    long long fixed = 0, wanted = 0;
+    int nsplit = 0;
+    for (int j = 0; j < cnt; ++j) {
+        const lvt_reduce_entry &e = entries[idx[j]];
+        if (e.kind == LVT_REDUCE_SPLITS) { wanted += lvt_cdiv(e.n / 4, 256); ++nsplit; }
+        else if (e.kind == LVT_REDUCE_ROWS) fixed += lvt_cdiv(e.n, 8);
+        else fixed += lvt_cdiv((long long)e.H * (e.nt + e.nh + e.nw), 4);
+    }
+    long long avail = WG_BUDGET - fixed;
+    if (avail < nsplit) avail = nsplit;
+    for (int j = 0; j < cnt; ++j) {
+        const lvt_reduce_entry &e = entries[idx[j]];
+        long long w;
+        if (e.kind == LVT_REDUCE_SPLITS) {
+            w = lvt_cdiv(e.n / 4, 256);
+            if (wanted > avail) { w = w * avail / wanted; if (w < 1) w = 1; }
+        } else if (e.kind == LVT_REDUCE_ROWS) w = lvt_cdiv(e.n, 8);
+        else w = lvt_cdiv((long long)e.H * (e.nt + e.nh + e.nw), 4);
+        wg_count[idx[j]] = (int)w;
+    }
+}
+
+}
+
+extern "C" int lvt_reduce_multi_plan(const lvt_reduce_entry *entries, int n, int *launch_of, int *wg_begin, int *wg_count,
+                                     int *grids, int max_launches) {
+    LVT_REQUIRE(entries && n >= 0 && launch_of && wg_begin && wg_count && grids, "reduce_multi_plan: bad args");
+    int launches = 0, idx[LVT_REDUCE_MAX_ENTRIES], cnt = 0;
+    for (int i = 0; i <= n; ++i) {
+        if (i < n) {
+            const int rc = check_entry(entries[i], i);
+            if (rc != LVT_OK) return rc;
+            launch_of[i] = -1; wg_begin[i] = 0; wg_count[i] = 0;
+            if (entry_empty(entries[i])) continue;
+            idx[cnt++] = i;
+        }
+        if (cnt == LVT_REDUCE_MAX_ENTRIES || (i == n && cnt > 0)) {
+            LVT_REQUIRE(launches < max_launches, "reduce_multi_plan: more than %d launches", max_launches);
+            size_launch(entries, idx, cnt, wg_count);
+            int at = 0;
+            for (int j = 0; j < cnt; ++j) { launch_of[idx[j]] = launches; wg_begin[idx[j]] = at; at += wg_count[idx[j]]; }
+            grids[launches++] = at;
+            cnt = 0;
+        }
+    }
+    return launches;
+}
+
+extern "C" int lvt_reduce_multi(const lvt_reduce_entry *entries, int n, void *stream) {
+    LVT_REQUIRE(entries && n > 0, "reduce_multi: bad args");
+    const int max_launches = n / LVT_REDUCE_MAX_ENTRIES + 1;
+    std::vector<int> plan(3 * (size_t)n + max_launches);
+    int *launch_of = plan.data(), *wg_begin = launch_of + n, *wg_count = wg_begin + n, *grids = wg_count + n;
+    const int launches = lvt_reduce_multi_plan(entries, n, launch_of, wg_begin, wg_count, grids, max_launches);
+    if (launches < 0) return launches;
+    int i = 0;
+    for (int l = 0; l < launches; ++l) {
+        ReduceTable t = {};
+        for (; i < n && launch_of[i] <= l; ++i) {
+            if (launch_of[i] < 0) continue;
+            t.e[t.n] = entries[i];
+            t.wg_begin[t.n++] = wg_begin[i];
+        }
+        for (int j = t.n; j <= LVT_REDUCE_MAX_ENTRIES; ++j) t.wg_begin[j] = grids[l];
+        hipLaunchKernelGGL(lvt_reduce_multi_kernel, dim3((unsigned)grids[l]), dim3(256), 0, (hipStream_t)stream, t);
+        LVT_CHECK_LAUNCH("lvt_reduce_multi_kernel");
+    }
+    return LVT_OK;
+}
diff --git a/lvt_amd/hip/binding.py b/lvt_amd/hip/binding.py
--- a/lvt_amd/hip/binding.py
+++ b/lvt_amd/hip/binding.py
@@ -8,7 +8,7 @@
 
 EPI_BIAS, EPI_RESIDUAL, EPI_RELU, EPI_TANH, EPI_MASK, EPI_ACCUM, EPI_PLANES = 1, 2, 4, 8, 16, 32, 64
 CAUSAL_KMAX, CAUSAL_KMIN, CAUSAL_TILE = 1 << 8, 1 << 9, 1 << 10
-ABI_VERSION = 630
+ABI_VERSION = 640
 MATH_F32 = 1 << 16
 MATH_F16X2 = 1 << 18
 ONEHOT_DENSE = 1 << 19
@@ -70,6 +70,12 @@
                 ("Ci_real", C.c_int), ("Co_real", C.c_int)]
 
 
+class ReduceEntry(C.Structure):
+    _fields_ = [("kind", C.c_int), ("partial", C.c_void_p), ("n", C.c_longlong), ("stride", C.c_longlong), ("count", C.c_int),
+                ("accumulate", C.c_int), ("out", C.c_void_p), ("out1", C.c_void_p), ("out2", C.c_void_p),
+                ("H", C.c_int), ("nt", C.c_int), ("nh", C.c_int), ("nw", C.c_int)]
+
+
 class WeightImageEntry(C.Structure):
     _fields_ = [("wp", C.c_void_p), ("rows", C.c_int), ("cols", C.c_int), ("amax", C.c_void_p)]
 
@@ -110,6 +116,9 @@
         "lvt_device_info": (ci, [C.c_char_p, ci, P(ci), P(ci), P(cll)]),
         "lvt_gemm_workspace_bytes": (sz, [P(GemmDesc)]),
         "lvt_gemm_f32": (ci, [P(GemmDesc), vp, sz, vp]),
+        "lvt_gemm_f32_deferred": (ci, [P(GemmDesc), vp, sz, P(ReduceEntry), P(ci), vp]),
+        "lvt_reduce_multi": (ci, [P(ReduceEntry), ci, vp]),
+        "lvt_reduce_multi_plan": (ci, [P(ReduceEntry), ci, P(ci), P(ci), P(ci), P(ci), ci]),
         "lvt_vq_argmax_scores": (ci, [vp, cll, ci, cll, vp, ci, vp, vp]),
         "lvt_gemm_p2_f32": (ci, [P(GemmP2Desc), vp]),
         "lvt_p2_pack_multi": (ci, [P(P2PackEntry), ci, vp]),
@@ -162,6 +171,7 @@
         "lvt_layernorm_fwd": (ci, [vp, cll, ci, cf, vp, vp, vp, vp, vp, vp, vp, vp, vp]),
         "lvt_layernorm_bwd_workspace_bytes": (sz, [ci]),
         "lvt_layernorm_bwd": (ci, [vp, vp, vp, vp, vp, cll, ci, vp, vp, vp, vp, vp, vp, sz, vp]),
+        "lvt_layernorm_bwd_deferred": (ci, [vp, vp, vp, vp, vp, cll, ci, vp, vp, vp, vp, vp, vp, sz, P(ReduceEntry), vp]),
         "lvt_attn_softmax_fwd": (ci, [vp, ci, ci, ci, cf, vp, vp, vp, ci, ci, ci, ci, cf, vp]),
         "lvt_attn_softmax_bwd": (ci, [vp, vp, ci, ci, ci, cf, ci, ci, ci, vp, vp, vp, vp, vp]),
         "lvt_attn_fwd": (ci, [vp, vp, vp, ci, ci, ci, ci, cf, vp, vp, vp, ci, ci, ci, ci, cf, vp, vp, vp]),
@@ -174,6 +184,8 @@
         "lvt_attn_bwd_flash_workspace_bytes": (sz, [ci, ci, ci, ci, ci, ci]),
         "lvt_attn_bwd_flash": (ci, [vp, vp, vp, vp, cll, vp, vp, ci, ci, ci, ci, cf, vp, vp, vp, ci, ci, ci, ci, cf, vp, vp, vp, vp,
                                     vp, vp, vp, vp, sz, vp]),
+        "lvt_attn_bwd_flash_deferred": (ci, [vp, vp, vp, vp, cll, vp, vp, ci, ci, ci, ci, cf, vp, vp, vp, ci, ci, ci, ci, cf, vp, vp,
+                                             vp, vp, vp, vp, vp, vp, sz, P(ReduceEntry), vp]),
         "lvt_attn_decode": (ci, [vp, cll, vp, vp, ci, ci, ci, ci, ci, cf, vp, vp, vp, ci, ci, ci, vp, vp, cll, vp]),
         "lvt_decode_gather_codes": (ci, [vp, vp, vp, ci, ci, ci, vp, vp]),
         "lvt_decode_commit": (ci, [vp, ci, ci, vp, vp, vp]),
diff --git a/lvt_amd/hip/ew.py b/lvt_amd/hip/ew.py
--- a/lvt_amd/hip/ew.py
+++ b/lvt_amd/hip/ew.py
@@ -100,13 +100,20 @@
     return y, yp, mean, rstd
 
 
-def layernorm_bwd(dy, x, mean, rstd, w, add=None):
+def layernorm_bwd(dy, x, mean, rstd, w, add=None, defer=None):
     L.require(dy, x, mean, rstd, w, add)
     d = x.shape[-1]
     rows = x.numel() // d
     dx = torch.empty_like(x)
     dw, db = _f32(d, like=x), _f32(d, like=x)
     n = L.lib().lvt_layernorm_bwd_workspace_bytes(d)
+    if defer is not None:
+        ws, slots = defer.scratch(n), defer.entry_slots(2)
+        L.check(L.lib().lvt_layernorm_bwd_deferred(L.ptr(dy), L.ptr(x), L.ptr(mean), L.ptr(rstd), L.ptr(w), rows, d, L.ptr(add),
+                                                   L.ptr(dx), L.ptr(dw), L.ptr(db), L.out_amax(dx), L.ptr(ws), n, slots,
+                                                   L.stream_ptr()), "lvt_layernorm_bwd_deferred")
+        defer.take(slots)
+        return dx, dw, db
     ws = L.workspace(n, x.device, "ln")
     L.check(L.lib().lvt_layernorm_bwd(L.ptr(dy), L.ptr(x), L.ptr(mean), L.ptr(rstd), L.ptr(w), rows, d, L.ptr(add),
                                       L.ptr(dx), L.ptr(dw), L.ptr(db), L.out_amax(dx), L.ptr(ws), n, L.stream_ptr()),
diff --git a/lvt_amd/hip/gemm.py b/lvt_amd/hip/gemm.py
--- a/lvt_amd/hip/gemm.py
+++ b/lvt_amd/hip/gemm.py
@@ -8,7 +8,7 @@
 
 def gemm(A, B, C_out, M, N, K, ta=0, tb=0, lda=None, ldb=None, ldc=None, a_kb=0, a_skb=0, b_kb=0,
          b_skb=0, batch_outer=1, batch_inner=1, sA=(0, 0), sB=(0, 0), sC=(0, 0), alpha=1.0, flags=0,
-         bias=None, res=None, ldr=0, mask=None, ldm=0, splits=1, a_colsum=None, c_plane=0, a_also=None, b_also=None):
+         bias=None, res=None, ldr=0, mask=None, ldm=0, splits=1, a_colsum=None, c_plane=0, a_also=None, b_also=None, defer=None):
     L.require(A, B, C_out, bias, res, mask)
     d = L.GemmDesc()
     d.M, d.N, d.K, d.ta, d.tb = M, N, K, ta, tb
@@ -40,9 +40,14 @@
     ws, nws = None, 0
     if splits > 1:
         nws = lib.lvt_gemm_workspace_bytes(C.byref(d))
-        ws = L.workspace(nws, A.device, "gemm")
-    t0 = L.TIMER.begin() if L.TIMER is not None else None
-    L.check(lib.lvt_gemm_f32(C.byref(d), L.ptr(ws), nws, L.stream_ptr()), "lvt_gemm_f32")
+        ws = L.workspace(nws, A.device, "gemm") if defer is None else defer.scratch(nws)
+    t0 = L.TIMER.begin() if L.TIMER is not None else None
+    if splits > 1 and defer is not None:
+        slots, n = defer.entry_slots(2), C.c_int(0)
+        L.check(lib.lvt_gemm_f32_deferred(C.byref(d), L.ptr(ws), nws, slots, C.byref(n), L.stream_ptr()), "lvt_gemm_f32_deferred")
+        defer.take(slots, n.value)
+    else:
+        L.check(lib.lvt_gemm_f32(C.byref(d), L.ptr(ws), nws, L.stream_ptr()), "lvt_gemm_f32")
     if t0 is not None:
         causal = 0.75 if flags & (L.CAUSAL_KMAX | L.CAUSAL_KMIN | L.CAUSAL_TILE) and M == 256 and N % 128 == 0 else 1.0
         L.TIMER.end("gemm_%s%s" % ("nt"[ta], "tn"[tb]), 2.0 * M * N * K * batch_outer * batch_inner * causal, t0)
diff --git a/lvt_amd/hip/reduce.py b/lvt_amd/hip/reduce.py
--- /dev/null
+++ b/lvt_amd/hip/reduce.py
@@ -0,0 +1,41 @@
+import ctypes as C
+
+import torch
+
+from . import binding as L
+
+_arena = {}
+
+
+class ReduceBatch:
+
+    def __init__(self, device):
+        if torch.cuda.is_current_stream_capturing():
+            raise L.LvtError("ReduceBatch during hipGraph capture: its arena may be replaced by a later, larger batch")
+        self.device = device
+        self.key = (device, torch.cuda.current_stream(device).cuda_stream)
+        self.entries, self.used, self.extra = [], 0, []
+
+    def scratch(self, nbytes):
+        nbytes = (int(nbytes) + 255) & ~255
+        arena = _arena.get(self.key)
+        at, self.used = self.used, self.used + nbytes
+        if arena is not None and at + nbytes <= arena.numel():
+            return arena[at:at + nbytes]
+        buf = torch.empty(max(nbytes, 1), dtype=torch.uint8, device=self.device)
+        self.extra.append(buf)
+        return buf
+
+    def entry_slots(self, n):
+        return (L.ReduceEntry * n)()
+
+    def take(self, slots, n=None):
+        self.entries.extend(slots[i] for i in range(len(slots) if n is None else n))
+
+    def launch(self):
+        if self.entries:
+            arr = (L.ReduceEntry * len(self.entries))(*self.entries)
+            L.check(L.lib().lvt_reduce_multi(arr, len(self.entries), L.stream_ptr()), "lvt_reduce_multi")
+        if self.extra:
+            _arena[self.key] = torch.empty(self.used, dtype=torch.uint8, device=self.device)
+        self.entries, self.used, self.extra = [], 0, []
diff --git a/lvt_amd/hip/tx.py b/lvt_amd/hip/tx.py
--- a/lvt_amd/hip/tx.py
+++ b/lvt_amd/hip/tx.py
@@ -96,7 +96,7 @@
     return o, stats
 
 
-def attn_bwd_flash(qkv, do, stats, B, H, S, da, temper, dt, dh, dw, block, masked, fill=-1e4, o=None):
+def attn_bwd_flash(qkv, do, stats, B, H, S, da, temper, dt, dh, dw, block, masked, fill=-1e4, o=None, defer=None):
     L.require(qkv, do, stats, dt, dh, dw, o)
     M, hd = B * S, H * da
     dev = qkv.device
@@ -106,12 +106,17 @@
     ddw = torch.empty(H, 2 * block[2] - 1, dtype=torch.float32, device=dev)
     lib = L.lib()
     nws = lib.lvt_attn_bwd_flash_workspace_bytes(B, H, S, block[0], block[1], block[2])
-    ws = L.workspace(nws, dev, "attn_bwd")
-    t0 = L.TIMER.begin() if L.TIMER is not None else None
-    L.check(lib.lvt_attn_bwd_flash(L.ptr(qkv[0]), L.ptr(qkv[1]), L.ptr(qkv[2]), L.ptr(do), hd, L.ptr(stats), L.ptr(o), B, H, S, da, temper,
-                                   L.ptr(dt), L.ptr(dh), L.ptr(dw), block[0], block[1], block[2], 1 if masked else 0, fill,
-                                   L.ptr(dqkv[0]), L.ptr(dqkv[1]), L.ptr(dqkv[2]), L.ptr(ddt), L.ptr(ddh), L.ptr(ddw),
-                                   L.out_amax(dqkv), L.ptr(ws), nws, L.stream_ptr()), "lvt_attn_bwd_flash")
+    ws = L.workspace(nws, dev, "attn_bwd") if defer is None else defer.scratch(nws)
+    t0 = L.TIMER.begin() if L.TIMER is not None else None
+    args = (L.ptr(qkv[0]), L.ptr(qkv[1]), L.ptr(qkv[2]), L.ptr(do), hd, L.ptr(stats), L.ptr(o), B, H, S, da, temper,
+            L.ptr(dt), L.ptr(dh), L.ptr(dw), block[0], block[1], block[2], 1 if masked else 0, fill,
+            L.ptr(dqkv[0]), L.ptr(dqkv[1]), L.ptr(dqkv[2]), L.ptr(ddt), L.ptr(ddh), L.ptr(ddw), L.out_amax(dqkv), L.ptr(ws), nws)
+    if defer is not None:
+        slots = defer.entry_slots(1)
+        L.check(lib.lvt_attn_bwd_flash_deferred(*args, slots, L.stream_ptr()), "lvt_attn_bwd_flash_deferred")
+        defer.take(slots)
+    else:
+        L.check(lib.lvt_attn_bwd_flash(*args, L.stream_ptr()), "lvt_attn_bwd_flash")
     if t0 is not None:
         L.TIMER.end("attn_bwd", 8.0 * B * H * S * S * da, t0)
     return dqkv, ddt, ddh, ddw
diff --git a/lvt_amd/modeling/autoregressive/vt_attention.py b/lvt_amd/modeling/autoregressive/vt_attention.py
--- a/lvt_amd/modeling/autoregressive/vt_attention.py
+++ b/lvt_amd/modeling/autoregressive/vt_attention.py
@@ -9,6 +9,7 @@
 from ...hip import binding as L
 from ...hip import ew, tx
 from ...hip import gemm as G
+from ...hip.reduce import ReduceBatch
 
 
 class PositionalEncoding(nn.Module):
@@ -119,42 +120,45 @@
         m._p2 = (iq, i1)
 
 
-def linear_wgrad(dy, x, n_out, k_in, rows, want_bias=False):
+def linear_wgrad(dy, x, n_out, k_in, rows, want_bias=False, defer=None):
     dw = torch.empty(n_out, k_in, dtype=torch.float32, device=dy.device)
     tiles = -(-n_out // 128) * -(-k_in // 128)
     splits = _splits(tiles, rows)
     if not want_bias:
-        G.gemm(dy, x, dw, n_out, k_in, rows, ta=1, tb=1, lda=dy.shape[-1], ldb=x.shape[-1], splits=splits)
+        G.gemm(dy, x, dw, n_out, k_in, rows, ta=1, tb=1, lda=dy.shape[-1], ldb=x.shape[-1], splits=splits, defer=defer)
         return dw
     if splits < 2:
         G.gemm(dy, x, dw, n_out, k_in, rows, ta=1, tb=1, lda=dy.shape[-1], ldb=x.shape[-1], splits=splits)
         return dw, G.colsum(dy, rows, n_out)
     db = torch.empty(n_out, dtype=torch.float32, device=dy.device)
-    G.gemm(dy, x, dw, n_out, k_in, rows, ta=1, tb=1, lda=dy.shape[-1], ldb=x.shape[-1], splits=splits, a_colsum=db)
+    G.gemm(dy, x, dw, n_out, k_in, rows, ta=1, tb=1, lda=dy.shape[-1], ldb=x.shape[-1], splits=splits, a_colsum=db, defer=defer)
     return dw, db
 
 
-def linear_wgrad_pair(dy0, x0, dy1, x1, n_out, k_in, rows):
+def _wgrad_pair_apart(dy0, x0, dy1, x1, n_out, k_in, rows):
+    a, ab = linear_wgrad(dy0, x0, n_out, k_in, rows, want_bias=True)
+    b, bb = linear_wgrad(dy1, x1, n_out, k_in, rows, want_bias=True)
+    return torch.stack([a, b]), torch.stack([ab, bb])
+
+
+def linear_wgrad_pair(dy0, x0, dy1, x1, n_out, k_in, rows, defer=None):
     es = dy0.element_size()
     da, dx = dy1.data_ptr() - dy0.data_ptr(), x1.data_ptr() - x0.data_ptr()
     if (da % (4 * es) or dx % (4 * es) or dy0.shape != dy1.shape or x0.shape != x1.shape or not
             (dy0.is_contiguous() and dy1.is_contiguous() and x0.is_contiguous() and x1.is_contiguous())):
-        a, ab = linear_wgrad(dy0, x0, n_out, k_in, rows, want_bias=True)
-        b, bb = linear_wgrad(dy1, x1, n_out, k_in, rows, want_bias=True)
-        return torch.stack([a, b]), torch.stack([ab, bb])
+        return _wgrad_pair_apart(dy0, x0, dy1, x1, n_out, k_in, rows)
     dw = torch.empty(2, n_out, k_in, dtype=torch.float32, device=dy0.device)
     db = torch.empty(2, n_out, dtype=torch.float32, device=dy0.device)
     tiles = 2 * -(-n_out // 128) * -(-k_in // 128)
     splits = _splits(tiles, rows)
     if splits < 2:
-        a, ab = linear_wgrad(dy0, x0, n_out, k_in, rows, want_bias=True)
-        b, bb = linear_wgrad(dy1, x1, n_out, k_in, rows, want_bias=True)
-        return torch.stack([a, b]), torch.stack([ab, bb])
+        return _wgrad_pair_apart(dy0, x0, dy1, x1, n_out, k_in, rows)
     G.gemm(dy0, x0, dw, n_out, k_in, rows, ta=1, tb=1, lda=n_out, ldb=k_in, batch_inner=2, sA=(0, da // es), sB=(0, dx // es),
-           sC=(0, n_out * k_in), splits=splits, a_colsum=db, a_also=dy1, b_also=x1)
+           sC=(0, n_out * k_in), splits=splits, a_colsum=db, a_also=dy1, b_also=x1, defer=defer)
     return dw, db
 
 
+LAYER_END_REDUCE = True
 FUSED_ATTENTION = True
 PLANE_ATTENTION = None
 FLASH_ATTENTION = None
@@ -251,29 +255,30 @@
         dev = x.device
         dy2 = dy2.contiguous()
         dff = f1w.shape[0]
+        rb = ctx.rb = ReduceBatch(dev) if LAYER_END_REDUCE else None
         dh1 = torch.empty(M, dff, dtype=torch.float32, device=dev)
         G.gemm(dy2, f3w, dh1, M, dff, d, ta=0, tb=1, ldb=dff, flags=L.EPI_MASK, mask=h1)
         dfn = torch.empty(M, d, dtype=torch.float32, device=dev)
         G.gemm(dh1, f1w, dfn, M, d, dff, ta=0, tb=1, ldb=d)
         if d == dff:
-            dwp, dbp = linear_wgrad_pair(dy2, h1, dh1, fn, d, dff, M)
+            dwp, dbp = linear_wgrad_pair(dy2, h1, dh1, fn, d, dff, M, defer=rb)
             df3w, df3b, df1w, df1b = dwp[0], dbp[0], dwp[1], dbp[1]
         else:
-            df3w, df3b = linear_wgrad(dy2, h1, d, dff, M, want_bias=True)
-            df1w, df1b = linear_wgrad(dh1, fn, dff, d, M, want_bias=True)
-        dy1, df0w, df0b = ew.layernorm_bwd(dfn, y1, mean2, rstd2, f0w, add=dy2)
+            df3w, df3b = linear_wgrad(dy2, h1, d, dff, M, want_bias=True, defer=rb)
+            df1w, df1b = linear_wgrad(dh1, fn, dff, d, M, want_bias=True, defer=rb)
+        dy1, df0w, df0b = ew.layernorm_bwd(dfn, y1, mean2, rstd2, f0w, add=dy2, defer=rb)
         if ctx.planes:
             do = torch.empty(3, M, hd, dtype=torch.bfloat16, device=dev)
             G.gemm(dy1, proj_w, do, M, hd, d, ta=0, tb=1, ldb=hd, flags=L.EPI_PLANES, c_plane=M * hd)
-            dproj = linear_wgrad(dy1, o, d, hd, M)
+            dproj = linear_wgrad(dy1, o, d, hd, M, defer=rb)
             dqkv, ddt, ddh, ddw = tx.attn_bwd_planes(qkv, do, P, o, b, na, S, da, temper, ctx.block, ctx.masked)
             return _BlockLocalAttentionFn._finish_backward(ctx, dqkv, ddt, ddh, ddw, dy1, dproj, df0w, df0b, df1w, df1b,
                                                             df3w, df3b)
         do = torch.empty(M, hd, dtype=torch.float32, device=dev)
         G.gemm(dy1, proj_w, do, M, hd, d, ta=0, tb=1, ldb=hd)
-        dproj = linear_wgrad(dy1, o, d, hd, M)
+        dproj = linear_wgrad(dy1, o, d, hd, M, defer=rb)
         if ctx.flash:
-            dqkv, ddt, ddh, ddw = tx.attn_bwd_flash(qkv, do, P, b, na, S, da, temper, dt, dh, dw, ctx.block, ctx.masked, o=o)
+            dqkv, ddt, ddh, ddw = tx.attn_bwd_flash(qkv, do, P, b, na, S, da, temper, dt, dh, dw, ctx.block, ctx.masked, o=o, defer=rb)
             return _BlockLocalAttentionFn._finish_backward(ctx, dqkv, ddt, ddh, ddw, dy1, dproj, df0w, df0b, df1w, df1b,
                                                             df3w, df3b)
         q, k, v = qkv[0], qkv[1], qkv[2]
@@ -304,8 +309,11 @@
         G.gemm(dqkv, wqkv, dxn, M, d, 3 * hd, ta=0, tb=0, lda=hd, a_kb=hd, a_skb=M * hd, ldb=da, b_kb=da, b_skb=d * da)
         dws = torch.empty(3, na, d, da, dtype=torch.float32, device=dev)
         G.gemm(xn, dqkv, dws, d, da, M, ta=1, tb=1, lda=d, ldb=hd, ldc=da, batch_outer=3, batch_inner=na,
-               sB=(M * hd, da), sC=(na * d * da, d * da), splits=_splits(3 * na * -(-d // 128), M))
-        dx, dlnw, dlnb = ew.layernorm_bwd(dxn, x, mean1, rstd1, ln_w, add=dy1)
+               sB=(M * hd, da), sC=(na * d * da, d * da), splits=_splits(3 * na * -(-d // 128), M), defer=ctx.rb)
+        dx, dlnw, dlnb = ew.layernorm_bwd(dxn, x, mean1, rstd1, ln_w, add=dy1, defer=ctx.rb)
+        if ctx.rb is not None:
+            ctx.rb.launch()
+            ctx.rb = None
         return (dx, None, None, ddt, ddh, ddw, dlnw, dlnb, dws[0], dws[1], dws[2], dproj, df0w, df0b,
                 df1w, df1b, df3w, df3b, None, None)
 
```

New measurement: 1432 (median of 6 runs). About the same (+0.4%).
